# zhou-lab/biscuit

Measured on AMD Instinct MI355X. Metric: paired-end reads aligned/sec, higher is better.
Workload: dtype int32

## Files before the change

### biscuit_amd/csrc/hip/dev_common.hpp

```cpp
#pragma once
#include <stdint.h>
#include "bsx.h"

#if defined(__HIPCC__)
#include <hip/hip_runtime.h>
#define BSX_HD __host__ __device__ __forceinline__
#define BSX_D  __device__ __forceinline__
#else
#define BSX_HD inline
#define BSX_D  inline
struct uint4 { uint32_t x, y, z, w; };
#endif

struct DevFmi {
	uint64_t primary;
	uint64_t L2[5];
	uint64_t seq_len;
	const uint32_t *bwt;
	const uint64_t *sa;
	uint32_t sa_mask;
	uint32_t sa_shift;
};

struct DevSeedTab { const uint4 *t[2]; int32_t K; int32_t pad_; };

struct DevIndex {
	DevFmi fmi[2];
	const uint8_t *pac;
	int64_t l_pac;
	const int64_t *ctg_off;
	const uint8_t *ctg_alt;
	int32_t n_seqs;
	DevSeedTab tab;
	const int64_t *hole_off, *hole_end;
	int32_t n_holes, pad2_;
};

struct RegParams {
	int32_t a, w, o_del, e_del, o_ins, e_ins, pen_clip5, pen_clip3;
	int32_t min_seed_len, min_chain_weight, max_chain_gap, max_occ, bsstrand;
	uint32_t max_chain_extend;
	float mask_level, drop_ratio;
	int32_t prof;
	int32_t walk_on;
	int32_t ext_win;
	int32_t gap_cap;
	int32_t flt_len;
	const int32_t *flt_tab;
};

struct DevScoring {
	int8_t ctmat[25];
	int8_t gamat[25];
	int32_t o_del, e_del, o_ins, e_ins, zdrop, a;
	int32_t mx_ct, mx_ga;
};

BSX_HD int dev_ref_base(const uint8_t *pac, int64_t l_pac, int64_t p)
{
	if (p >= l_pac) { p = (l_pac << 1) - 1 - p; return 3 - ((pac[p >> 2] >> ((~p & 3) << 1)) & 3); }
	return (pac[p >> 2] >> ((~p & 3) << 1)) & 3;
}

BSX_HD void dev_fetch_window(uint8_t *win, const uint8_t *pac, int64_t l_pac, int64_t beg, int span, int lane)
{
	if (beg < l_pac && beg + span > l_pac) {
		for (int i = lane; i < span; i += 64) win[i] = (uint8_t)dev_ref_base(pac, l_pac, beg + i);
		return;
	}
	const bool rev = beg >= l_pac;
	const int64_t f_lo = rev ? (l_pac << 1) - (beg + span) : beg;
	const int64_t b0 = (f_lo >> 2) & ~(int64_t)3;
	const int nw = (int)((((f_lo + span - 1) >> 2) - b0) >> 2) + 1;
	for (int w = lane; w < nw; w += 64) {
		const uint8_t *pw = pac + b0 + (int64_t)4 * w;
		const uint32_t v = *reinterpret_cast<const uint32_t*>(pw);
		const int64_t f0 = (b0 + (int64_t)4 * w) << 2;
#pragma unroll
		for (int k = 0; k < 16; ++k) {
			const int b = (int)(v >> (8 * (k >> 2) + ((~k & 3) << 1))) & 3;
			const int64_t i = rev ? (f_lo + span - 1) - (f0 + k) : (f0 + k) - f_lo;
			if (i >= 0 && i < span) win[i] = (uint8_t)(rev ? 3 - b : b);
		}
	}
}

BSX_HD int dev_popc(uint32_t x)
{
#if defined(__HIP_DEVICE_COMPILE__)
	return __popc(x);
#else
	return __builtin_popcount(x);
#endif
}

BSX_HD void dev_block_count(const uint32_t w[8], int upto, uint32_t cnt[4])
{
	uint32_t a = 0, c = 0, g = 0, t = 0;
#pragma unroll
	for (int i = 0; i < 8; ++i) {
		int nv = upto + 1 - 16 * i;
		nv = nv < 0 ? 0 : (nv > 16 ? 16 : nv);
		uint32_t valid = nv == 0 ? 0u : (0x55555555u & ~(uint32_t)((1ull << ((16 - nv) << 1)) - 1));
		uint32_t lo = w[i] & valid, hi = (w[i] >> 1) & valid;
		uint32_t nt = (uint32_t)dev_popc(hi & lo), ng = (uint32_t)dev_popc(hi & ~lo), nc = (uint32_t)dev_popc(lo & ~hi);
		t += nt; g += ng; c += nc; a += (uint32_t)nv - nt - ng - nc;
	}
	cnt[0] = a; cnt[1] = c; cnt[2] = g; cnt[3] = t;
// ... 142 lines not shown
```

### biscuit_amd/csrc/hip/ext_dp.hpp

```cpp
#pragma once
#include <hip/hip_runtime.h>
#include "dev_common.hpp"
#include "wave.hpp"

template <int NC>
__device__ __forceinline__ bsx_ext_res_t ext_dp(const DevIndex &ix, const DevScoring &sc, const uint8_t *reads, const bsx_ext_job_t &J,
                                                int32_t *H, int32_t *E, uint8_t *qb, int lane)
{
	const int qlen = J.qlen, tlen = J.tlen, h0 = J.h0;
	const int8_t *mat = J.parent ? sc.ctmat : sc.gamat;
	const int o_del = sc.o_del, e_del = sc.e_del, o_ins = sc.o_ins, e_ins = sc.e_ins;
	const int oe_del = o_del + e_del, oe_ins = o_ins + e_ins, zdrop = sc.zdrop;
	for (int j = lane; j < qlen; j += 64) qb[j] = reads[(long long)J.qoff + (long long)j * J.qdir];
	for (int j = lane; j <= qlen; j += 64) {
		int v = j == 0 ? h0 : h0 - oe_ins - (j - 1) * e_ins;
		H[j] = v > 0 ? v : 0; E[j] = 0;
	}
	int mx = 0;
	for (int k = 0; k < 25; ++k) mx = mx > mat[k] ? mx : mat[k];
	int w = J.w;
	{
		int max_ins = (int)((double)(qlen * mx + J.end_bonus - o_ins) / e_ins + 1.);
		max_ins = max_ins > 1 ? max_ins : 1;
		w = w < max_ins ? w : max_ins;
		int max_del = (int)((double)(qlen * mx + J.end_bonus - o_del) / e_del + 1.);
		max_del = max_del > 1 ? max_del : 1;
		w = w < max_del ? w : max_del;
	}
	int max = h0, max_i = -1, max_j = -1, max_ie = -1, gscore = -1, max_off = 0;
	int beg = 0, end = qlen;
	int tb_reg = 4;
	WAVE_SYNC();
	for (int i = 0; i < tlen; ++i) {
		if ((i & 63) == 0) tb_reg = (i + lane < tlen) ? dev_ref_base(ix.pac, ix.l_pac, J.tpos + (long long)(i + lane) * J.tdir) : 4;
		const int t = wave_bcast(tb_reg, i & 63);
		const int8_t s0 = mat[t * 5], s1 = mat[t * 5 + 1], s2 = mat[t * 5 + 2], s3 = mat[t * 5 + 3], s4 = mat[t * 5 + 4];
		if (beg < i - w) beg = i - w;
		if (end > i + w + 1) end = i + w + 1;
		if (end > qlen) end = qlen;
		int h1_init = 0;
		if (beg == 0) { h1_init = h0 - (o_del + e_del * (i + 1)); if (h1_init < 0) h1_init = 0; }
		int m = 0, mj = -1, h1_last = h1_init;
		if (beg < end) {
			const int nch = (end - beg + 63) >> 6;
			int M[NC], Ev[NC];
#pragma unroll
			for (int c = 0; c < NC; ++c) {
				M[c] = 0; Ev[c] = 0;
				if (c < nch) {
					const int j = beg + (c << 6) + lane;
					if (j < end) {
						const int hp = H[j], q = qb[j];
						const int s = q == 0 ? s0 : q == 1 ? s1 : q == 2 ? s2 : q == 3 ? s3 : s4;
						M[c] = hp ? hp + s : 0;
						Ev[c] = E[j];
					}
// ... 23 lines not shown
						H[j + 1] = h;
						if (j == beg) H[beg] = h1_init;
						if (j == end - 1) E[end] = 0;
						if (h >= lm) { lm = h; lj = j; }
					}
				}
			}
			WAVE_SYNC();
			m = wave_max_i32(lm);
			mj = wave_max_i32(lm == m ? lj : -1);
			h1_last = H[end];
		} else {
			if (lane == 0) { H[end] = h1_init; E[end] = 0; }
			WAVE_SYNC();
		}
		const int jfin = beg < end ? end : beg;
		if (jfin == qlen) { max_ie = gscore > h1_last ? max_ie : i; gscore = gscore > h1_last ? gscore : h1_last; }
		if (m == 0) break;
		if (m > max) {
			max = m; max_i = i; max_j = mj;
			int off = mj - i; off = off < 0 ? -off : off;
			max_off = max_off > off ? max_off : off;
		} else if (zdrop > 0) {
			if (i - max_i > mj - max_j) { if (max - m - ((i - max_i) - (mj - max_j)) * e_del > zdrop) break; }
			else { if (max - m - ((mj - max_j) - (i - max_i)) * e_ins > zdrop) break; }
		}
		{
			const int nchk = (end - beg + 1 + 63) >> 6;
			int nb = end, last;
			for (int c = 0; c < nchk; ++c) {
				const int j = beg + (c << 6) + lane;
				const bool nz = j < end && (H[j] != 0 || E[j] != 0);
				const unsigned long long b = __ballot(nz);
				if (b) { nb = beg + (c << 6) + __builtin_ctzll(b); break; }
			}
			last = nb - 1;
			for (int c = nchk - 1; c >= 0; --c) {
				const int j = beg + (c << 6) + lane;
				const bool nz = j <= end && j >= nb && (H[j] != 0 || E[j] != 0);
				const unsigned long long b = __ballot(nz);
				if (b) { last = beg + (c << 6) + 63 - __builtin_clzll(b); break; }
			}
			beg = nb;
			end = last + 2 < qlen ? last + 2 : qlen;
		}
		WAVE_SYNC();
	}
	bsx_ext_res_t r;
	r.score = max; r.qle = max_j + 1; r.tle = max_i + 1; r.gtle = max_ie + 1; r.gscore = gscore; r.max_off = max_off;
	WAVE_SYNC();
	return r;
}

template <int NC>
__device__ __forceinline__ bsx_ext_res_t ext_dp_reg(const DevIndex &ix, const DevScoring &sc, const uint8_t *reads, const bsx_ext_job_t &J, int lane,
                                                    const uint8_t *win = nullptr, long long win_beg = 0, const uint8_t *qlds = nullptr, uint32_t qlds_off = 0)
{
	const int qlen = J.qlen, tlen = J.tlen, h0 = J.h0;
	const int8_t *mat = J.parent ? sc.ctmat : sc.gamat;
	const int o_del = sc.o_del, e_del = sc.e_del, o_ins = sc.o_ins, e_ins = sc.e_ins;
	const int oe_del = o_del + e_del, oe_ins = o_ins + e_ins, zdrop = sc.zdrop;
	int Hr[NC], Er[NC], sq4[NC];
	uint32_t sqp[NC];
#pragma unroll
	for (int c = 0; c < NC; ++c) {
		const int a = (c << 6) + lane;
		const int q = a < qlen ? (qlds ? (int)qlds[(int)(J.qoff - qlds_off) + a * J.qdir] : (int)reads[(long long)J.qoff + (long long)a * J.qdir]) : 4;
		sqp[c] = (uint32_t)(uint8_t)mat[q] | (uint32_t)(uint8_t)mat[5 + q] << 8 | (uint32_t)(uint8_t)mat[10 + q] << 16 | (uint32_t)(uint8_t)mat[15 + q] << 24;
		sq4[c] = mat[20 + q];
		const int v = a == 0 ? h0 : h0 - oe_ins - (a - 1) * e_ins;
		Hr[c] = (a <= qlen && v > 0) ? v : 0;
		Er[c] = 0;
	}
	const int mx = J.parent ? sc.mx_ct : sc.mx_ga;
	int w = J.w;
	{
		int max_ins = (int)((double)(qlen * mx + J.end_bonus - o_ins) / e_ins + 1.);
		max_ins = max_ins > 1 ? max_ins : 1;
		w = w < max_ins ? w : max_ins;
		int max_del = (int)((double)(qlen * mx + J.end_bonus - o_del) / e_del + 1.);
		max_del = max_del > 1 ? max_del : 1;
		w = w < max_del ? w : max_del;
	}
	int max = h0, max_i = -1, max_j = -1, max_ie = -1, gscore = -1, max_off = 0;
	int beg = 0, end = qlen;
	int tb_reg = 4;
	const bool packed_max = qlen <= 512 && (long long)h0 + (long long)qlen * mx < (1 << 21);
	for (int i = 0; i < tlen; ++i) {
		if ((i & 63) == 0) {
			const long long tp = J.tpos + (long long)(i + lane) * J.tdir;
			tb_reg = (i + lane < tlen) ? (win ? (int)win[tp - win_beg] : dev_ref_base(ix.pac, ix.l_pac, tp)) : 4;
		}
		const int t = wave_bcast(tb_reg, i & 63);
		if (beg < i - w) beg = i - w;
		if (end > i + w + 1) end = i + w + 1;
		if (end > qlen) end = qlen;
		int h1_init = 0;
		if (beg == 0) { h1_init = h0 - (o_del + e_del * (i + 1)); if (h1_init < 0) h1_init = 0; }
		int m = 0, mj = -1, h1_last = h1_init;
		if (beg < end) {
			const int c0 = NC == 1 ? 0 : beg >> 6, c1 = NC == 1 ? 0 : (end - 1) >> 6;
			int hn[NC];
			int carry = NEG_BIG, lm = -1, lj = -1;
#pragma unroll
			for (int c = 0; c < NC; ++c) {
				hn[c] = 0;
				if (c >= c0 && c <= c1) {
					const int a = (c << 6) + lane;
					const bool act = a >= beg && a < end;
					const int s = t < 4 ? (int)(int8_t)(sqp[c] >> ((t & 3) << 3)) : sq4[c];
					const int M = (act && Hr[c]) ? Hr[c] + s : 0;
					int tins = M - oe_ins; tins = tins > 0 ? tins : 0;
					const int g = act ? tins + a * e_ins : NEG_BIG;
					const int incl = wave_scan_max_incl(g);
					int excl = wave_prev(incl, NEG_BIG);
					excl = excl > carry ? excl : carry;
					{ const int tot = __builtin_amdgcn_readlane(incl, 63); carry = carry > tot ? carry : tot; }
					int f = a == beg ? 0 : excl - (a - 1) * e_ins;
					if (f < 0) f = 0;
					if (act) {
						int h = M > Er[c] ? M : Er[c];
						h = h > f ? h : f;
						int tdel = M - oe_del; tdel = tdel > 0 ? tdel : 0;
						int e = Er[c] - e_del; e = e > tdel ? e : tdel;
						Er[c] = e;
						hn[c] = h;
						if (h >= lm) { lm = h; lj = a; }
					} else if (a == end) Er[c] = 0;
				}
			}
			if (NC > 1 && (end & 63) == 0 && (end >> 6) < NC && (end >> 6) > c1) {
#pragma unroll
				for (int c = 0; c < NC; ++c) if (c == (end >> 6) && lane == 0) Er[c] = 0;
			}
#pragma unroll
			for (int c = NC - 1; c >= 0; --c) {
				if (c >= c0 && c <= c1 + 1) {
					const int a = (c << 6) + lane;
					int up = wave_prev(hn[c], 0);
					const int edge = c > 0 ? __builtin_amdgcn_readlane(hn[c > 0 ? c - 1 : 0], 63) : 0;
					if (lane == 0) up = edge;
// ... 1 lines not shown
					else if (a - 1 >= beg && a - 1 < end) Hr[c] = up;
				}
			}
			if (packed_max) {
				const int key = wave_max_i32(lm < 0 ? -1 : (lm << 9 | lj));
				m = key >> 9; mj = key < 0 ? -1 : (key & 511);
			} else {
				m = wave_max_i32(lm);
				mj = wave_max_i32(lm == m ? lj : -1);
			}
			if (end == qlen) {
				int v = 0;
#pragma unroll
				for (int c = 0; c < NC; ++c) if (c == c1) v = hn[c];
				h1_last = wave_bcast(v, (end - 1) & 63);
			}
		} else {
#pragma unroll
			for (int c = 0; c < NC; ++c) if ((c << 6) + lane == end) { Hr[c] = h1_init; Er[c] = 0; }
		}
		const int jfin = beg < end ? end : beg;
		if (jfin == qlen) { max_ie = gscore > h1_last ? max_ie : i; gscore = gscore > h1_last ? gscore : h1_last; }
		if (m == 0) break;
		if (m > max) {
			max = m; max_i = i; max_j = mj;
			int off = mj - i; off = off < 0 ? -off : off;
			max_off = max_off > off ? max_off : off;
		} else if (zdrop > 0) {
			if (i - max_i > mj - max_j) { if (max - m - ((i - max_i) - (mj - max_j)) * e_del > zdrop) break; }
			else { if (max - m - ((mj - max_j) - (i - max_i)) * e_ins > zdrop) break; }
		}
		{
			int nb = end, last;
#pragma unroll
			for (int c = 0; c < NC; ++c) {
				if (NC == 1 || (nb == end && c >= (beg >> 6) && c <= ((end - 1) >> 6))) {
					const int a = (c << 6) + lane;
					const unsigned long long b = __ballot(a >= beg && a < end && (Hr[c] != 0 || Er[c] != 0));
					if (b) nb = (c << 6) + __builtin_ctzll(b);
				}
			}
			last = nb - 1;
#pragma unroll
			for (int c = NC - 1; c >= 0; --c) {
				if (NC == 1 || (last == nb - 1 && c <= (end >> 6) && c >= (nb >> 6))) {
					const int a = (c << 6) + lane;
					const unsigned long long b = __ballot(a <= end && a >= nb && (Hr[c] != 0 || Er[c] != 0));
					if (b) last = (c << 6) + 63 - __builtin_clzll(b);
				}
			}
			beg = nb;
			end = last + 2 < qlen ? last + 2 : qlen;
		}
	}
	bsx_ext_res_t r;
	r.score = max; r.qle = max_j + 1; r.tle = max_i + 1; r.gtle = max_ie + 1; r.gscore = gscore; r.max_off = max_off;
	return r;
}

template <int NW>
__device__ __forceinline__ bsx_ext_res_t ext_dp_win(const DevIndex &ix, const DevScoring &sc, const uint8_t *reads, const bsx_ext_job_t &J, int lane,
                                                    const uint8_t *win = nullptr, long long win_beg = 0, const uint8_t *qlds = nullptr, uint32_t qlds_off = 0)
{
	const int qlen = J.qlen, tlen = J.tlen, h0 = J.h0;
	const int8_t *mat = J.parent ? sc.ctmat : sc.gamat;
	const int o_del = sc.o_del, e_del = sc.e_del, o_ins = sc.o_ins, e_ins = sc.e_ins;
	const int oe_del = o_del + e_del, oe_ins = o_ins + e_ins, zdrop = sc.zdrop;
	int Hr[NW], Er[NW], sq4[NW];
	uint32_t sqp[NW];
	int cb = 0;
#define EXT_WIN_LOAD(c_, slot_) do { const int a_ = ((slot_) << 6) + lane; \
		const int q_ = a_ < qlen ? (qlds ? (int)qlds[(int)(J.qoff - qlds_off) + a_ * J.qdir] : (int)reads[(long long)J.qoff + (long long)a_ * J.qdir]) : 4; \
		sqp[c_] = (uint32_t)(uint8_t)mat[q_] | (uint32_t)(uint8_t)mat[5 + q_] << 8 | (uint32_t)(uint8_t)mat[10 + q_] << 16 | (uint32_t)(uint8_t)mat[15 + q_] << 24; \
		sq4[c_] = mat[20 + q_]; \
		const int v_ = a_ == 0 ? h0 : h0 - oe_ins - (a_ - 1) * e_ins; \
		Hr[c_] = (a_ <= qlen && v_ > 0) ? v_ : 0; Er[c_] = 0; } while (0)
#pragma unroll
	for (int c = 0; c < NW; ++c) EXT_WIN_LOAD(c, c);
	const int mx = J.parent ? sc.mx_ct : sc.mx_ga;
	int w = J.w;
	{
		int max_ins = (int)((double)(qlen * mx + J.end_bonus - o_ins) / e_ins + 1.);
		max_ins = max_ins > 1 ? max_ins : 1;
		w = w < max_ins ? w : max_ins;
		int max_del = (int)((double)(qlen * mx + J.end_bonus - o_del) / e_del + 1.);
		max_del = max_del > 1 ? max_del : 1;
		w = w < max_del ? w : max_del;
	}
	int max = h0, max_i = -1, max_j = -1, max_ie = -1, gscore = -1, max_off = 0;
	int beg = 0, end = qlen;
	int tb_reg = 4;
	for (int i = 0; i < tlen; ++i) {
		if ((i & 63) == 0) {
			const long long tp = J.tpos + (long long)(i + lane) * J.tdir;
			tb_reg = (i + lane < tlen) ? (win ? (int)win[tp - win_beg] : dev_ref_base(ix.pac, ix.l_pac, tp)) : 4;
		}
		const int t = wave_bcast(tb_reg, i & 63);
		if (beg < i - w) beg = i - w;
		if (end > i + w + 1) end = i + w + 1;
		if (end > qlen) end = qlen;
		while ((beg >> 6) > cb) {
#pragma unroll
			for (int c = 0; c + 1 < NW; ++c) { Hr[c] = Hr[c + 1]; Er[c] = Er[c + 1]; sqp[c] = sqp[c + 1]; sq4[c] = sq4[c + 1]; }
			++cb;
			EXT_WIN_LOAD(NW - 1, cb + NW - 1);
		}
// ... 103 lines not shown
```

### biscuit_amd/csrc/hip/ext_pk.hpp

```cpp
#pragma once
#include <hip/hip_runtime.h>
#include "dev_common.hpp"
#include "wave.hpp"
#include "ext_pk_bound.h"

typedef short pk2 __attribute__((ext_vector_type(2)));
__device__ __forceinline__ pk2 pk_of(uint32_t w) { return __builtin_bit_cast(pk2, w); }
__device__ __forceinline__ uint32_t pk_word(pk2 v) { return __builtin_bit_cast(uint32_t, v); }
__device__ __forceinline__ pk2 pk_splat(int v) { return pk_of((uint32_t)(v & 0xffff) * 0x10001u); }
__device__ __forceinline__ pk2 pk_pair(int lo, int hi) { return pk_of((uint32_t)(lo & 0xffff) | (uint32_t)hi << 16); }
__device__ __forceinline__ pk2 pk_max(pk2 a, pk2 b) { return __builtin_elementwise_max(a, b); }
__device__ __forceinline__ pk2 pk_neg_mask(pk2 v) { uint32_t w; asm("v_pk_ashrrev_i16 %0, 15, %1 op_sel_hi:[0,1]" : "=v"(w) : "v"(pk_word(v))); return pk_of(w); }
__device__ __forceinline__ pk2 pk_nonzero_01(pk2 v) { uint32_t w; asm("v_pk_min_u16 %0, %1, 1 op_sel_hi:[1,0]" : "=v"(w) : "v"(pk_word(v))); return pk_of(w); }
__device__ __forceinline__ pk2 pk_zero_mask(pk2 v) { return pk_nonzero_01(v) - (pk2){1, 1}; }
__device__ __forceinline__ pk2 pk_nonzero_mask(pk2 v) { return (pk2){0, 0} - pk_nonzero_01(v); }
__device__ __forceinline__ pk2 pk_sel(pk2 mask, pk2 a, pk2 b) { return (a & mask) | (b & ~mask); }

__device__ __forceinline__ pk2 wave_scan_max_incl_pk(pk2 v)
{
	int t = 0;
#define PK_SCAN_STEP(ctrl, rows) do { t = __builtin_amdgcn_update_dpp(t, (int)pk_word(v), ctrl, rows, 0xf, true); v = pk_max(v, pk_of((uint32_t)t)); } while (0)
	PK_SCAN_STEP(DPP_ROW_SHR(1), 0xf); PK_SCAN_STEP(DPP_ROW_SHR(2), 0xf); PK_SCAN_STEP(DPP_ROW_SHR(4), 0xf); PK_SCAN_STEP(DPP_ROW_SHR(8), 0xf);
	PK_SCAN_STEP(DPP_ROW_BCAST15, 0xa); PK_SCAN_STEP(DPP_ROW_BCAST31, 0xc);
#undef PK_SCAN_STEP
	return v;
}

template <int NP>
__device__ __forceinline__ bsx_ext_res_t ext_dp_pk(const DevIndex &ix, const DevScoring &sc, const uint8_t *reads, const bsx_ext_job_t &J, int lane,
                                                   const uint8_t *win = nullptr, long long win_beg = 0, const uint8_t *qlds = nullptr, uint32_t qlds_off = 0)
{
	const int qlen = J.qlen, tlen = J.tlen, h0 = J.h0;
	const int8_t *mat = J.parent ? sc.ctmat : sc.gamat;
	const int o_del = sc.o_del, e_del = sc.e_del, o_ins = sc.o_ins, e_ins = sc.e_ins;
	const int oe_del = o_del + e_del, oe_ins = o_ins + e_ins, zdrop = sc.zdrop;
	const pk2 k_oe_ins = pk_splat(oe_ins), k_oe_del = pk_splat(oe_del), k_e_del = pk_splat(e_del), k_e_ins = pk_splat(e_ins), k_zero = pk_splat(0);
	pk2 Hp[NP], Ep[NP], sq4[NP];
	uint32_t sql[NP], sqh[NP];
#pragma unroll
	for (int p = 0; p < NP; ++p) {
		int hv[2], s4[2]; uint32_t sq[2];
#pragma unroll
		for (int u = 0; u < 2; ++u) {
			const int a = (p << 7) + (u << 6) + lane;
			const int q = a < qlen ? (qlds ? (int)qlds[(int)(J.qoff - qlds_off) + a * J.qdir] : (int)reads[(long long)J.qoff + (long long)a * J.qdir]) : 4;
			sq[u] = (uint32_t)(uint8_t)mat[q] | (uint32_t)(uint8_t)mat[5 + q] << 8 | (uint32_t)(uint8_t)mat[10 + q] << 16 | (uint32_t)(uint8_t)mat[15 + q] << 24;
			s4[u] = mat[20 + q];
			const int v = a == 0 ? h0 : h0 - oe_ins - (a - 1) * e_ins;
			hv[u] = (a <= qlen && v > 0) ? v : 0;
		}
		sql[p] = sq[0]; sqh[p] = sq[1]; sq4[p] = pk_pair(s4[0], s4[1]);
		Hp[p] = pk_pair(hv[0], hv[1]);
		Ep[p] = k_zero;
	}
	const int mx = J.parent ? sc.mx_ct : sc.mx_ga;
	int w = J.w;
	{
		int max_ins = (int)((double)(qlen * mx + J.end_bonus - o_ins) / e_ins + 1.);
		max_ins = max_ins > 1 ? max_ins : 1;
		w = w < max_ins ? w : max_ins;
		int max_del = (int)((double)(qlen * mx + J.end_bonus - o_del) / e_del + 1.);
		max_del = max_del > 1 ? max_del : 1;
		w = w < max_del ? w : max_del;
	}
	int max = h0, max_i = -1, max_j = -1, max_ie = -1, gscore = -1, max_off = 0;
	int beg = 0, end = qlen;
	int tb_reg = 4;
	for (int i = 0; i < tlen; ++i) {
		if ((i & 63) == 0) {
			const long long tp = J.tpos + (long long)(i + lane) * J.tdir;
			tb_reg = (i + lane < tlen) ? (win ? (int)win[tp - win_beg] : dev_ref_base(ix.pac, ix.l_pac, tp)) : 4;
		}
		const int t = wave_bcast(tb_reg, i & 63);
		if (beg < i - w) beg = i - w;
		if (end > i + w + 1) end = i + w + 1;
		if (end > qlen) end = qlen;
		int h1_init = 0;
		if (beg == 0) { h1_init = h0 - (o_del + e_del * (i + 1)); if (h1_init < 0) h1_init = 0; }
		int m = 0, mj = -1, h1_last = h1_init;
		unsigned long long nzl[NP], nzh[NP];
#pragma unroll
		for (int p = 0; p < NP; ++p) nzl[p] = nzh[p] = 0;
		if (beg < end) {
			const int p0 = NP == 1 ? 0 : beg >> 7, p1 = NP == 1 ? 0 : end >> 7;
			const pk2 k_beg = pk_splat(beg), k_end = pk_splat(end), k_h1 = pk_splat(h1_init);
			const int tsh = (t & 3) << 3;
			int carry = 0, edge = 0, lkey = -1, vlast = 0;
#pragma unroll
			for (int p = 0; p < NP; ++p) {
				if (NP == 1 || (p >= p0 && p <= p1)) {
					const pk2 a = pk_pair((p << 7) + lane, (p << 7) + 64 + lane);
					const pk2 db = a - k_beg, de = a - k_end;
					const pk2 act = pk_neg_mask(de & ~db);
					const pk2 isbeg = pk_zero_mask(db), isend = pk_zero_mask(de);
					const pk2 hr = Hp[p], er = Ep[p];
					const pk2 s = t < 4 ? pk_pair((int)(int8_t)(sql[p] >> tsh), (int)(int8_t)(sqh[p] >> tsh)) : sq4[p];
					const pk2 M = (hr + s) & act & pk_nonzero_mask(hr);
					const pk2 tins = pk_max(M - k_oe_ins, k_zero);
					const pk2 g = (tins + a * k_e_ins) & act;
					const pk2 incl = wave_scan_max_incl_pk(g);
					pk2 excl = pk_of((uint32_t)__builtin_amdgcn_update_dpp(0, (int)pk_word(incl), DPP_WAVE_SHR1, 0xf, 0xf, true));
					{
						const uint32_t tot = (uint32_t)__builtin_amdgcn_readlane((int)pk_word(incl), 63);
						const int tl = (int)(tot & 0xffffu), th = (int)(tot >> 16);
						const int cl = carry > tl ? carry : tl;
						excl = pk_max(excl, pk_pair(carry, cl));
						carry = cl > th ? cl : th;
					}
					pk2 f = pk_max(excl - (a - (pk2){1, 1}) * k_e_ins, k_zero);
					f = f & ~isbeg;
					const pk2 h = pk_max(pk_max(M, er), f) & act;
					const pk2 e = pk_max(er - k_e_del, pk_max(M - k_oe_del, k_zero));
					const pk2 en = pk_sel(act, e, er & ~isend);
					Ep[p] = en;
					const uint32_t hw = pk_word(h);
					const uint32_t h63 = (uint32_t)__builtin_amdgcn_readlane((int)hw, 63);
					const pk2 up = pk_of((uint32_t)wave_prev((int)hw, (int)((uint32_t)edge | h63 << 16)));
					edge = (int)(h63 >> 16);
					const pk2 hn = pk_sel(isbeg, k_h1, pk_sel((act | isend) & ~isbeg, up, hr));
					Hp[p] = hn;
					{
						const int kl = (int)((hw & 0xffffu) << 9) | ((p << 7) + lane), kh = (int)((hw >> 16) << 9) | ((p << 7) + 64 + lane);
						lkey = lkey > kl ? lkey : kl; lkey = lkey > kh ? lkey : kh;
					}
					if (end == qlen && ((end - 1) >> 7) == p) vlast = (int)(((end - 1) & 64) ? hw >> 16 : hw & 0xffffu);
					const uint32_t nz = pk_word((hn | en) & (act | isend));
					nzl[p] = __ballot((nz & 0xffffu) != 0);
					nzh[p] = __ballot(nz > 0xffffu);
				}
			}
			{
				const int key = wave_max_i32(lkey);
				m = key >> 9; mj = key & 511;
			}
			if (end == qlen) h1_last = wave_bcast(vlast, (end - 1) & 63);
		}
		const int jfin = beg < end ? end : beg;
		if (jfin == qlen) { max_ie = gscore > h1_last ? max_ie : i; gscore = gscore > h1_last ? gscore : h1_last; }
		if (m == 0) break;
		if (m > max) {
			max = m; max_i = i; max_j = mj;
			int off = mj - i; off = off < 0 ? -off : off;
			max_off = max_off > off ? max_off : off;
		} else if (zdrop > 0) {
			if (i - max_i > mj - max_j) { if (max - m - ((i - max_i) - (mj - max_j)) * e_del > zdrop) break; }
			else { if (max - m - ((mj - max_j) - (i - max_i)) * e_ins > zdrop) break; }
		}
		{
			int nb = end, last = -2;
#pragma unroll
			for (int p = NP - 1; p >= 0; --p) {
				if (nzh[p]) nb = (p << 7) + 64 + __builtin_ctzll(nzh[p]);
				if (nzl[p]) nb = (p << 7) + __builtin_ctzll(nzl[p]);
			}
#pragma unroll
			for (int p = 0; p < NP; ++p) {
				if (nzl[p]) last = (p << 7) + 63 - __builtin_clzll(nzl[p]);
				if (nzh[p]) last = (p << 7) + 127 - __builtin_clzll(nzh[p]);
			}
			if (last == -2) last = nb - 1;
			beg = nb;
			end = last + 2 < qlen ? last + 2 : qlen;
		}
	}
	bsx_ext_res_t r;
	r.score = max; r.qle = max_j + 1; r.tle = max_i + 1; r.gtle = max_ie + 1; r.gscore = gscore; r.max_off = max_off;
	return r;
}
```

### biscuit_amd/csrc/hip/k_c2r.hip

```cpp
#include <hip/hip_runtime.h>
#include "dev_common.hpp"
#include "wave.hpp"
#include "kernels.h"
#include "ext_dp.hpp"
#include "ext_pk.hpp"
#include "rgx.hpp"
#include "rg_common.hpp"

#define RG_XSEEDS 128
#define RG_XREGS 64
#define RG_XCBLK 16
template <int QC, int WC, int XSD, int XRG = RG_XREGS, bool ROWS_ = true>
struct RgC2rT {
	static const int QCAP = QC, WINCAP = WC, XSEEDS = XSD, XREGS = XRG, GAPCAP = QC > RG_QCAP ? RG_QCAP : QC;
	static const bool HBM = false, ROWS = ROWS_;
	unsigned long long pf[RG_NPF];
	bsx_region_t regs[XRG];
	RgXChain xc[RG_XCBLK];
	RgXExt xe[RG_XCBLK];
	RgXSeed sd[XSD];
	unsigned long long srt[XSD];
	uint8_t q[QC];
	uint8_t win[WC];
	int n_regs;
// ... 140 lines not shown
					if (!any) {
						if constexpr (TALLY) if (has_ext == 1 && pass == 0 && uni(W.xe[ci - xc_lo].status) == 1 && uni(W.xe[ci - xc_lo].si) == si) {
							const unsigned long long at = (unsigned long long)((const unsigned char*)(XEw + (size_t)ci * (sizeof(RgXExt) / 8)) - X.base);
							const unsigned int rw = (unsigned int)uni((int)((const unsigned int*)(X.base + rgx_rows_offset(X.cap)))[RGX_ROWS_AT(at)]);
							const unsigned long long rows = rw & ~RGX_ROWS_L;
							const unsigned long long v = lane == X4W_JOBS ? 1ull : lane == X4W_ROWS ? rows : u != 0 ? 0ull : lane == X4W_JOBS_R0 ? 1ull : rows;
							if (lane < 4 && v) atomicAdd(&counters[CTR_X4W + ((rw & RGX_ROWS_L) ? 4 : 0) + lane], v);
						}
						++pf_skip; WAVE_SYNC(); if (lane == 0) W.srt[k] = 0; WAVE_SYNC(); continue;
					}
				}
				RgXExt xe = W.xe[ci - xc_lo];
				if (has_ext == 2 && pass == 0) {
					const unsigned long long *xp = XEw + (size_t)(l0 + si) * (sizeof(RgXExt) / 8);
					const unsigned long long v = lane < (int)(sizeof(RgXExt) / 8) ? xp[lane] : 0ull;
					unsigned long long w6[sizeof(RgXExt) / 8];
#pragma unroll
					for (int q = 0; q < (int)(sizeof(RgXExt) / 8); ++q) w6[q] = (unsigned long long)(unsigned)__builtin_amdgcn_readlane((int)(v >> 32), q) << 32 | (unsigned)__builtin_amdgcn_readlane((int)v, q);
					memcpy(&xe, w6, sizeof(xe));
				}
				const bool cached = has_ext && pass == 0 && uni(xe.status) == 1 && uni(xe.si) == si;
				if (cached) ++pf_cached; else ++pf_inl;
				if (!cached && win_ok == 0) {
					const int span = (int)(rmax1 - rmax0);
					if (span > 0 && span <= WT::WINCAP) {
						dev_fetch_window(W.win, ix.pac, l_pac, rmax0, span, lane);
						win_ok = 1;
						WAVE_SYNC();
					} else win_ok = -1;
				}
				bsx_region_t R; memset(&R, 0, sizeof(R));
				int aw0 = P.w, aw1 = P.w;
				const int qe = s_qbeg + s_len;
				R.score = R.truesc = -1; R.rid = rid;
				if (cached) {
					R.rb = uni64(xe.rb); R.re = uni64(xe.re); R.qb = uni(xe.qb); R.qe = uni(xe.qe); R.score = uni(xe.score); R.truesc = uni(xe.truesc);
					aw0 = uni(xe.aw0); aw1 = uni(xe.aw1);
				} else
				for (int side = 0; side < 2; ++side) {
					if (side == 0 && s_qbeg == 0) { R.score = R.truesc = s_len * P.a; R.qb = 0; R.rb = s_rbeg; continue; }
					if (side == 1 && qe == l_query) { R.qe = l_query; R.re = s_rbeg + s_len; continue; }
					const int sc0 = R.score, clip = side ? P.pen_clip3 : P.pen_clip5;
					int aw = P.w;
					bsx_ext_res_t res; res.score = -1; res.qle = res.tle = res.gtle = 0; res.gscore = -1; res.max_off = 0;
					bsx_ext_job_t J;
					J.parent = (uint8_t)parent; J.pad = 0; J.end_bonus = clip;
					if (side == 0) { J.qoff = qoff + (uint32_t)s_qbeg - 1; J.qdir = -1; J.qlen = s_qbeg; J.tpos = s_rbeg - 1; J.tdir = -1; J.tlen = (int)(s_rbeg - rmax0); J.h0 = s_len * P.a; }
					else { J.qoff = qoff + (uint32_t)qe; J.qdir = 1; J.qlen = l_query - qe; J.tpos = s_rbeg + s_len; J.tdir = 1; J.tlen = (int)(rmax1 - (s_rbeg + s_len)); J.h0 = sc0; }
					for (int i = 0; i < 2; ++i) {
						const int prev = R.score;
						aw = P.w << i;
						J.w = aw;
						if (P.prof) { const long long now_ = (long long)__builtin_readcyclecounter(); RG_PF_ADD(W, 6, now_ - pf_t); pf_t = now_; }
						if (J.qlen < 64) res = ext_dp_reg<1>(ix, sc, reads, J, lane, win_ok > 0 ? W.win : nullptr, rmax0, W.q, qoff);
						else if constexpr (PK && WT::QCAP <= 256) {
							if (J.qlen < 128) res = ext_dp_pk<1>(ix, sc, reads, J, lane, win_ok > 0 ? W.win : nullptr, rmax0, W.q, qoff);
							else res = ext_dp_pk<2>(ix, sc, reads, J, lane, win_ok > 0 ? W.win : nullptr, rmax0, W.q, qoff);
						}
						else if (J.qlen < 128) res = ext_dp_reg<2>(ix, sc, reads, J, lane, win_ok > 0 ? W.win : nullptr, rmax0, W.q, qoff);
						else if (WT::QCAP <= 256 || J.qlen < 256) res = ext_dp_reg<RG_NC>(ix, sc, reads, J, lane, win_ok > 0 ? W.win : nullptr, rmax0, W.q, qoff);
						else if (P.ext_win && 2 * J.w + 1 <= 256 && (long long)J.h0 + (long long)J.qlen * (parent ? sc.mx_ct : sc.mx_ga) < (1 << 21))
							res = ext_dp_win<5>(ix, sc, reads, J, lane, win_ok > 0 ? W.win : nullptr, rmax0, W.q, qoff);
						else if (WT::ROWS && 2 * J.w + 1 <= 512) { WAVE_SYNC(); res = ext_dp<8>(ix, sc, reads, J, W.Hrow, W.Erow, W.qrow, lane); }
						else return 2;
						res.score = uni(res.score); res.qle = uni(res.qle); res.tle = uni(res.tle); res.gtle = uni(res.gtle);
						res.gscore = uni(res.gscore); res.max_off = uni(res.max_off);
						R.score = res.score;
						if (P.prof) { const long long now_ = (long long)__builtin_readcyclecounter(); RG_PF_ADD(W, 7, now_ - pf_t); pf_t = now_; }
						++pf_ext; pf_rows += (unsigned int)(res.tle > res.gtle ? res.tle : res.gtle);
						if (P.prof && J.qlen >= 64) RG_PF_ADD(W, 15, (unsigned long long)(res.tle > res.gtle ? res.tle : res.gtle) << (J.qlen >= 128 ? 32 : 0));
						if (R.score == prev || res.max_off < (aw >> 1) + (aw >> 2)) break;
					}
					const int local = res.gscore <= 0 || res.gscore <= R.score - clip;
					if (side == 0) {
						aw0 = aw;
						if (local) { R.qb = s_qbeg - res.qle; R.rb = s_rbeg - res.tle; R.truesc = R.score; }
						else { R.qb = 0; R.rb = s_rbeg - res.gtle; R.truesc = res.gscore; }
					} else {
						aw1 = aw;
						if (local) { R.qe = qe + res.qle; R.re = s_rbeg + s_len + res.tle; R.truesc += R.score - sc0; }
						else { R.qe = l_query; R.re = s_rbeg + s_len + res.gtle; R.truesc += res.gscore - sc0; }
					}
				}
				R.bss = (uint8_t)RG_BSS(parent, l_pac, R.rb); R.parent = (uint8_t)parent;
				if (RG_BSS(parent, l_pac, R.re) != R.bss) continue;
				int cov = 0;
				for (int i = lane; i < nl; i += 64) {
					const RgXSeed td = Lsd[i];
					if (td.qbeg >= R.qb && td.qbeg + td.len <= R.qe && td.rbeg >= R.rb && td.rbeg + td.len <= R.re) cov += td.len;
				}
				R.seedcov = uni(wave_sum_i32(cov));
				R.w = aw0 > aw1 ? aw0 : aw1; R.seedlen0 = s_len; R.frac_rep = frac_rep;
				if (uni(W.n_regs) == WT::XREGS) return 6;
				WAVE_SYNC();
				if (lane == 0) { W.regs[W.n_regs] = R; ++W.n_regs; }
				WAVE_SYNC();
			}
		}
	}
	if (P.prof) { RG_PF_ADD(W, 6, (long long)__builtin_readcyclecounter() - pf_t); RG_PF_ADD(W, 8, pf_ext); RG_PF_ADD(W, 9, pf_rows);
	              RG_PF_ADD(W, 11, pf_seen); RG_PF_ADD(W, 12, pf_skip); RG_PF_ADD(W, 13, pf_cached); RG_PF_ADD(W, 14, pf_inl); }
	return 0;
#undef C2R_STAGE_CHAINS
#undef C2R_STAGE_SEEDS
}

#ifndef C2R_WPB
#define C2R_WPB 1
#endif
template <typename WT, int OCC, bool PK = false, bool TALLY = false>
__global__ void __launch_bounds__(64 * C2R_WPB, OCC)
k_c2r(DevIndex ix, DevScoring sc, RegParams P, const uint8_t *reads, const bsx_seed_task_t *tasks, RgXPool X,
      bsx_region_t *out, unsigned long long out_cap, unsigned long long *out_cursor, long long *reg_off, int *reg_n,
// ... 84 lines not shown
```

### biscuit_amd/csrc/hip/k_ext4.hip

```cpp
#include <hip/hip_runtime.h>
#include <stdlib.h>
#include <string.h>
#include <algorithm>
#include "dev_common.hpp"
#include "wave.hpp"
#include "kernels.h"
#include "tune.h"
#include "rgx.hpp"
#include "x4.hpp"

size_t x4_job_bytes(void) { return sizeof(X4Job); }

#define X4_GAPCAP 256
#define X4_XSEEDS 128
#define X4P_WPB 4
__global__ void __launch_bounds__(64 * X4P_WPB)
k_x4prep(DevIndex ix, RegParams P, const bsx_seed_task_t *tasks, RgXPool X, X4Job *jobs, unsigned int jcap, unsigned int *jcount)
{
	__shared__ int gap_tab[X4_GAPCAP + 1];
	__shared__ int s_pre[X4P_WPB][64];
	__shared__ unsigned long long s_rec[X4P_WPB][64];
	__shared__ unsigned int s_qoff[X4P_WPB][64];
	__shared__ int s_lq[X4P_WPB][64];
	P.gap_cap = X4_GAPCAP;
	for (int q = threadIdx.x; q <= X4_GAPCAP; q += blockDim.x) gap_tab[q] = rg_cal_max_gap(P, q);
	__syncthreads();
	const int lane = wave_lane(), wv = (int)(threadIdx.x >> 6);
	const unsigned int n = *X.xcount;
	const unsigned int i0 = ((unsigned int)blockIdx.x * X4P_WPB + (unsigned int)wv) * 64u;
	if (i0 >= n) return;
	const long long l_pac = ix.l_pac;
	int nk = 0;
	if (i0 + lane < n) {
		const int t = X.xlist[i0 + lane];
		const unsigned long long at = (unsigned long long)X.xoff[t];
		const RgXHdr *H = (const RgXHdr*)(X.base + at);
		nk = H->has_ext ? H->n_chains : 0;
		s_rec[wv][lane] = at;
		s_qoff[wv][lane] = tasks[t].qoff;
		s_lq[wv][lane] = tasks[t].len << 1 | (tasks[t].parent & 1);
	}
	const int incl = wave_scan_sum_incl(nk);
	s_pre[wv][lane] = incl;
	const int tot = __builtin_amdgcn_readlane(incl, 63);
	WAVE_SYNC();
	for (int b = 0; b < tot; b += 64) {
		const int j = b + lane;
		int n_it = 0, mode = 0, best = -1, ci = 0, l_query = 0, parent = 0, s = 0;
		long long rmax0 = 0, rmax1 = 0;
		const RgXSeed *XS = nullptr; RgXExt *XE = nullptr; RgXChain c; c.pos = 0; c.rid = 0; c.seed_off = 0; c.n_main = c.n_extra = 0; c.pad = 0;
		RgXExt xe0; xe0.rb = xe0.re = 0; xe0.qb = xe0.qe = 0; xe0.score = xe0.truesc = -1; xe0.aw0 = xe0.aw1 = P.w; xe0.si = -1; xe0.status = 0;
		if (j < tot) {
			int lo = 0, hi = 63;
			while (lo < hi) { const int mid = (lo + hi) >> 1; if (s_pre[wv][mid] > j) hi = mid; else lo = mid + 1; }
			s = lo;
			const unsigned long long at = s_rec[wv][s];
			const RgXHdr *H = (const RgXHdr*)(X.base + at);
			const int nch = H->n_chains, n_sd = H->n_seeds;
			mode = H->has_ext;
			ci = j - (s_pre[wv][s] - nch);
			l_query = s_lq[wv][s] >> 1; parent = s_lq[wv][s] & 1;
			const RgXChain *XC = (const RgXChain*)(H + 1);
// ... 97 lines not shown
{
#define X4_PK_STEP(n) do { const uint32_t t_ = (uint32_t)__builtin_amdgcn_update_dpp(0, (int)v, DPP_ROW_ROR(n), 0xf, 0xf, false); \
		const x4_us2 m_ = __builtin_elementwise_max(__builtin_bit_cast(x4_us2, v), __builtin_bit_cast(x4_us2, t_)); v = __builtin_bit_cast(uint32_t, m_); } while (0)
	X4_PK_STEP(1); X4_PK_STEP(2); X4_PK_STEP(4); X4_PK_STEP(8);
#undef X4_PK_STEP
	return v;
}
__device__ __forceinline__ int q_prev(int v, int first) { return __builtin_amdgcn_update_dpp(first, v, DPP_ROW_SHR(1), 0xf, 0xf, false); }
__device__ __forceinline__ int q_ror1(int v) { return __builtin_amdgcn_update_dpp(v, v, DPP_ROW_ROR(1), 0xf, 0xf, false); }
__device__ __forceinline__ int q_last(int v) { return __builtin_amdgcn_update_dpp(v, v, DPP_ROW_NEWBCAST(15), 0xf, 0xf, false); }

enum { X4_IDLE = 0, X4_NEXT, X4_ROW, X4_AFTER, X4_REFILL, X4_DONE };
#define X4_ROWS 48

template <int NCQ, bool CHAIN, bool TALLY = false>
__global__ void __launch_bounds__(256, X4_OCC)
k_ext4(DevIndex ix, DevScoring sc, RegParams P, const uint8_t *reads, const void *jobs_, void *res_, unsigned char *xbase,
       const unsigned int *n_ptr, unsigned int n_fixed, unsigned int *cursor, unsigned long long *prof, int take_second)
{
	__shared__ uint32_t s_sqp[2][8];
	if (threadIdx.x < 10) {
		const int p = threadIdx.x / 5, q = threadIdx.x % 5;
		const int8_t *mat = p ? sc.ctmat : sc.gamat;
		s_sqp[p][q] = (uint32_t)(uint8_t)mat[q] | (uint32_t)(uint8_t)mat[5 + q] << 8 | (uint32_t)(uint8_t)mat[10 + q] << 16 | (uint32_t)(uint8_t)mat[15 + q] << 24;
	}
	__syncthreads();
	const int lane = wave_lane(), l = lane & 15, gsh = lane & 48;
	unsigned int n = n_ptr ? *n_ptr : n_fixed, n_first = n;
	if (CHAIN) {
		n_first = n < n_fixed / 2 ? n : n_fixed / 2;
		const unsigned int n_second = take_second ? (n_ptr[2] < n_fixed / 2 ? n_ptr[2] : n_fixed / 2) : 0u;
		n = n_first + n_second;
	}
	const int o_del = sc.o_del, e_del = sc.e_del, o_ins = sc.o_ins, e_ins = sc.e_ins;
	const int oe_del = o_del + e_del, oe_ins = o_ins + e_ins, zdrop = sc.zdrop;
	const long long l_pac = ix.l_pac;
	int st = X4_IDLE, wait = 0;
	unsigned int e = 0;
	unsigned int wnext = 0, wend = 0; bool wdone = false;
	long long s_rbeg = 0, rmax0 = 0, rmax1 = 0; unsigned long long ext_at = 0;
	unsigned int qoff0 = 0; int l_query = 0, s_qbeg = 0, s_len = 0, par = 0, si = 0;
	int side = 0, attempt = 0, prev = 0, sc0 = 0, aw = 0, clip = 0;
	int R_qb = 0, R_qe = 0, R_score = 0, R_truesc = 0, aw0 = 0, aw1 = 0; long long R_rb = 0, R_re = 0;
	unsigned int jq = 0; int jqdir = 1, jtdir = 1, jbonus = 0; long long jtpos = 0;
	int qlen = 0, tlen = 0, h0 = 0, w = 0, i = 0, beg = 0, end = 0;
	long long tF = 0; int tfd = 1, tcomp = 0, yleft = 0;
	uint32_t y0 = 0, y1 = 0, y2 = 0;
	int max = 0, max_i = -1, max_j = -1, max_ie = -1, gscore = -1, max_off = 0;
	int Hr[NCQ], Er[NCQ]; uint32_t sqp[NCQ];
#pragma unroll
	for (int c = 0; c < NCQ; ++c) { Hr[c] = Er[c] = 0; sqp[c] = 0; }
	unsigned int pf_rows = 0, pf_trips = 0, pf_jobs = 0, pf_cold = 0, pf_slots = 0, pf_nrows = 0;
	[[maybe_unused]] unsigned int jrows = 0;
	for (;;) {
		{
			const bool cold = st != X4_ROW && st != X4_DONE;
			const unsigned long long cm = __ballot(cold), rm = __ballot(st == X4_ROW);
			if (cold) ++wait;
			if (cm && (rm == 0 || __popcll(cm) >= 32 || __ballot(wait >= 3))) {
				++pf_cold;
				if (st == X4_REFILL) {
					x4_bases(ix.pac, tF + (long long)i * tfd, tfd, tlen - i, y0, y1, y2);
					yleft = X4_ROWS; st = X4_ROW;
				}
				if (st == X4_AFTER) {
					const int r_score = max, r_qle = max_j + 1, r_tle = max_i + 1, r_gtle = max_ie + 1, r_gscore = gscore, r_off = max_off;
					if (!CHAIN) {
						if (l == 0) { bsx_ext_res_t r; r.score = r_score; r.qle = r_qle; r.tle = r_tle; r.gtle = r_gtle; r.gscore = r_gscore; r.max_off = r_off; ((bsx_ext_res_t*)res_)[e] = r; }
						st = X4_IDLE;
					} else {
						R_score = r_score;
						if (attempt == 0 && !(R_score == prev || r_off < (aw >> 1) + (aw >> 2))) { attempt = 1; st = X4_NEXT; }
						else {
							const int local = r_gscore <= 0 || r_gscore <= R_score - clip;
							if (side == 0) {
								aw0 = aw;
								if (local) { R_qb = s_qbeg - r_qle; R_rb = s_rbeg - r_tle; R_truesc = R_score; }
								else { R_qb = 0; R_rb = s_rbeg - r_gtle; R_truesc = r_gscore; }
							} else {
								aw1 = aw;
								if (local) { R_qe = s_qbeg + s_len + r_qle; R_re = s_rbeg + s_len + r_tle; R_truesc += R_score - sc0; }
								else { R_qe = l_query; R_re = s_rbeg + s_len + r_gtle; R_truesc += r_gscore - sc0; }
							}
							++side; attempt = 0; st = X4_NEXT;
						}
					}
				}
				auto x4_step = [&]() {
					if (CHAIN && st == X4_NEXT && attempt == 0) {
						if (side == 0 && s_qbeg == 0) { R_score = R_truesc = s_len * P.a; R_qb = 0; R_rb = s_rbeg; side = 1; }
						if (side == 1 && s_qbeg + s_len == l_query) { R_qe = l_query; R_re = s_rbeg + s_len; side = 2; }
						if (side >= 2) {
							if (l == 0) {
								RgXExt xe; xe.rb = R_rb; xe.re = R_re; xe.qb = R_qb; xe.qe = R_qe; xe.score = R_score; xe.truesc = R_truesc;
								xe.aw0 = aw0; xe.aw1 = aw1; xe.si = si; xe.status = 1;
								*(RgXExt*)(xbase + ext_at) = xe;
								if constexpr (TALLY) ((unsigned int*)res_)[RGX_ROWS_AT(ext_at)] = jrows;
							}
							st = X4_IDLE;
						}
					}
				};
				x4_step();
				const unsigned long long need = __ballot(st == X4_IDLE);
				if (need) {
					const unsigned long long heads = need & 0x0001000100010001ull;
					if (wnext == wend) {
						unsigned int base = 0;
						if (lane == 0) base = atomicAdd(cursor, 64u);
						base = (unsigned int)__builtin_amdgcn_readfirstlane((int)base);
						wnext = base < n ? base : n; wend = base + 64u < n ? base + 64u : n;
						if (wnext == wend) wdone = true;
					}
					const unsigned int e_new = wnext + (unsigned int)__popcll(heads & ((1ull << gsh) - 1));
					const bool served = e_new < wend;
					wnext = wnext + (unsigned int)__popcll(heads) < wend ? wnext + (unsigned int)__popcll(heads) : wend;
					if (st == X4_IDLE) {
					if (!served) { if (wdone) st = X4_DONE; }
					else if (CHAIN) {
						e = e_new;
						const X4Job J = ((const X4Job*)jobs_)[e < n_first ? e : n_fixed / 2 + (e - n_first)];
						s_rbeg = J.s_rbeg; rmax0 = J.rmax0; rmax1 = J.rmax1; ext_at = J.ext_at; qoff0 = J.qoff;
						l_query = J.l_query; s_qbeg = J.s_qbeg; s_len = J.s_len; par = J.parent; si = J.si;
						side = 0; attempt = 0; aw0 = aw1 = P.w; R_score = R_truesc = -1; R_qb = R_qe = 0; R_rb = R_re = 0;
						if constexpr (TALLY) jrows = 0;
						++pf_jobs;
						st = X4_NEXT;
					} else {
						e = e_new;
						const bsx_ext_job_t J = ((const bsx_ext_job_t*)jobs_)[e];
						par = J.parent ? 1 : 0;
						jq = J.qoff; jqdir = J.qdir; qlen = J.qlen; jtpos = J.tpos; jtdir = J.tdir; tlen = J.tlen; h0 = J.h0; aw = J.w; jbonus = J.end_bonus;
						++pf_jobs;
						st = X4_NEXT;
					}
					}
				}
				x4_step();
				if (st == X4_NEXT) {
					const bool go = true;
					if (CHAIN) {
						const int qe = s_qbeg + s_len;
						prev = R_score;
						if (attempt == 0) sc0 = R_score;
						aw = P.w << attempt;
						clip = side ? P.pen_clip3 : P.pen_clip5;
						jbonus = clip;
						if (side == 0) { jq = qoff0 + (unsigned int)s_qbeg - 1; jqdir = -1; qlen = s_qbeg; jtpos = s_rbeg - 1; jtdir = -1; tlen = (int)(s_rbeg - rmax0); h0 = s_len * P.a; }
						else { jq = qoff0 + (unsigned int)qe; jqdir = 1; qlen = l_query - qe; jtpos = s_rbeg + s_len; jtdir = 1; tlen = (int)(rmax1 - (s_rbeg + s_len)); h0 = sc0; }
					}
					if (go) {
						const int mx = par ? sc.mx_ct : sc.mx_ga;
						if (qlen + 1 > 16 * NCQ || qlen < 0 || (long long)h0 + (long long)qlen * mx >= (1 << 21)) {
							if (CHAIN) st = X4_IDLE;
							else { if (l == 0) { bsx_ext_res_t r; r.score = X4_DECLINED; r.qle = r.tle = r.gtle = r.gscore = r.max_off = 0; ((bsx_ext_res_t*)res_)[e] = r; } st = X4_IDLE; }
						} else {
							max = h0; max_i = max_j = max_ie = -1; gscore = -1; max_off = 0;
							beg = 0; end = qlen; i = 0;
							if (tlen <= 0) st = X4_AFTER;
							else {
#pragma unroll
								for (int c = 0; c < NCQ; ++c) {
									const int a = (c << 4) + l;
									int q = a < qlen ? (int)reads[(long long)jq + (long long)a * jqdir] : 4;
									q = q < 4 ? q : 4;
									sqp[c] = s_sqp[par][q];
									const int v = a == 0 ? h0 : h0 - oe_ins - (a - 1) * e_ins;
									Hr[c] = (a <= qlen && v > 0) ? v : 0;
									Er[c] = 0;
								}
								w = aw;
								{
									int max_ins = (int)((double)(qlen * mx + jbonus - o_ins) / e_ins + 1.);
									max_ins = max_ins > 1 ? max_ins : 1;
									w = w < max_ins ? w : max_ins;
									int max_del = (int)((double)(qlen * mx + jbonus - o_del) / e_del + 1.);
									max_del = max_del > 1 ? max_del : 1;
									w = w < max_del ? w : max_del;
								}
								if (jtpos >= l_pac) { tF = (l_pac << 1) - 1 - jtpos; tfd = -jtdir; tcomp = 3; } else { tF = jtpos; tfd = jtdir; tcomp = 0; }
								x4_bases(ix.pac, tF, tfd, tlen, y0, y1, y2);
								yleft = X4_ROWS;
								st = X4_ROW;
							}
						}
					}
				}
				if (st == X4_ROW || st == X4_DONE) wait = 0;
			}
			if (rm == 0 && __ballot(st == X4_ROW) == 0) { if (__ballot(st != X4_DONE) == 0) break; continue; }
		}
		++pf_trips;
		const bool run = st == X4_ROW;
		if (run) { ++pf_rows; if (CHAIN && s_len < X4_NARROW) ++pf_nrows; if constexpr (TALLY) ++jrows; }
		const int t = (int)(y0 & 3u) ^ tcomp;
		y0 = __builtin_amdgcn_alignbit(y1, y0, 2); y1 = __builtin_amdgcn_alignbit(y2, y1, 2); y2 >>= 2; --yleft;
		beg = beg > i - w ? beg : i - w;
		end = end < i + w + 1 ? end : i + w + 1; end = end < qlen ? end : qlen;
		int h1_init = h0 - (o_del + e_del * (i + 1)); h1_init = (beg == 0 && h1_init > 0) ? h1_init : 0;
		int m = 0, mj = -1, h1_last = h1_init;
		const bool nonempty = run && beg < end;
		const int c_lo = beg >> 4, c_hi = end >> 4;
		const unsigned int sm_l = nonempty ? (2u << c_hi) - (1u << c_lo) : 0u;
		const unsigned int smask = (unsigned int)__builtin_amdgcn_readlane((int)sm_l, 0) | (unsigned int)__builtin_amdgcn_readlane((int)sm_l, 16) |
		                           (unsigned int)__builtin_amdgcn_readlane((int)sm_l, 32) | (unsigned int)__builtin_amdgcn_readlane((int)sm_l, 48);
		uint32_t zpk = 0;
		pf_slots += (unsigned int)__builtin_popcount(smask);
		if (smask) {
			int carry = NEG_BIG, kmax = -1, hprev = 0, vlast = 0;
			const int tsh = t << 3;
#pragma unroll
			for (int c = 0; c < NCQ; ++c) {
				if (smask >> c & 1u) {
					const int a = (c << 4) + l;
					const bool in = nonempty && c >= c_lo && c <= c_hi;
					const bool act = in && a >= beg && a < end;
					const int hr = Hr[c], er = Er[c];
					const int s = (int)(int8_t)(sqp[c] >> tsh);
					const int M = (act && hr) ? hr + s : 0;
					int tins = M - oe_ins; tins = tins > 0 ? tins : 0;
					const int g = act ? tins + a * e_ins : NEG_BIG;
					const int incl = q_scan_max_incl(g);
					int excl = q_prev(incl, NEG_BIG);
					excl = excl > carry ? excl : carry;
					{ const int tot = q_last(incl); carry = carry > tot ? carry : tot; }
					int f = excl - (a - 1) * e_ins;
					f = (a == beg || f < 0) ? 0 : f;
					int h = M > er ? M : er; h = h > f ? h : f; h = act ? h : 0;
					int ee = M - oe_del; ee = ee > 0 ? ee : 0; ee = ee > er - e_del ? ee : er - e_del;
					const int en = act ? ee : ((in && a == end) ? 0 : er);
					Er[c] = en;
					{ const int key = act ? (h << 9 | a) : -1; kmax = kmax > key ? kmax : key; }
					vlast = (act && a == end - 1) ? h : vlast;
					int up = q_prev(h, 0);
					const int edge = q_ror1(hprev);
					up = l == 0 ? edge : up;
					const int hn = !in ? hr : a == beg ? h1_init : (a - 1 >= beg && a - 1 < end) ? up : hr;
					Hr[c] = hn;
					hprev = h;
					const bool nz = in && a >= beg && a <= end && (hn | en) != 0;
					{
						const uint32_t hi = (nz && a < end && (zpk >> 16) == 0) ? (uint32_t)(0xffff - a) << 16 : zpk & 0xffff0000u;
						const uint32_t lo = nz ? (uint32_t)(a + 1) : zpk & 0xffffu;
						zpk = hi | lo;
					}
				}
			}
			{
				const int key = q_allmax(kmax);
				m = nonempty ? key >> 9 : 0; mj = (nonempty && key >= 0) ? (key & 511) : -1;
			}
			if (__ballot(nonempty && end == qlen)) {
				const int v = q_allmax(vlast);
				h1_last = (nonempty && end == qlen) ? v : h1_last;
			}
		}
		if (__ballot(run && !nonempty)) {
#pragma unroll
			for (int c = 0; c < NCQ; ++c) { const bool hit = run && !nonempty && (c << 4) + l == end; Hr[c] = hit ? h1_init : Hr[c]; Er[c] = hit ? 0 : Er[c]; }
		}
		bool stop = false;
		if (run) {
			const int jfin = beg < end ? end : beg;
			if (jfin == qlen) { max_ie = gscore > h1_last ? max_ie : i; gscore = gscore > h1_last ? gscore : h1_last; }
			stop = m == 0;
			if (!stop) {
				if (m > max) {
					max = m; max_i = i; max_j = mj;
					int off = mj - i; off = off < 0 ? -off : off;
					max_off = max_off > off ? max_off : off;
				} else if (zdrop > 0) {
					if (i - max_i > mj - max_j) stop = max - m - ((i - max_i) - (mj - max_j)) * e_del > zdrop;
					else stop = max - m - ((mj - max_j) - (i - max_i)) * e_ins > zdrop;
				}
			}
		}
		const bool shrink = run && !stop;
		{
			const uint32_t zr = q_allmax_pk(zpk);
			int nb = (zr >> 16) ? 0xffff - (int)(zr >> 16) : 0x7fffffff;
			int last = (int)(zr & 0xffffu) - 1;
			if (shrink) {
				nb = nb < end ? nb : end;
				last = last > nb - 1 ? last : nb - 1;
				beg = nb;
				end = last + 2 < qlen ? last + 2 : qlen;
				++i;
				if (i >= tlen) stop = true;
				else if (yleft == 0) st = X4_REFILL;
			}
		}
		if (run && stop) st = X4_AFTER;
	}
	if (prof) {
		pf_rows = (unsigned int)wave_sum_i32(l == 0 ? (int)pf_rows : 0); pf_jobs = (unsigned int)wave_sum_i32(l == 0 ? (int)pf_jobs : 0);
		if (lane == 0) { atomicAdd(&prof[EXT4_JOBS], (unsigned long long)pf_jobs); atomicAdd(&prof[EXT4_ROWS], (unsigned long long)pf_rows); atomicAdd(&prof[EXT4_TRIPS], (unsigned long long)pf_trips); atomicAdd(&prof[EXT4_COLD], (unsigned long long)pf_cold); atomicAdd(&prof[EXT4_SLOTS], (unsigned long long)pf_slots); }
		pf_nrows = (unsigned int)wave_sum_i32(l == 0 ? (int)pf_nrows : 0);
		if (lane == 0) atomicAdd(&prof[EXT4_NARROW_ROWS], (unsigned long long)pf_nrows);
	}
}

int x4_max_query(int ncq) { return 16 * ncq - 1; }

void launch_ext4_batch(hipStream_t st, int n_cu, const DevIndex &ix, const DevScoring &sc, const uint8_t *reads, const bsx_ext_job_t *jobs, bsx_ext_res_t *res,
                       unsigned int n, unsigned int *cursor, int max_qlen)
{
	const long long want = ((long long)n + 15) / 16;
	const int grid = (int)std::max<long long>(1, std::min<long long>(want, (long long)n_cu * 8));
	RegParams P; memset(&P, 0, sizeof(P));
	if (max_qlen <= x4_max_query(10))
		hipLaunchKernelGGL((k_ext4<10, false>), dim3(grid), dim3(256), 0, st, ix, sc, P, reads, (const void*)jobs, (void*)res, (unsigned char*)nullptr, (const unsigned int*)nullptr, n, cursor, (unsigned long long*)nullptr, 0);
	else
		hipLaunchKernelGGL((k_ext4<16, false>), dim3(grid), dim3(256), 0, st, ix, sc, P, reads, (const void*)jobs, (void*)res, (unsigned char*)nullptr, (const unsigned int*)nullptr, n, cursor, (unsigned long long*)nullptr, 0);
}

void launch_x4(hipStream_t st, int n_cu, const RgLaunch &G, const RgXPoolArg &XA, void *jobs, unsigned long long job_cap, unsigned int *ctr32, unsigned long long *prof)
{
	const DevIndex &ix = *G.ix; const DevScoring &sc = *G.sc; const RegParams &P = *G.P;
	const uint8_t *reads = G.reads; const bsx_seed_task_t *tasks = G.tasks; const long long n_tasks = G.n_tasks;
	RgXPool X = rgx_pool(&XA);
	const unsigned int jcap = (unsigned int)std::min<unsigned long long>(job_cap, 0xfffffff0ull);
	const int pgrid = (int)((n_tasks + 64 * X4P_WPB - 1) / (64 * X4P_WPB));
	(void)hipMemsetAsync(ctr32, 0, 16, st);
	if (XA.rows) (void)hipMemsetAsync(XA.rows, 0, rgx_rows_bytes(X.cap), st);
	hipLaunchKernelGGL(k_x4prep, dim3(std::max(1, pgrid)), dim3(64 * X4P_WPB), 0, st, ix, P, tasks, X, (X4Job*)jobs, jcap, ctr32);
	const int use_l = (int)bsx_tune_long("xl", 1);
	if (use_l) launch_extl(st, n_cu, ix, sc, P, reads, jobs, jcap, ctr32, X.base, n_tasks * 4, prof, XA.rows);
	const int wpc = 3;
	const int grid = (int)std::max<long long>(1, std::min<long long>((n_tasks * 4 + 15) / 16, (long long)n_cu * wpc));
	if (XA.rows) hipLaunchKernelGGL((k_ext4<10, true, true>), dim3(grid), dim3(256), 0, st, ix, sc, P, reads, (const void*)jobs, (void*)XA.rows, X.base, (const unsigned int*)ctr32, jcap, ctr32 + 1, prof, use_l ? 0 : 1);
	else hipLaunchKernelGGL((k_ext4<10, true>), dim3(grid), dim3(256), 0, st, ix, sc, P, reads, (const void*)jobs, (void*)nullptr, X.base, (const unsigned int*)ctr32, jcap, ctr32 + 1, prof, use_l ? 0 : 1);
}
```

### biscuit_amd/csrc/hip/k_extend.hip

```cpp
#include <hip/hip_runtime.h>
#include "dev_common.hpp"
#include "wave.hpp"
#include "kernels.h"
#include "ext_dp.hpp"
#include "ext_pk.hpp"

template <int NC>
__global__ void __launch_bounds__(256)
k_extend(DevIndex ix, DevScoring sc, const uint8_t *reads, const bsx_ext_job_t *jobs, const int *order, long long n,
         bsx_ext_res_t *res, int qcap, int32_t *hbm_rows)
{
	extern __shared__ int32_t lds[];
	const int lane = wave_lane();
	const int waves_per_block = blockDim.x >> 6;
	const int wave = threadIdx.x >> 6;
	const int stride = 2 * (qcap + 2) + ((qcap + 3) >> 2) + 1;
	int32_t *H = hbm_rows ? hbm_rows + ((size_t)blockIdx.x * waves_per_block + wave) * (size_t)stride : lds + wave * stride;
	int32_t *E = H + (qcap + 2);
	uint8_t *qb = reinterpret_cast<uint8_t*>(E + (qcap + 2));

	for (long long jj = (long long)blockIdx.x * waves_per_block + wave; jj < n; jj += (long long)gridDim.x * waves_per_block) {
		const int job = order[jj];
		const bsx_ext_job_t J = jobs[job];
		const bsx_ext_res_t r = ext_dp<NC>(ix, sc, reads, J, H, E, qb, lane);
// ... 12 lines not shown
	const size_t lds = (size_t)wpb * stride * 4;
	long long blocks = (n + wpb - 1) / wpb;
	long long cap = (long long)n_cu * 32;
	if (blocks > cap) blocks = cap;
	if (lds > 48 * 1024) (void)hipFuncSetAttribute((const void*)k_extend<NC>, hipFuncAttributeMaxDynamicSharedMemorySize, (int)lds);
	hipLaunchKernelGGL(k_extend<NC>, dim3((unsigned)blocks), dim3(wpb * 64), lds, st, ix, sc, reads, jobs, order, n, res, qcap, (int32_t*)nullptr);
}
size_t extend_hbm_row_bytes(int qcap) { return (size_t)(2 * (qcap + 2) + ((qcap + 3) >> 2) + 1) * 4; }
void launch_extend_hbm(hipStream_t st, const DevIndex &ix, const DevScoring &sc, const uint8_t *reads, const bsx_ext_job_t *jobs, const int *order,
                       long long n, bsx_ext_res_t *res, int qcap, int blocks, void *rows)
{
	hipLaunchKernelGGL(k_extend<32>, dim3((unsigned)blocks), dim3(256), 0, st, ix, sc, reads, jobs, order, n, res, qcap, (int32_t*)rows);
}

void launch_extend(hipStream_t st, const DevIndex &ix, const DevScoring &sc, const uint8_t *reads, const bsx_ext_job_t *jobs, const int *order,
                   long long n, bsx_ext_res_t *res, int qcap, int nc, int n_cu)
{
	if (nc <= 4) launch_ext_nc<4>(st, ix, sc, reads, jobs, order, n, res, qcap, n_cu);
	else if (nc <= 8) launch_ext_nc<8>(st, ix, sc, reads, jobs, order, n, res, qcap, n_cu);
	else launch_ext_nc<32>(st, ix, sc, reads, jobs, order, n, res, qcap, n_cu);
}

__global__ void __launch_bounds__(256)
k_extend_win(DevIndex ix, DevScoring sc, const uint8_t *reads, const bsx_ext_job_t *jobs, long long n, bsx_ext_res_t *res)
{
	const int lane = wave_lane();
	const int waves_per_block = blockDim.x >> 6, wave = threadIdx.x >> 6;
	for (long long jj = (long long)blockIdx.x * waves_per_block + wave; jj < n; jj += (long long)gridDim.x * waves_per_block) {
		const bsx_ext_job_t J = jobs[jj];
		const int mx = J.parent ? sc.mx_ct : sc.mx_ga;
		bsx_ext_res_t r;
		if (2 * J.w + 1 <= 256 && (long long)J.h0 + (long long)J.qlen * mx < (1 << 21)) r = ext_dp_win<5>(ix, sc, reads, J, lane);
		else { r.score = X4_DECLINED; r.qle = r.tle = r.gtle = r.gscore = r.max_off = 0; }
		if (lane == 0) res[jj] = r;
	}
}
void launch_extwin_batch(hipStream_t st, int n_cu, const DevIndex &ix, const DevScoring &sc, const uint8_t *reads, const bsx_ext_job_t *jobs, bsx_ext_res_t *res, long long n)
{
	long long blocks = (n + 3) / 4;
	if (blocks > (long long)n_cu * 8) blocks = (long long)n_cu * 8;
	hipLaunchKernelGGL(k_extend_win, dim3((unsigned)(blocks > 0 ? blocks : 1)), dim3(256), 0, st, ix, sc, reads, jobs, n, res);
}

template <bool PK>
__global__ void __launch_bounds__(256)
k_extend_pk(DevIndex ix, DevScoring sc, const uint8_t *reads, const bsx_ext_job_t *jobs, long long n, bsx_ext_res_t *res)
{
	const int lane = wave_lane();
	const int waves_per_block = blockDim.x >> 6, wave = threadIdx.x >> 6;
	for (long long jj = (long long)blockIdx.x * waves_per_block + wave; jj < n; jj += (long long)gridDim.x * waves_per_block) {
		const bsx_ext_job_t J = jobs[jj];
		bsx_ext_res_t r;
		if (J.qlen > EXT_PK_QMAX) { r.score = X4_DECLINED; r.qle = r.tle = r.gtle = r.gscore = r.max_off = 0; }
		else if (!PK) r = ext_dp_reg<4>(ix, sc, reads, J, lane);
		else if (J.qlen < 128) r = ext_dp_pk<1>(ix, sc, reads, J, lane);
		else r = ext_dp_pk<2>(ix, sc, reads, J, lane);
		if (lane == 0) res[jj] = r;
	}
}
void launch_extpk_batch(hipStream_t st, int n_cu, const DevIndex &ix, const DevScoring &sc, const uint8_t *reads, const bsx_ext_job_t *jobs, bsx_ext_res_t *res, long long n, bool packed)
{
	long long blocks = (n + 3) / 4;
	if (blocks > (long long)n_cu * 8) blocks = (long long)n_cu * 8;
	if (packed) hipLaunchKernelGGL(k_extend_pk<true>, dim3((unsigned)(blocks > 0 ? blocks : 1)), dim3(256), 0, st, ix, sc, reads, jobs, n, res);
	else hipLaunchKernelGGL(k_extend_pk<false>, dim3((unsigned)(blocks > 0 ? blocks : 1)), dim3(256), 0, st, ix, sc, reads, jobs, n, res);
}
```

### biscuit_amd/csrc/hip/k_extl.hip

```cpp
#include <hip/hip_runtime.h>
#include <stdlib.h>
#include <string.h>
#include <algorithm>
#include "dev_common.hpp"
#include "wave.hpp"
#include "kernels.h"
#include "rgx.hpp"
#include "x4.hpp"

#define XL_W 64
#define XL_QCOLS 128
#ifndef XL_OCC
#define XL_OCC 2
#endif
enum { XL_IDLE = 0, XL_NEXT, XL_ROW, XL_AFTER, XL_REFILL, XL_BAIL, XL_DONE };

__device__ __forceinline__ int xl_max3(int a, int b, int c) { const int m = a > b ? a : b; return m > c ? m : c; }

template <bool CHAIN, bool TALLY = false>
__global__ void __launch_bounds__(64, XL_OCC)
k_extl(DevIndex ix, DevScoring sc, RegParams P, const uint8_t *reads, void *jobs_, void *res_, unsigned int jcap, unsigned int *ctr32, unsigned char *xbase, unsigned long long *prof)
{
	X4Job *jobs = (X4Job*)jobs_;
	__shared__ uint32_t s_srow[2][4];
	if (threadIdx.x < 8) {
		const int p = threadIdx.x >> 2, t = threadIdx.x & 3;
		const int8_t *mat = p ? sc.ctmat : sc.gamat;
		s_srow[p][t] = (uint32_t)(uint8_t)mat[t * 5] | (uint32_t)(uint8_t)mat[t * 5 + 1] << 8 | (uint32_t)(uint8_t)mat[t * 5 + 2] << 16 | (uint32_t)(uint8_t)mat[t * 5 + 3] << 24;
	}
	__syncthreads();
	const int lane = (int)threadIdx.x;
	const unsigned int half = jcap / 2;
	const unsigned int n = !CHAIN ? jcap : ctr32[2] < half ? ctr32[2] : half;
	unsigned int e = 0;
	unsigned int bq = 0; int bqdir = 1, btdir = 1; long long btpos = 0;
	const int o_del = sc.o_del, e_del = sc.e_del, o_ins = sc.o_ins, e_ins = sc.e_ins;
	const int oe_del = o_del + e_del, oe_ins = o_ins + e_ins, zdrop = sc.zdrop;
	const long long l_pac = ix.l_pac;
	int st = XL_IDLE, wait = 0;
	unsigned int wnext = 0, wend = 0; bool wdone = false;
	long long s_rbeg = 0, rmax0 = 0, rmax1 = 0; unsigned long long ext_at = 0;
	unsigned int qoff0 = 0; int l_query = 0, s_qbeg = 0, s_len = 0, par = 0, si = 0;
	int side = 0, attempt = 0, prev = 0, sc0 = 0, aw = 0, clip = 0;
	int R_qb = 0, R_qe = 0, R_score = 0, R_truesc = 0, aw0 = 0, aw1 = 0; long long R_rb = 0, R_re = 0;
	int qlen = 0, tlen = 0, h0 = 0, w = 0, i = 0, beg = 0, end = 0, base = 0;
	long long tF = 0; int tfd = 1, tcomp = 0, yleft = 0;
	uint32_t y0 = 0, y1 = 0, y2 = 0;
	int max = 0, max_i = -1, max_j = -1, max_ie = -1, gscore = -1, max_off = 0;
	uint32_t R[XL_W];
	uint32_t QF[XL_QCOLS / 16];
	uint32_t QW[XL_W / 16];
	uint32_t M0 = 0, M1 = 0, M2 = 0, M3 = 0;
#pragma unroll
	for (int p = 0; p < XL_W; ++p) R[p] = 0;
#pragma unroll
	for (int g = 0; g < XL_QCOLS / 16; ++g) QF[g] = 0;
#pragma unroll
	for (int g = 0; g < XL_W / 16; ++g) QW[g] = 0;
	unsigned int pf_rows = 0, pf_trips = 0, pf_jobs = 0, pf_cold = 0, pf_bail = 0;
	[[maybe_unused]] unsigned int jrows = 0;
#define XL_QWIN() do { const int b16_ = base >> 4; _Pragma("unroll") for (int g_ = 0; g_ < XL_W / 16; ++g_) { uint32_t v_ = 0; \
		_Pragma("unroll") for (int k_ = 0; k_ < XL_QCOLS / 16; ++k_) v_ = b16_ + g_ == k_ ? QF[k_] : v_; QW[g_] = v_; } } while (0)
	for (;;) {
		{
			const bool cold = st != XL_ROW && st != XL_DONE;
			const unsigned long long cm = __ballot(cold), rm = __ballot(st == XL_ROW);
			if (cold) ++wait;
			if (cm && (rm == 0 || __popcll(cm) >= 16 || __ballot(wait >= 4))) {
				++pf_cold;
				if (st == XL_REFILL) { x4_bases(ix.pac, tF + (long long)i * tfd, tfd, tlen - i, y0, y1, y2); yleft = 48; st = XL_ROW; }
				if (st == XL_AFTER) {
					const int r_score = max, r_qle = max_j + 1, r_tle = max_i + 1, r_gtle = max_ie + 1, r_gscore = gscore, r_off = max_off;
					R_score = r_score;
					if (!CHAIN) {
						bsx_ext_res_t r; r.score = r_score; r.qle = r_qle; r.tle = r_tle; r.gtle = r_gtle; r.gscore = r_gscore; r.max_off = r_off;
						((bsx_ext_res_t*)res_)[e] = r;
						st = XL_IDLE;
					} else
					if (attempt == 0 && !(R_score == prev || r_off < (aw >> 1) + (aw >> 2))) { attempt = 1; st = XL_NEXT; }
					else {
						const int local = r_gscore <= 0 || r_gscore <= R_score - clip;
						if (side == 0) {
							aw0 = aw;
							if (local) { R_qb = s_qbeg - r_qle; R_rb = s_rbeg - r_tle; R_truesc = R_score; }
							else { R_qb = 0; R_rb = s_rbeg - r_gtle; R_truesc = r_gscore; }
						} else {
							aw1 = aw;
							if (local) { R_qe = s_qbeg + s_len + r_qle; R_re = s_rbeg + s_len + r_tle; R_truesc += R_score - sc0; }
							else { R_qe = l_query; R_re = s_rbeg + s_len + r_gtle; R_truesc += r_gscore - sc0; }
						}
						++side; attempt = 0; st = XL_NEXT;
					}
				}
				auto xl_step = [&]() {
					if (CHAIN && st == XL_NEXT && attempt == 0) {
						if (side == 0 && s_qbeg == 0) { R_score = R_truesc = s_len * P.a; R_qb = 0; R_rb = s_rbeg; side = 1; }
						if (side == 1 && s_qbeg + s_len == l_query) { R_qe = l_query; R_re = s_rbeg + s_len; side = 2; }
						if (side >= 2) {
							RgXExt xe; xe.rb = R_rb; xe.re = R_re; xe.qb = R_qb; xe.qe = R_qe; xe.score = R_score; xe.truesc = R_truesc;
							xe.aw0 = aw0; xe.aw1 = aw1; xe.si = si; xe.status = 1;
							*(RgXExt*)(xbase + ext_at) = xe;
							if constexpr (TALLY) ((unsigned int*)res_)[RGX_ROWS_AT(ext_at)] = jrows | RGX_ROWS_L;
							st = XL_IDLE;
						}
					}
				};
				xl_step();
				{
					const unsigned long long bm = __ballot(st == XL_BAIL);
					if (bm) {
						unsigned int b0 = 0;
						if (lane == 0) b0 = atomicAdd(&ctr32[0], (unsigned int)__popcll(bm));
						b0 = (unsigned int)__builtin_amdgcn_readfirstlane((int)b0);
// ... 10 lines not shown
					}
				}
				const unsigned long long need = __ballot(st == XL_IDLE);
				if (need) {
					if (wnext == wend) {
						unsigned int b0 = 0;
						if (lane == 0) b0 = atomicAdd(&ctr32[3], 64u);
						b0 = (unsigned int)__builtin_amdgcn_readfirstlane((int)b0);
						wnext = b0 < n ? b0 : n; wend = b0 + 64u < n ? b0 + 64u : n;
						if (wnext == wend) wdone = true;
					}
					const unsigned int e_new = wnext + (unsigned int)__popcll(need & ((1ull << lane) - 1));
					const bool served = e_new < wend;
					wnext = wnext + (unsigned int)__popcll(need) < wend ? wnext + (unsigned int)__popcll(need) : wend;
					if (st == XL_IDLE) {
						if (!served) { if (wdone) st = XL_DONE; }
						else if (!CHAIN) {
							e = e_new;
							const bsx_ext_job_t J = ((const bsx_ext_job_t*)jobs_)[e];
							par = J.parent ? 1 : 0;
							bq = J.qoff; bqdir = J.qdir; qlen = J.qlen; btpos = J.tpos; btdir = J.tdir; tlen = J.tlen; h0 = J.h0; aw = J.w; clip = J.end_bonus;
							++pf_jobs;
							st = XL_NEXT;
						} else {
							const X4Job J = jobs[half + e_new];
							s_rbeg = J.s_rbeg; rmax0 = J.rmax0; rmax1 = J.rmax1; ext_at = J.ext_at; qoff0 = J.qoff;
							l_query = J.l_query; s_qbeg = J.s_qbeg; s_len = J.s_len; par = J.parent; si = J.si;
							side = 0; attempt = 0; aw0 = aw1 = P.w; R_score = R_truesc = -1; R_qb = R_qe = 0; R_rb = R_re = 0;
							if constexpr (TALLY) jrows = 0;
							++pf_jobs;
							st = XL_NEXT;
						}
					}
				}
				xl_step();
				if (st == XL_NEXT) {
					const int qe = s_qbeg + s_len;
					unsigned int jq; int jqdir, jtdir; long long jtpos;
					if (!CHAIN) { jq = bq; jqdir = bqdir; jtdir = btdir; jtpos = btpos; }
					else {
					prev = R_score;
					if (attempt == 0) sc0 = R_score;
					aw = P.w << attempt;
					clip = side ? P.pen_clip3 : P.pen_clip5;
					if (side == 0) { jq = qoff0 + (unsigned int)s_qbeg - 1; jqdir = -1; qlen = s_qbeg; jtpos = s_rbeg - 1; jtdir = -1; tlen = (int)(s_rbeg - rmax0); h0 = s_len * P.a; }
					else { jq = qoff0 + (unsigned int)qe; jqdir = 1; qlen = l_query - qe; jtpos = s_rbeg + s_len; jtdir = 1; tlen = (int)(rmax1 - (s_rbeg + s_len)); h0 = sc0; }
					}
					const int mx = par ? sc.mx_ct : sc.mx_ga;
					int jmax0 = h0 > oe_ins ? (h0 - oe_ins - 1) / e_ins + 1 : 0;
					jmax0 = jmax0 < qlen ? jmax0 : qlen;
					if (qlen < 0 || h0 < 0 || jmax0 + 2 >= XL_W || (long long)h0 + (long long)qlen * mx >= 32768) st = XL_BAIL;
					else {
						max = h0; max_i = max_j = max_ie = -1; gscore = -1; max_off = 0;
						beg = 0; end = qlen; i = 0; base = 0;
						if (tlen <= 0) st = XL_AFTER;
						else {
							const uint8_t *qp = reads + jq;
							const int nq = qlen < XL_QCOLS ? qlen : XL_QCOLS;
							uint32_t amb = 0;
#pragma unroll
							for (int k = 0; k < XL_QCOLS / 16; ++k) QF[k] = 0;
#pragma unroll
							for (int g = 0; g < XL_QCOLS / 4; ++g) {
								uint32_t x = 0;
								if (g * 4 + 4 <= nq) {
									if (jqdir > 0) { uint32_t v; __builtin_memcpy(&v, qp + g * 4, 4); x = v; }
									else { uint32_t v; __builtin_memcpy(&v, qp - g * 4 - 3, 4); x = __builtin_bswap32(v); }
								} else if (g * 4 < nq) {
									for (int k = 0; k < 3; ++k) if (g * 4 + k < nq) x |= (uint32_t)qp[(long long)(g * 4 + k) * jqdir] << (k << 3);
								}
								amb |= x & 0xfcfcfcfcu;
								const uint32_t p4 = (x & 3u) | ((x >> 6) & 0xcu) | ((x >> 12) & 0x30u) | ((x >> 18) & 0xc0u);
								QF[g >> 2] |= p4 << ((g & 3) << 3);
							}
							if (amb) st = XL_BAIL;
							else {
								XL_QWIN();
								M0 = s_srow[par][0]; M1 = s_srow[par][1]; M2 = s_srow[par][2]; M3 = s_srow[par][3];
#pragma unroll
								for (int p = 0; p < XL_W; ++p) {
									const int v = p == 0 ? h0 : h0 - oe_ins - (p - 1) * e_ins;
									R[p] = (p <= qlen && v > 0) ? (uint32_t)v : 0u;
								}
								w = aw;
								{
									int max_ins = (int)((double)(qlen * mx + clip - o_ins) / e_ins + 1.);
									max_ins = max_ins > 1 ? max_ins : 1;
									w = w < max_ins ? w : max_ins;
									int max_del = (int)((double)(qlen * mx + clip - o_del) / e_del + 1.);
									max_del = max_del > 1 ? max_del : 1;
									w = w < max_del ? w : max_del;
								}
								if (jtpos >= l_pac) { tF = (l_pac << 1) - 1 - jtpos; tfd = -jtdir; tcomp = 3; } else { tF = jtpos; tfd = jtdir; tcomp = 0; }
								x4_bases(ix.pac, tF, tfd, tlen, y0, y1, y2);
								yleft = 48;
								st = XL_ROW;
							}
						}
					}
				}
				if (st == XL_ROW || st == XL_DONE) wait = 0;
			}
			if (rm == 0 && __ballot(st == XL_ROW) == 0) { if (__ballot(st != XL_DONE) == 0) break; continue; }
		}
		++pf_trips;
		const bool run = st == XL_ROW;
		if (run) { ++pf_rows; if constexpr (TALLY) ++jrows; }
		const int t = (int)(y0 & 3u) ^ tcomp;
		y0 = __builtin_amdgcn_alignbit(y1, y0, 2); y1 = __builtin_amdgcn_alignbit(y2, y1, 2); y2 >>= 2; --yleft;
		beg = beg > i - w ? beg : i - w;
		end = end < i + w + 1 ? end : i + w + 1; end = end < qlen ? end : qlen;
		int h1 = h0 - (o_del + e_del * (i + 1)); h1 = (beg == 0 && h1 > 0) ? h1 : 0;
		int f = 0, key = -1, first = XL_W, last = -1;
		const uint32_t srow = t == 0 ? M0 : t == 1 ? M1 : t == 2 ? M2 : M3;
		const int rb = run ? beg - base : XL_W + 1, re_e = run ? end - base : -1, re = re_e < XL_W ? re_e : XL_W;
#pragma unroll
		for (int p = 0; p < XL_W; ++p) {
			const uint32_t x = R[p];
			const bool c_act = p >= rb && p < re;
			const bool c_end = p == re_e;
			const int Hd = (int)(x & 0xffffu), e = (int)(x >> 16);
			const int q2 = (int)((QW[p >> 4] >> ((p & 15) << 1)) & 3u);
			const int s = (int)(int8_t)(srow >> (q2 << 3));
			const int M = Hd ? Hd + s : 0;
			const int h = xl_max3(M, e, f);
			const int e2 = xl_max3(e - e_del, M - oe_del, 0);
			const int f2 = xl_max3(f - e_ins, M - oe_ins, 0);
			const uint32_t nr = (uint32_t)h1 | (c_act ? (uint32_t)e2 << 16 : 0u);
			const uint32_t xn = (c_act || c_end) ? nr : x;
			R[p] = xn;
			{ const int k = h << 8 | p; key = (c_act && k > key) ? k : key; }
			h1 = c_act ? h : h1;
			f = c_act ? f2 : f;
			const bool nz = (c_act || c_end) && xn != 0u;
			first = (nz && first == XL_W) ? p : first;
			last = nz ? p : last;
		}
		const bool wide = run && re_e >= XL_W && (h1 | f) != 0;
		const int m = key < 0 ? 0 : key >> 8, mj = key < 0 ? -1 : base + (key & 255);
		bool stop = false;
		if (run) {
			const int jfin = beg < end ? end : beg;
			if (jfin == qlen) { max_ie = gscore > h1 ? max_ie : i; gscore = gscore > h1 ? gscore : h1; }
			stop = m == 0;
			if (!stop) {
				if (m > max) {
					max = m; max_i = i; max_j = mj;
					int off = mj - i; off = off < 0 ? -off : off;
					max_off = max_off > off ? max_off : off;
				} else if (zdrop > 0) {
					if (i - max_i > mj - max_j) stop = max - m - ((i - max_i) - (mj - max_j)) * e_del > zdrop;
					else stop = max - m - ((mj - max_j) - (i - max_i)) * e_ins > zdrop;
				}
			}
			if (!stop) {
				int nb = first < XL_W ? base + first : end;
				int lastc = last >= 0 ? base + last : nb - 1;
				lastc = lastc > nb - 1 ? lastc : nb - 1;
				beg = nb;
				end = lastc + 2 < qlen ? lastc + 2 : qlen;
				++i;
				if (i >= tlen) stop = true;
				else if (yleft == 0) st = XL_REFILL;
			}
			if (stop) st = XL_AFTER;
			if (wide) st = XL_BAIL;
		}
		while (__ballot((st == XL_ROW || st == XL_REFILL) && beg - base >= 16)) {
			const bool sh = (st == XL_ROW || st == XL_REFILL) && beg - base >= 16;
			if (sh && base + 16 + XL_W > XL_QCOLS) st = XL_BAIL;
			const bool go = sh && st != XL_BAIL;
#pragma unroll
			for (int p = 0; p < XL_W; ++p) { const uint32_t nx = p + 16 < XL_W ? R[p + 16 < XL_W ? p + 16 : p] : 0u; R[p] = go ? nx : R[p]; }
			base += go ? 16 : 0;
			if (go) XL_QWIN();
			if (sh && !go) base = beg;
		}
	}
	if (prof) {
		const unsigned int r = (unsigned int)wave_sum_i32((int)pf_rows), jb = (unsigned int)wave_sum_i32((int)pf_jobs), bl = (unsigned int)wave_sum_i32((int)pf_bail);
		if (lane == 0) { atomicAdd(&prof[EXTL_JOBS], (unsigned long long)jb); atomicAdd(&prof[EXTL_ROWS], (unsigned long long)r); atomicAdd(&prof[EXTL_TRIPS], (unsigned long long)pf_trips); atomicAdd(&prof[EXTL_COLD], (unsigned long long)pf_cold); atomicAdd(&prof[EXTL_SENT_ON], (unsigned long long)bl); }
	}
}

void launch_extl(hipStream_t st, int n_cu, const DevIndex &ix, const DevScoring &sc, const RegParams &P, const uint8_t *reads, void *jobs, unsigned int jcap,
                 unsigned int *ctr32, unsigned char *xbase, long long n_upper, unsigned long long *prof, unsigned int *rows)
{
	const int wpc = 4 * XL_OCC;
	const int grid = (int)std::max<long long>(1, std::min<long long>((n_upper + 63) / 64, (long long)n_cu * wpc));
	if (rows) hipLaunchKernelGGL((k_extl<true, true>), dim3(grid), dim3(64), 0, st, ix, sc, P, reads, jobs, (void*)rows, jcap, ctr32, xbase, prof);
	else hipLaunchKernelGGL(k_extl<true>, dim3(grid), dim3(64), 0, st, ix, sc, P, reads, jobs, (void*)nullptr, jcap, ctr32, xbase, prof);
}

void launch_extl_batch(hipStream_t st, int n_cu, const DevIndex &ix, const DevScoring &sc, const uint8_t *reads, const bsx_ext_job_t *jobs, bsx_ext_res_t *res,
                       unsigned int n, unsigned int *ctr32)
{
	RegParams P; memset(&P, 0, sizeof(P));
	const int grid = (int)std::max<long long>(1, std::min<long long>(((long long)n + 63) / 64, (long long)n_cu * 4 * XL_OCC));
	hipLaunchKernelGGL(k_extl<false>, dim3(grid), dim3(64), 0, st, ix, sc, P, reads, (void*)jobs, (void*)res, n, ctr32, (unsigned char*)nullptr, (unsigned long long*)nullptr);
}
```

### biscuit_amd/csrc/hip/rg_task.hpp

```cpp
#pragma once
#include "parsort.hpp"
#include "ext_dp.hpp"
#include "ext_pk.hpp"
#include "rgx.hpp"
#include "rg_common.hpp"

__device__ __forceinline__ int rg_seed_conv_test(const DevIndex &ix, long long rb, int ln, const uint8_t *q)
{
	const long long l_pac = ix.l_pac;
	int bad = 0;
	const bool rev = rb >= l_pac;
	const long long f0 = rev ? (l_pac << 1) - rb - ln : rb;
	for (int done = 0; done < ln; ) {
		const long long f = f0 + done;
		unsigned long long w;
		__builtin_memcpy(&w, ix.pac + (f >> 2), 8);
		const int k0 = (int)(f & 3);
		int m = 32 - k0; if (m > ln - done) m = ln - done;
		for (int k = k0; k < k0 + m; ++k) {
			const int b = (int)(w >> (((k >> 2) << 3) + ((~k & 3) << 1))) & 3;
			const int at = done + (k - k0);
			const int i = rev ? ln - 1 - at : at, r = rev ? 3 - b : b, qq = q[i];
			bad |= (r == 3 && qq == 1) || (r == 0 && qq == 2);
		}
// ... 883 lines not shown
							qd = rg.qe - (s_qbeg + s_len); rd = rg.re - (s_rbeg + s_len);
							max_gap = rg_gap(gap, P, (int)(qd < rd ? qd : rd));
							w = max_gap < rg.w ? max_gap : rg.w;
							hit = hit || (qd - rd < w && rd - qd < w);
						}
					}
					const unsigned long long hm = __ballot(hit);
					if (hm) u = base + (int)__builtin_ctzll(hm);
				}
				if (u < nr) {
					bool any = false;
					for (int base = k + 1; base < nl && !any; base += 64) {
						const int i = base + lane;
						bool alt = false;
						if (i < nl && S.srt[i] != 0) {
							const int oo = S.lst[(int)(uint32_t)S.srt[i]];
							const long long t_rbeg = S.s_rbeg[oo]; const int t_qbeg = S.s_qbeg[oo], t_len = S.s_len[oo];
							if (!(t_len < s_len * .95))
								alt = (s_qbeg <= t_qbeg && s_qbeg + s_len - t_qbeg >= s_len >> 2 && t_qbeg - s_qbeg != t_rbeg - s_rbeg) ||
								      (t_qbeg <= s_qbeg && t_qbeg + t_len - s_qbeg >= s_len >> 2 && s_qbeg - t_qbeg != s_rbeg - t_rbeg);
						}
						any = __ballot(alt) != 0;
					}
					if (!any) { ++pf_skip; WAVE_SYNC(); if (lane == 0) S.srt[k] = 0; WAVE_SYNC(); continue; }
				}
				++pf_inl;
				if (win_ok == 0) {
					const int span = (int)(rmax1 - rmax0);
					if (span > 0 && span <= RG_WIN) {
						dev_fetch_window(D.win, ix.pac, l_pac, rmax0, span, lane);
						win_ok = 1;
						WAVE_SYNC();
					} else win_ok = -1;
				}
				bsx_region_t R; memset(&R, 0, sizeof(R));
				int aw0 = P.w, aw1 = P.w;
				const int qe = s_qbeg + s_len;
				R.score = R.truesc = -1; R.rid = rid;
				for (int side = 0; side < 2; ++side) {
					if (side == 0 && s_qbeg == 0) { R.score = R.truesc = s_len * P.a; R.qb = 0; R.rb = s_rbeg; continue; }
					if (side == 1 && qe == l_query) { R.qe = l_query; R.re = s_rbeg + s_len; continue; }
					const int sc0 = R.score, clip = side ? P.pen_clip3 : P.pen_clip5;
					int aw = P.w;
					bsx_ext_res_t res; res.score = -1; res.qle = res.tle = res.gtle = 0; res.gscore = -1; res.max_off = 0;
					bsx_ext_job_t J;
					J.parent = (uint8_t)parent; J.pad = 0; J.end_bonus = clip;
					if (side == 0) { J.qoff = qoff + (uint32_t)s_qbeg - 1; J.qdir = -1; J.qlen = s_qbeg; J.tpos = s_rbeg - 1; J.tdir = -1; J.tlen = (int)(s_rbeg - rmax0); J.h0 = s_len * P.a; }
					else { J.qoff = qoff + (uint32_t)qe; J.qdir = 1; J.qlen = l_query - qe; J.tpos = s_rbeg + s_len; J.tdir = 1; J.tlen = (int)(rmax1 - (s_rbeg + s_len)); J.h0 = sc0; }
					for (int i = 0; i < 2; ++i) {
						const int prev = R.score;
						aw = P.w << i;
						J.w = aw;
						RG_STAGE(6);
						if (J.qlen < 64) res = ext_dp_reg<1>(ix, sc, reads, J, lane, win_ok > 0 ? D.win : nullptr, rmax0, D.q, qoff);
						else if constexpr (PK) {
							if (J.qlen < 128) res = ext_dp_pk<1>(ix, sc, reads, J, lane, win_ok > 0 ? D.win : nullptr, rmax0, D.q, qoff);
							else res = ext_dp_pk<2>(ix, sc, reads, J, lane, win_ok > 0 ? D.win : nullptr, rmax0, D.q, qoff);
						}
						else if (J.qlen < 128) res = ext_dp_reg<2>(ix, sc, reads, J, lane, win_ok > 0 ? D.win : nullptr, rmax0, D.q, qoff);
						else res = ext_dp_reg<RG_NC>(ix, sc, reads, J, lane, win_ok > 0 ? D.win : nullptr, rmax0, D.q, qoff);
						res.score = uni(res.score); res.qle = uni(res.qle); res.tle = uni(res.tle); res.gtle = uni(res.gtle);
						res.gscore = uni(res.gscore); res.max_off = uni(res.max_off);
						R.score = res.score;
						RG_STAGE(7);
						++pf_ext; pf_rows += (unsigned int)(res.tle > res.gtle ? res.tle : res.gtle);
						if (P.prof && J.qlen >= 64) RG_PF_ADD(D, 15, (unsigned long long)(res.tle > res.gtle ? res.tle : res.gtle) << (J.qlen >= 128 ? 32 : 0));
						if (R.score == prev || res.max_off < (aw >> 1) + (aw >> 2)) break;
					}
					const int local = res.gscore <= 0 || res.gscore <= R.score - clip;
					if (side == 0) {
						aw0 = aw;
						if (local) { R.qb = s_qbeg - res.qle; R.rb = s_rbeg - res.tle; R.truesc = R.score; }
						else { R.qb = 0; R.rb = s_rbeg - res.gtle; R.truesc = res.gscore; }
					} else {
						aw1 = aw;
						if (local) { R.qe = qe + res.qle; R.re = s_rbeg + s_len + res.tle; R.truesc += R.score - sc0; }
						else { R.qe = l_query; R.re = s_rbeg + s_len + res.gtle; R.truesc += res.gscore - sc0; }
					}
				}
				R.bss = (uint8_t)RG_BSS(parent, l_pac, R.rb); R.parent = (uint8_t)parent;
				if (RG_BSS(parent, l_pac, R.re) != R.bss) continue;
				int cov = 0;
				for (int i = lane; i < nl; i += 64) {
					const int oo = S.lst[i];
					const long long t_rbeg = S.s_rbeg[oo]; const int t_qbeg = S.s_qbeg[oo], t_len = S.s_len[oo];
					if (t_qbeg >= R.qb && t_qbeg + t_len <= R.qe && t_rbeg >= R.rb && t_rbeg + t_len <= R.re) cov += t_len;
				}
				R.seedcov = uni(wave_sum_i32(cov));
				R.w = aw0 > aw1 ? aw0 : aw1; R.seedlen0 = s_len; R.frac_rep = frac_rep;
				if (uni(S.n_regs) == Store::RCAP) return 6;
				WAVE_SYNC();
				if (lane == 0) { S.regs[S.n_regs] = R; ++S.n_regs; }
				WAVE_SYNC();
			}
		}
	}
	RG_STAGE(6);
	if (P.prof) { RG_PF_ADD(D, 8, pf_ext); RG_PF_ADD(D, 9, pf_rows); RG_PF_ADD(D, 11, pf_seen); RG_PF_ADD(D, 12, pf_skip); RG_PF_ADD(D, 14, pf_inl); }
	return 0;
#undef RG_STAGE
}
```

### biscuit_amd/csrc/hip/shim.hip

```cpp
#include <time.h>
#include <atomic>
#include "shim_dev.hpp"
#include "index_build.h"
#include "ext_pk_bound.h"
#include "rgx.hpp"

#include <sys/time.h>
static double bsx_now_s(void) { struct timeval tv; gettimeofday(&tv, 0); return tv.tv_sec + tv.tv_usec * 1e-6; }
#define BSX_DEVICE_SA_INTV_DEFAULT 2
static inline unsigned long long *dev_counters(Lane &L) { return (unsigned long long*)L.small.p; }
static inline CtrShared *ctr_shared(Lane &L) { return (CtrShared*)(dev_counters(L) + CTR_SHARED); }
static inline TierCtr *ctr_tiers(Lane &L, bool main_seq) { return (TierCtr*)(dev_counters(L) + (main_seq ? CTR_MAIN : CTR_SIDE)); }
static inline size_t seed_lane_bytes(long long mem_cap, int list_cap) { return (size_t)mem_cap * 32 + (size_t)list_cap * 16; }

extern "C" BSX_API int bsx_device_open(int ordinal, bsx_device_t **out)
{
	int n = 0;
	*out = nullptr;
	if (hipGetDeviceCount(&n) != hipSuccess || n <= 0) { fprintf(stderr, "[bsx-hip] no HIP device available\n"); return BSX_E_NODEVICE; }
	if (ordinal < 0 || ordinal >= n) return BSX_E_ARG;
	HIPCHK(hipSetDevice(ordinal));
	if (hipSetDeviceFlags(hipDeviceScheduleBlockingSync) != hipSuccess) (void)hipGetLastError();
	bsx_device *d = new bsx_device();
	d->ordinal = ordinal;
	hipDeviceProp_t prop;
	HIPCHK(hipGetDeviceProperties(&prop, ordinal));
	snprintf(d->name, sizeof(d->name), "%s (%s, %d CUs)", prop.name, prop.gcnArchName, prop.multiProcessorCount);
	d->n_cu = prop.multiProcessorCount;
	for (int l = 0; l < BSX_LANES; ++l) {
		Lane &L = d->lane[l];
		int lo = 0, hi = 0;
		HIPCHK(hipDeviceGetStreamPriorityRange(&lo, &hi));
		const int reserve = (int)bsx_tune_long("reserve_cu_every", 0);
		bool masked = false;
		if (reserve >= 2 && d->n_cu >= 16) {
			std::vector<uint32_t> mask((size_t)(d->n_cu + 31) / 32, 0u);
			int n_free = d->n_cu / reserve;
			if (d->n_cu >= 64) n_free = (n_free + 31) / 32 * 32;
			if (n_free >= d->n_cu) n_free = d->n_cu / 2;
			for (int cu = 0; cu < d->n_cu - n_free; ++cu) mask[cu >> 5] |= 1u << (cu & 31);
			masked = hipExtStreamCreateWithCUMask(&L.st, (uint32_t)mask.size(), mask.data()) == hipSuccess &&
			         hipExtStreamCreateWithCUMask(&L.st2, (uint32_t)mask.size(), mask.data()) == hipSuccess &&
			         hipExtStreamCreateWithCUMask(&L.st3, (uint32_t)mask.size(), mask.data()) == hipSuccess;
			if (!masked) { (void)hipGetLastError(); if (L.st) { (void)hipStreamDestroy(L.st); L.st = nullptr; } if (L.st2) { (void)hipStreamDestroy(L.st2); L.st2 = nullptr; } if (L.st3) { (void)hipStreamDestroy(L.st3); L.st3 = nullptr; } }
		}
		if (!masked) {
			HIPCHK(hipStreamCreateWithPriority(&L.st, hipStreamNonBlocking, lo));
			HIPCHK(hipStreamCreateWithPriority(&L.st2, hipStreamNonBlocking, lo));
			HIPCHK(hipStreamCreateWithPriority(&L.st3, hipStreamNonBlocking, lo));
		}
		for (hipEvent_t *e : {&L.ev_timed_begin, &L.ev_timed_end, &L.ev_seed2_begin, &L.ev_seed2_end, &L.ev_occ_end, &L.ev_tier1_end, &L.ev_tiers_end}) HIPCHK(hipEventCreate(e));
		HIPCHK(hipEventCreate(&L.ev_t3a));
		HIPCHK(hipEventCreate(&L.ev_t3b));
		HIPCHK(hipStreamCreateWithPriority(&L.st_hi, hipStreamNonBlocking, hi));
		if (masked && bsx_tune_long("small_copies_unmasked", 1)) { HIPCHK(hipStreamCreateWithPriority(&L.st_cp, hipStreamNonBlocking, hi)); HIPCHK(hipEventCreateWithFlags(&L.ev_cp, hipEventDisableTiming)); }
		HIPCHK(hipEventCreateWithFlags(&L.ev_seed_done, hipEventDisableTiming));
		HIPCHK(hipEventCreateWithFlags(&L.ev_regions_done, hipEventDisableTiming));
// ... 167 lines not shown
	}
	if ((rc = build_seed_tables(d)) != BSX_OK) return rc;
	d->has_index = true;
	return BSX_OK;
}

extern "C" BSX_API int bsx_device_build_index(bsx_device_t *d, bsx_index_t *idx, int fill_host)
{
	if (!d || !idx || !idx->pac || idx->ref.l_pac <= 0) return BSX_E_ARG;
	HIPCHK(hipSetDevice(d->ordinal));
	int rc;
	if ((rc = upload_ref(d, idx)) != BSX_OK) return rc;
	const char *e = bsx_tune_str("device_sa_intv");
	int dense = e ? atoi(e) : BSX_DEVICE_SA_INTV_DEFAULT;
	if (dense < 1 || dense > 32 || (dense & (dense - 1))) dense = BSX_DEVICE_SA_INTV_DEFAULT;
	Lane &L = d->lane[0];
	for (int i = 1; i >= 0; --i) {
		bsx_fmi_t *f = &idx->fmi[i], meta;
		memset(&meta, 0, sizeof(meta));
		free(f->bwt); free(f->sa); f->bwt = nullptr; f->sa = nullptr;
		d->bwt[i].release(); d->sa[i].release();
		const uint64_t n = (uint64_t)idx->ref.l_pac * 2;
		uint32_t *h_bwt = nullptr; uint64_t *h_sa = nullptr;
		if (fill_host) {
			const uint64_t n_occ = (n + 127) / 128 + 1, words = ((n + 15) >> 4) + n_occ * 8, n_sa = (n + 32) / 32;
			h_bwt = (uint32_t*)calloc(words + 16, 4); h_sa = (uint64_t*)calloc(n_sa, 8);
			if (!h_bwt || !h_sa) { free(h_bwt); free(h_sa); return BSX_E_NOMEM; }
		}
		rc = bsx_ix_build_fmi(L.st, d->n_cu, (const uint8_t*)d->pac.p, idx->ref.l_pac, i, dense, 32, &d->bwt[i], &d->sa[i], &meta, h_bwt, h_sa);
		if (rc != BSX_OK) { free(h_bwt); free(h_sa); return rc; }
		launch_bwt_planes(L.st, (uint32_t*)d->bwt[i].p, (unsigned long long)meta.bwt_size);
		HIPCHK(hipStreamSynchronize(L.st));
		*f = meta; f->bwt = h_bwt; f->sa = h_sa;
		DevFmi &g = d->ix.fmi[i];
		g.primary = meta.primary; for (int k = 0; k < 5; ++k) g.L2[k] = meta.L2[k];
		g.seq_len = meta.seq_len; g.bwt = (const uint32_t*)d->bwt[i].p; g.sa = (const uint64_t*)d->sa[i].p;
		g.sa_mask = (uint32_t)dense - 1; g.sa_shift = 0;
		while ((1 << g.sa_shift) < dense) ++g.sa_shift;
	}
	devbuf_drain(d->ordinal);
	if ((rc = build_seed_tables(d)) != BSX_OK) return rc;
	d->has_index = true;
	return BSX_OK;
}

static int lane_set_opt(bsx_device_t *d, int lane, const bsx_opt_t *o)
{
	if (!d || !o) return BSX_E_ARG;
	DevScoring &sc = d->lane[lane].sc;
	memcpy(sc.ctmat, o->ctmat, 25); memcpy(sc.gamat, o->gamat, 25);
	sc.o_del = o->o_del; sc.e_del = o->e_del; sc.o_ins = o->o_ins; sc.e_ins = o->e_ins; sc.zdrop = o->zdrop; sc.a = o->a;
	sc.mx_ct = sc.mx_ga = 0;
	for (int k = 0; k < 25; ++k) { sc.mx_ct = std::max<int>(sc.mx_ct, sc.ctmat[k]); sc.mx_ga = std::max<int>(sc.mx_ga, sc.gamat[k]); }
	return BSX_OK;
}
extern "C" BSX_API int bsx_device_set_opt(bsx_device_t *d, const bsx_opt_t *o) { return lane_set_opt(d, 0, o); }

#define XFER_CHUNK ((size_t)8 << 20)
__global__ void __launch_bounds__(256)
k_patch_lists(const int *which, int n, const long long *off2, const int *cnt2, long long *off, int *cnt)
{
	const int j = blockIdx.x * blockDim.x + threadIdx.x;
	if (j < n) { off[which[j]] = off2[j]; cnt[which[j]] = cnt2[j]; }
}
__global__ void __launch_bounds__(256)
k_copy_bytes(const unsigned char *src, unsigned char *dst, size_t n)
{
	const size_t tid = (size_t)blockIdx.x * blockDim.x + threadIdx.x, nth = (size_t)gridDim.x * blockDim.x;
	if ((((size_t)src | (size_t)dst) & 15) == 0) {
		const size_t n16 = n >> 4;
		for (size_t i = tid; i < n16; i += nth) reinterpret_cast<uint4*>(dst)[i] = reinterpret_cast<const uint4*>(src)[i];
		for (size_t i = (n16 << 4) + tid; i < n; i += nth) dst[i] = src[i];
	} else if ((((size_t)src | (size_t)dst) & 3) == 0) {
		const size_t n4 = n >> 2;
		for (size_t i = tid; i < n4; i += nth) reinterpret_cast<uint32_t*>(dst)[i] = reinterpret_cast<const uint32_t*>(src)[i];
		for (size_t i = (n4 << 2) + tid; i < n; i += nth) dst[i] = src[i];
	} else for (size_t i = tid; i < n; i += nth) dst[i] = src[i];
}
static void copy_by_kernel(hipStream_t st, void *dst, const void *src, size_t n)
{
	const unsigned int blocks = (unsigned int)std::min<size_t>(std::max<size_t>(1, (n / 16 + 255) / 256), 2048);
	hipLaunchKernelGGL(k_copy_bytes, dim3(blocks), dim3(256), 0, st, (const unsigned char*)src, (unsigned char*)dst, n);
}
int xfer(Lane &L, hipStream_t st, void *dst, const void *src, size_t n, bool h2d)
{
	if (n == 0) return BSX_OK;
	const bool zc = st == L.st_hi;
	if (!zc && n < ((size_t)256 << 10)) {
		hipStream_t cs = L.st_cp && (st == L.st || st == L.st2 || st == L.st3) ? L.st_cp : st;
		if (cs != st) { HIPCHK(hipEventRecord(L.ev_cp, st)); HIPCHK(hipStreamWaitEvent(cs, L.ev_cp, 0)); }
		HIPCHK(hipMemcpyAsync(dst, src, n, h2d ? hipMemcpyHostToDevice : hipMemcpyDeviceToHost, cs));
		HIPCHK(hipStreamSynchronize(cs));
		return BSX_OK;
	}
	int rc;
	if ((rc = L.pin.reserve(2 * XFER_CHUNK)) != BSX_OK) return rc;
	char *pin = (char*)L.pin.p;
	size_t off = 0, prev_off = 0, prev_m = 0;
	int i = 0;
	for (; off < n; off += XFER_CHUNK, ++i) {
		const size_t m = std::min(XFER_CHUNK, n - off);
		char *p = pin + (size_t)(i & 1) * XFER_CHUNK;
		if (h2d) {
			if (i >= 2) HIPCHK(hipEventSynchronize(L.pev[i & 1]));
			memcpy(p, (const char*)src + off, m);
			if (zc) copy_by_kernel(st, (char*)dst + off, p, m); else HIPCHK(hipMemcpyAsync((char*)dst + off, p, m, hipMemcpyHostToDevice, st));
// ... 65 lines not shown
	HIPCHK(hipSetDevice(d->ordinal));
	uint64_t tot = 0;
	for (int l = 0; l < BSX_LANES; ++l) {
		static const int at[3] = {CTR_TAB_LOOKUPS, CTR_SEED2 + CTR_TAB_LOOKUPS, CTR_SEED3 + CTR_TAB_LOOKUPS};
		for (int b = 0; b < 3; ++b) {
			uint64_t t = 0;
			HIPCHK(hipMemcpy(&t, dev_counters(d->lane[l]) + at[b], 8, hipMemcpyDeviceToHost));
			tot += t;
			if (reset) HIPCHK(hipMemset(dev_counters(d->lane[l]) + at[b], 0, 8));
		}
	}
	if (lookups) *lookups = tot;
	if (depth) *depth = d->has_index ? d->ix.tab.K : 0;
	return BSX_OK;
}

extern "C" BSX_API int bsx_device_seed_passes(bsx_device_t *d, uint64_t w[6], double ms[2], int reset)
{
	if (!d || !w || !ms) return BSX_E_ARG;
	HIPCHK(hipSetDevice(d->ordinal));
	for (int k = 0; k < 6; ++k) w[k] = 0;
	ms[0] = ms[1] = 0;
	for (int l = 0; l < BSX_LANES; ++l) {
		Lane &L = d->lane[l];
		uint64_t t[2], u = 0;
		unsigned long long *ctr = dev_counters(L);
		HIPCHK(hipMemcpy(t, ctr + CTR_FM_SLOW, 16, hipMemcpyDeviceToHost));
		HIPCHK(hipMemcpy(&u, ctr + CTR_TAB_LOOKUPS, 8, hipMemcpyDeviceToHost));
		w[0] += t[0] + t[1]; w[1] += u;
		HIPCHK(hipMemcpy(t, ctr + CTR_SEED2 + CTR_FM_SLOW, 16, hipMemcpyDeviceToHost));
		HIPCHK(hipMemcpy(&u, ctr + CTR_SEED2 + CTR_TAB_LOOKUPS, 8, hipMemcpyDeviceToHost));
		w[2] += t[0] + t[1]; w[3] += u;
		w[4] += (uint64_t)L.seed2_launches; w[5] += L.seed2_tasks;
		ms[0] += L.k_ms[KT_SEED]; ms[1] += L.seed2_ms;
		if (reset) { L.seed2_ms = 0; L.seed2_launches = 0; L.seed2_tasks = 0; }
	}
	return BSX_OK;
}

static std::atomic<uint64_t> g_ext_forms[2];
static bool ext_pk_wanted(void) { return bsx_tune_long("ext_pk", 1) != 0; }
static bool ext_pk_scoring(const DevScoring &sc, long long hmax, int qmax, bool per_read)
{
	int mn = 0;
	for (int k = 0; k < 25; ++k) mn = std::min<int>(mn, std::min<int>(sc.ctmat[k], sc.gamat[k]));
	const int mx = std::max(sc.mx_ct, sc.mx_ga);
	if (per_read) return ext_pk_exact_reads(sc.a, mx, mn, sc.o_del, sc.e_del, sc.o_ins, sc.e_ins, qmax);
	return ext_pk_exact(mx, mn, sc.o_del, sc.e_del, sc.o_ins, sc.e_ins, hmax, qmax);
}
extern "C" BSX_API int bsx_ext_forms(uint64_t c[2], int reset)
{
	if (!c) return BSX_E_ARG;
	for (int k = 0; k < 2; ++k) { c[k] = g_ext_forms[k].load(); if (reset) g_ext_forms[k].store(0); }
	return BSX_OK;
}

extern "C" BSX_API int bsx_device_region_work(bsx_device_t *d, uint64_t w[5], int reset)
{
	if (!d || !w) return BSX_E_ARG;
	for (int k = 0; k < 5; ++k) w[k] = 0;
	for (int l = 0; l < BSX_LANES; ++l) for (int k = 0; k < 5; ++k) { w[k] += d->lane[l].work[k]; if (reset) d->lane[l].work[k] = 0; }
	return BSX_OK;
}

extern "C" BSX_API int bsx_device_kernel_time(bsx_device_t *d, int k, double *total_ms, int64_t *launches, int reset)
{
	if (!d || k < 0 || k >= KT_N) return BSX_E_ARG;
	double ms = 0; int64_t n = 0;
	for (int l = 0; l < BSX_LANES; ++l) {
		ms += d->lane[l].k_ms[k]; n += d->lane[l].k_launch[k];
		if (reset) { d->lane[l].k_ms[k] = 0; d->lane[l].k_launch[k] = 0; }
	}
	if (total_ms) *total_ms = ms;
	if (launches) *launches = n;
	return BSX_OK;
}

static bool intv_info_lt(const bsx_intv_t &a, const bsx_intv_t &b) { return a.info < b.info; }

struct SeedAsm {
	const long long *off; const int *cnt; const bsx_intv_t *dense;
	const int64_t *redo_of; const std::vector<std::vector<bsx_intv_t>> *redo;
	bsx_intv_t *out; const int64_t *out_off;
};
static void seed_asm_worker(void *data, long i, int tid)
{
	const SeedAsm *A = (const SeedAsm*)data;
	(void)tid;
	bsx_intv_t *dst = A->out + A->out_off[i];
	const int64_t n = A->out_off[i + 1] - A->out_off[i];
	if (n <= 0) return;
	if (A->redo_of && A->redo_of[i] >= 0) std::copy((*A->redo)[A->redo_of[i]].begin(), (*A->redo)[A->redo_of[i]].end(), dst);
	else memcpy(dst, A->dense + A->off[i], sizeof(bsx_intv_t) * (size_t)n);
	if (n > 1) std::sort(dst, dst + n, intv_info_lt);
}

struct SeedPlan {
	int mem_cap, list_cap; bool direct;
	unsigned long long direct_n, dense_cap;
	int quota, trip_budget, budget2_mul, n_slabs, grid;
	size_t scratch_bytes;
};
static SeedPlan seed_plan(const bsx_device_t *d, int64_t n, int max_len)
{
	SeedPlan S;
	S.mem_cap = bsx_tune_is_set("seed_mem_cap") ? std::max(4, (int)bsx_tune_long("seed_mem_cap", 64)) : std::max(64, max_len); S.list_cap = max_len + 2;
// ... 265 lines not shown
	B.seed_direct = SP.direct; B.direct_n = SP.direct_n;
	B.dense_cap = SP.dense_cap; B.regs_cap = (unsigned long long)n * 24 + 65536;
	B.seed_quota = SP.quota; B.trip_budget = SP.trip_budget; B.budget2_mul = SP.budget2_mul;
	B.merge_min = bsx_tune_long("redo_merge_min", 4096);
	B.reg_quota = std::max(1, (int)bsx_tune_long("regions_quota", 16));
	B.n_slabs = SP.n_slabs; B.grid = SP.grid;
	const size_t scratch_bytes = SP.scratch_bytes;
	B.big_grid = d->n_cu * 3; B.huge_grid = d->n_cu * std::max(1, std::min(3, (int)bsx_tune_long("tier3_wgs", 2)));
	B.order3 = bsx_tune_long("tier3_order", 1) != 0;
	B.c2rh_grid = d->n_cu * 5;
	B.chain = (int)bsx_tune_long("chain_stages", 3);
	B.use_mid = (int)bsx_tune_long("regions_mid", 1);
	B.mid_quota = std::max(1, (int)bsx_tune_long("mid_quota", 8));
	B.c2r_quota = std::max(1, (int)bsx_tune_long("c2r_quota", 16));
	B.use_1c = bsx_tune_long("tier1c", 1) != 0;
	B.tier2_export = (int)bsx_tune_long("tier2_export", 0);
	B.trace = bsx_phases() != 0; B.trace_tiers = B.trace || bsx_tune_long("tiers", 0) != 0; B.per_tier = bsx_phases() == 2;
	B.early3 = bsx_tune_long("tier3_early", 1) != 0 && !B.export_all && !B.long_reads && bsx_phases() != 2 && L.st3;
	TRY(L.scratch.reserve(scratch_bytes));
	TRY(L.jobs.reserve((size_t)n * sizeof(bsx_seed_task_t)));
	TRY(L.out.reserve((size_t)B.dense_cap * sizeof(DevIntv)));
	TRY(L.aux.reserve((size_t)n * 12 + 64));
	TRY(L.qpack.reserve(seedt_pack_bytes(n)));
	TRY(L.regs.reserve((size_t)B.regs_cap * sizeof(bsx_region_t)));
	TRY(L.regmeta.reserve((size_t)n * 49 + 64));
	TRY(L.c2rslab.reserve(std::max((size_t)B.c2rh_grid * c2r_hbm_slab_bytes(false), B.export_all ? (size_t)d->n_cu * 2 * c2r_hbm_slab_bytes(true) : (size_t)0)));
	TRY(L.slabs.reserve((size_t)B.big_grid * 6 * regions_slab_bytes(2)));
	TRY(L.slabs3.reserve((size_t)B.huge_grid * 4 * regions_slab_bytes(3)));
	B.pos_cap = bsx_tune_is_set("pos_cap") ? strtoull(bsx_tune_str("pos_cap"), 0, 10) : (unsigned long long)n * 384 * lf + (1u << 20);
	TRY(L.pos.reserve((size_t)B.pos_cap * 8));
	TRY(L.posoff.reserve((size_t)n * 8 + 64));
	B.xcap = (unsigned long long)n * 2560 * lf + (64u << 20);
	TRY(L.xpool.reserve(B.trace ? (size_t)rgx_rows_offset(B.xcap) + rgx_rows_bytes(B.xcap) : (size_t)B.xcap));
	TRY(L.xmeta.reserve((size_t)n * 12 + 64));
	B.use_x4 = (int)bsx_tune_long("x4", 1);
	B.x4_cap = (unsigned long long)n * 12 * lf + (1u << 20);
	if (B.use_x4 && !B.export_all) TRY(L.x4jobs.reserve((size_t)B.x4_cap * x4_job_bytes()));
	B.ssw_cap = !B.any_flt ? 0 : bsx_tune_is_set("ssw_cap") ? std::max(8ull, strtoull(bsx_tune_str("ssw_cap"), 0, 10))
	                                   : std::min<unsigned long long>((unsigned long long)n * 24 * lf + (1u << 20), 0x3ffffff0ull);
	if (B.any_flt) TRY(L.sswjobs.reserve((size_t)B.ssw_cap * seedsw_job_bytes()));

	TierSeq &M = B.main;
	M.st = L.st; M.main_seq = true; M.c = ctr_tiers(L, true);
	Bump lists(L.aux), meta(L.regmeta), xmeta(L.xmeta), posoff(L.posoff);
	seq_carve(M, (size_t)n, lists, meta, xmeta, posoff);
	B.retry_e = meta.take<int>((size_t)n);
	if (!lists.ok() || !meta.ok() || !xmeta.ok() || !posoff.ok()) return BSX_E_INTERNAL;
	CtrShared *SH = ctr_shared(L);
	RgLaunch &G = M.G;
	G.ix = &d->ix; G.sc = &L.sc; G.P = &B.R; G.reads = (const uint8_t*)L.reads.p; G.tasks = (const bsx_seed_task_t*)L.jobs.p;
	G.seeds_dense = (const DevIntv*)L.out.p;
	G.out = (bsx_region_t*)L.regs.p; G.out_cap = B.regs_cap; G.out_cursor = &SH->region_cursor;
	G.counters = dev_counters(L); G.pos = (unsigned long long*)L.pos.p;
	G.ext_pk = !B.long_reads && ext_pk_wanted() && ext_pk_scoring(L.sc, 0, B.max_len, true);
	++g_ext_forms[G.ext_pk ? 0 : 1];
	M.X.base = (unsigned char*)L.xpool.p; M.X.cap = B.xcap; M.X.cursor = &SH->xpool_cursor; M.X.xcount = &M.c->front.x_count;
	M.X.ext = B.use_x4 && !B.export_all ? 1 : 0;
	M.X.rows = B.trace && M.X.ext ? (unsigned int*)((unsigned char*)L.xpool.p + rgx_rows_offset(B.xcap)) : nullptr;
	return BSX_OK;
}

static int rg_seed_first(RgBatch &B)
{
	Lane &L = B.L; bsx_device_t *d = B.d; const int64_t n = B.n; TierSeq &M = B.main;
	CtrShared *SH = ctr_shared(L); unsigned long long *ctr = dev_counters(L);
	L.rb_tasks = n;
	L.ddl.valid = false;
	H2D(L.st, L.jobs.p, B.tasks, (size_t)n * sizeof(bsx_seed_task_t));
	HIPCHK(hipMemsetAsync(SH, 0, offsetof(CtrShared, early3), L.st));
	HIPCHK(hipMemsetAsync(&M.c->front, 0, sizeof(M.c->front), L.st));
	HIPCHK(hipMemsetAsync(&SH->early3, 0, sizeof(SH->early3), L.st));
	HIPCHK(hipMemsetAsync(ctr + CTR_OVERFLOW, 0, 8, L.st));
	HIPCHK(hipMemsetAsync(&M.c->late, 0, sizeof(M.c->late), L.st));
	HIPCHK(hipMemsetD32Async((hipDeviceptr_t)&SH->seed.intv_cursor, (int)(uint32_t)B.direct_n, 1, L.st));
	HIPCHK(hipMemsetD32Async((hipDeviceptr_t)((uint32_t*)&SH->seed.intv_cursor + 1), (int)(uint32_t)(B.direct_n >> 32), 1, L.st));
	if (B.chain >= 1) {
		std::lock_guard<std::mutex> g(d->chain_mu);
		if (d->chain_seed && d->chain_seed != L.ev_seed_done) HIPCHK(hipStreamWaitEvent(L.st, d->chain_seed, 0));
		if (B.chain >= 4 && d->chain_regions && d->chain_regions != L.ev_regions_done) HIPCHK(hipStreamWaitEvent(L.st, d->chain_regions, 0));
	}
	HIPCHK(hipEventRecord(L.ev_timed_begin, L.st));
	launch_seed(L.st, B.grid, d->ix, M.G.reads, M.G.tasks, (int)n, B.P,
	            (DevIntv*)L.scratch.p, B.list_cap, B.mem_cap, (DevIntv*)L.out.p, B.dense_cap, &SH->seed.intv_cursor, M.offs, M.cnts,
	            &SH->seed.task_cursor, ctr, B.seed_quota, (unsigned int*)L.slabflags.p, B.n_slabs, B.trip_budget, B.R.prof, (uint32_t*)L.qpack.p, B.seed_direct ? 0ull : ~0ull);
	HIPCHK(hipEventRecord(L.ev_timed_end, L.st));
	if (B.chain >= 1) {
		std::lock_guard<std::mutex> g(d->chain_mu);
		HIPCHK(hipEventRecord(L.ev_seed_done, L.st));
		d->chain_seed = L.ev_seed_done;
	}
	return BSX_OK;
}

static int rg_seed_merged(RgBatch &B)
{
	Lane &L = B.L; bsx_device_t *d = B.d; const int64_t n = B.n; TierSeq &M = B.main;
	CtrShared *SH = ctr_shared(L); unsigned long long *ctr = dev_counters(L);
	unsigned long long n_over = 0;
	const bool may_merge = B.merge_min >= 0 && B.merge_min <= (long)n;
	if (may_merge && (L.last_overflow < 0 || L.last_overflow >= B.merge_min / 4)) {
		HIPCHK(hipEventSynchronize(L.ev_timed_end));
		D2H(L.st, &n_over, ctr + CTR_OVERFLOW, 8);
		L.last_overflow = (long)n_over;
	}
	if (may_merge && (long)n_over >= B.merge_min) {
		B.first_n.resize((size_t)n);
// ... 296 lines not shown
	L.k_ms[KT_SEED] += ms0; L.k_launch[KT_SEED] += 1; L.k_ms[KT_TIER1] += ms1; L.k_launch[KT_TIER1] += 1; L.k_ms[KT_TIERS_LATER] += ms2; L.k_launch[KT_TIERS_LATER] += 1;
	HIPCHK(hipGetLastError());
	return BSX_OK;
}

static int rg_download(RgBatch &B, bsx_region_t **out, int64_t *out_cap, int64_t *out_off, int32_t *out_n)
{
	Lane &L = B.L; const int64_t n = B.n; TierSeq &M = B.main; CtrShared *SH = ctr_shared(L);
	unsigned long long used = 0;
	std::vector<long long> h_off((size_t)n);
	D2H(L.st, h_off.data(), M.G.reg_off, (size_t)n * 8);
	D2H(L.st, out_n, M.G.reg_n, (size_t)n * 4);
	D2H(L.st, &used, &SH->region_cursor, 8);
	if (used > B.regs_cap) used = B.regs_cap;
	{
		unsigned long long n_occ = 0;
		D2H(L.st, &n_occ, &SH->k3_cursor, 8);
		L.work[0] += (uint64_t)n; L.work[2] += n_occ < B.pos_cap ? n_occ : B.pos_cap; L.work[3] += used;
		for (int64_t i = 0; i < n; ++i) L.work[4] += (uint64_t)(B.tasks[i].len > 0 ? B.tasks[i].len : 0);
	}
	for (int64_t i = 0; i < n; ++i) out_off[i] = h_off[i];
	L.rs.used_main = used; L.rs.regs_cap = B.regs_cap;
	for (size_t j = 0; j < B.redo.size(); ++j) out_n[B.redo[j]] = BSX_REGIONS_PENDING;
	if (*out_cap < (int64_t)used + 65536) { *out_cap = (int64_t)used + 65536; *out = (bsx_region_t*)realloc(*out, sizeof(bsx_region_t) * (size_t)*out_cap); }
	D2H(L.st, *out, L.regs.p, (size_t)used * sizeof(bsx_region_t));
	B.used = used;
	return BSX_OK;
}

static int rg_report(RgBatch &B)
{
	Lane &L = B.L; unsigned long long *ctr = dev_counters(L);
	CtrShared sh; TierCtr tc;
	D2H(L.st, &tc, B.main.c, sizeof(tc));
	D2H(L.st, &sh, ctr_shared(L), sizeof(sh));
	const TierCtr::Front &f = tc.front;
	fprintf(stderr, "[M::regions_batch] %lld strand searches: %llu intervals, %llu occurrences looked up ahead | left tier 1: %u, left tier 1b: %u, reached tier 2: %u, left tier 2: %u | second chains -> regions launch: %u | every tier exports: %d\n",
	        (long long)B.n, sh.seed.intv_cursor, sh.k3_cursor, f.ra_count, f.rm_count, B.long_reads || B.export_all ? f.rl_count : f.rl_count ? f.rl_count : f.rm_count, f.rb_count, f.rc_count, B.export_all ? 1 : 0);
	unsigned long long sp[CTR_SEED_N];
	D2H(L.st, sp, ctr + CTR_SEED_CYC, sizeof(sp));
	HIPCHK(hipMemsetAsync(ctr + CTR_SEED_CYC, 0, sizeof(sp), L.st));
	if (sp[0]) fprintf(stderr, "[M::regions_batch] k_seed: %.0f M wave cycles, %.1f%% in the full machine (%llu passes, %.0f cycles each), publishing %.1f%% | %llu wave trips, %.0f cycles per trip\n",
	                   sp[0] * 1e-6, 100.0 * sp[1] / sp[0], sp[4], sp[4] ? (double)sp[1] / sp[4] : 0.0, 100.0 * sp[2] / sp[0], sp[3], sp[3] ? (double)sp[0] / sp[3] : 0.0);
	unsigned long long tq[CTR_SEEDT_N];
	D2H(L.st, tq, ctr + CTR_SEEDT_HOT, sizeof(tq));
	HIPCHK(hipMemsetAsync(ctr + CTR_SEEDT_HOT, 0, sizeof(tq), L.st));
	if (sp[0] && tq[3]) fprintf(stderr, "[M::regions_batch] k_seedt: short machine %.1f%%, fetch %.1f%%, post %.1f%% of the wave cycles | %.1f requests per wave trip\n",
	                            100.0 * tq[0] / sp[0], 100.0 * tq[1] / sp[0], 100.0 * tq[2] / sp[0], sp[3] ? (double)tq[3] / sp[3] : 0.0);
	unsigned long long xp[CTR_EXT_N];
	D2H(L.st, xp, ctr + CTR_EXT, sizeof(xp));
	HIPCHK(hipMemsetAsync(ctr + CTR_EXT, 0, sizeof(xp), L.st));
	if (xp[EXT4_JOBS] || xp[EXTL_JOBS]) fprintf(stderr, "[M::regions_batch] k_ext4: %llu jobs, %llu rows in %llu wave trips (%.2f rows per trip), %llu passes between extensions, %.2f slots per trip, %llu rows of narrow jobs\n", xp[0], xp[1], xp[2], xp[2] ? (double)xp[1] / xp[2] : 0.0, xp[3], xp[2] ? (double)xp[4] / xp[2] : 0.0, xp[5]);
	if (xp[EXTL_JOBS]) fprintf(stderr, "[M::regions_batch] k_extl: %llu jobs (%llu sent on to k_ext4), %llu rows in %llu wave trips (%.1f rows per trip), %llu passes between extensions\n", xp[6], xp[10], xp[7], xp[8], xp[8] ? (double)xp[7] / xp[8] : 0.0, xp[9]);
	unsigned long long xw[CTR_X4W_N];
	D2H(L.st, xw, ctr + CTR_X4W, sizeof(xw));
	HIPCHK(hipMemsetAsync(ctr + CTR_X4W, 0, sizeof(xw), L.st));
	if (xp[EXT4_JOBS] || xp[EXTL_JOBS]) for (int k = 0; k < 2; ++k)
		fprintf(stderr, "[M::regions_batch] %s: unread jobs %llu with %llu rows (%.3f%% of the kernel's rows) | of which inside the strand search's first region: %llu jobs, %llu rows (%.4f%%)\n",
		        k ? "k_extl" : "k_ext4", xw[4 * k + X4W_JOBS], xw[4 * k + X4W_ROWS], xp[k ? EXTL_ROWS : EXT4_ROWS] ? 100.0 * xw[4 * k + X4W_ROWS] / xp[k ? EXTL_ROWS : EXT4_ROWS] : 0.0,
		        xw[4 * k + X4W_JOBS_R0], xw[4 * k + X4W_ROWS_R0], xp[k ? EXTL_ROWS : EXT4_ROWS] ? 100.0 * xw[4 * k + X4W_ROWS_R0] / xp[k ? EXTL_ROWS : EXT4_ROWS] : 0.0);
	unsigned long long pf[CTR_STAGE_N];
	D2H(L.st, pf, ctr + CTR_STAGE, sizeof(pf));
	HIPCHK(hipMemsetAsync(ctr + CTR_STAGE, 0, sizeof(pf), L.st));
	double tot = 0; for (int k = 0; k < 8; ++k) tot += (double)pf[k];
	if (tot > 0) fprintf(stderr, "[M::regions_batch] wave cycles by stage (all tiers): intervals %.1f%% occurrences %.1f%% chaining %.1f%% weights+order %.1f%% sort %.1f%% filter %.1f%% chain prologues+seed tests %.1f%% extension %.1f%% | %.0f M cycles, %llu extensions, %llu rows\n",
	        100 * pf[0] / tot, 100 * pf[1] / tot, 100 * pf[2] / tot, 100 * pf[3] / tot, 100 * pf[4] / tot, 100 * pf[5] / tot, 100 * pf[6] / tot, 100 * pf[7] / tot, tot * 1e-6, pf[8], pf[9]);
	if (pf[10]) fprintf(stderr, "[M::regions_batch] seed filter: %llu alignments\n", pf[10]);
	if (pf[11]) fprintf(stderr, "[M::regions_batch] seed loops (mem_chain2region1): %llu seeds reached, %llu skipped as contained, %llu took the extension made ahead, %llu extended in place\n", pf[11], pf[12], pf[13], pf[14]);
	unsigned long long tk[2 * CTR_TIER_TIME_N];
	D2H(L.st, tk, ctr + CTR_TIER2_TIME, sizeof(tk));
	HIPCHK(hipMemsetAsync(ctr + CTR_TIER2_TIME, 0, sizeof(tk), L.st));
	for (int k = 0; k < 2; ++k) if (tk[4 * k + 2])
		fprintf(stderr, "[M::regions_batch] tier %d: %llu strand searches, %.2f M cycles each on average, the longest %.1f M, the busiest wave %.1f M, all of them %.0f M\n",
		        2 + k, tk[4 * k + 2], 1e-6 * tk[4 * k + 1] / tk[4 * k + 2], 1e-6 * tk[4 * k], 1e-6 * tk[4 * k + 3], 1e-6 * tk[4 * k + 1]);
	unsigned long long th[CTR_T3_N];
	D2H(L.st, th, ctr + CTR_T3_LONGEST, sizeof(th));
	HIPCHK(hipMemsetAsync(ctr + CTR_T3_LONGEST, 0, sizeof(th), L.st));
	if (th[0]) {
		fprintf(stderr, "[M::regions_batch] tier 3: the longest strand search: %.1f M cycles, %llu intervals, %llu chains kept, %llu regions | strand searches by duration, < 2^k x 65536 cycles:",
		        (double)(th[0] >> 36) * 4096e-6, (th[0] >> 24) & 4095, (th[0] >> 14) & 16383, th[0] & 16383);
		for (int k = 0; k < CTR_T3_HIST_N; ++k) if (th[2 + k]) fprintf(stderr, " k=%d: %llu |", k, th[2 + k]);
		fprintf(stderr, "\n");
	}
	return BSX_OK;
}

static int rg_declined(RgBatch &B, const int32_t *out_n, bsx_intv_t **decl_intv, int64_t *decl_cap, int64_t *decl_off)
{
	Lane &L = B.L; const int64_t n = B.n; TierSeq &M = B.main;
	std::vector<int64_t> decl;
	for (int64_t i = 0; i < n; ++i) if (out_n[i] < -1 && out_n[i] != BSX_REGIONS_PENDING) decl.push_back(i);
	decl_off[0] = 0;
	if (decl.empty()) return BSX_OK;
	std::vector<long long> s_off((size_t)n); std::vector<int> s_n((size_t)n);
	D2H(L.st, s_off.data(), M.offs, (size_t)n * 8);
	D2H(L.st, s_n.data(), M.cnts, (size_t)n * 4);
	int64_t tot = 0;
	for (size_t j = 0; j < decl.size(); ++j) { decl_off[j] = tot; tot += s_n[decl[j]]; }
	decl_off[decl.size()] = tot;
	if (*decl_cap < tot) { *decl_cap = tot + (tot >> 2) + 16; *decl_intv = (bsx_intv_t*)realloc(*decl_intv, sizeof(bsx_intv_t) * (size_t)*decl_cap); }
	const bsx_intv_t *dense = nullptr;
	if (decl.size() > 256 && tot > 0) {
		std::vector<long long> which(decl.begin(), decl.end()), doff(decl_off, decl_off + decl.size());
		for (size_t j = 0; j < decl.size(); ++j) if (s_n[decl[j]] < 0) { which.clear(); break; }
		if (!which.empty()) {
			const size_t nb = decl.size() * 8;
// ... 82 lines not shown
		bool any = false;
		for (size_t j = 0; j < n2 && !any; ++j) any = rn[j] > 0;
		if (any) { stretch.resize((size_t)(hi - lo)); D2H(L.st2, stretch.data(), (const bsx_region_t*)L.regs.p + lo, sizeof(bsx_region_t) * (size_t)(hi - lo)); }
	}
	long hist[16] = {0};
	for (size_t j = 0; j < n2; ++j) {
		const int64_t i = L.rs.tasks[j];
		if (rn[j] < 0) { out_n[i] = -1; out_off[i] = 0; ++hist[(-rn[j]) & 15]; continue; }
		if (*out_cap < used + rn[j]) { *out_cap = used + rn[j] + 1024 + (*out_cap >> 2); *out = (bsx_region_t*)realloc(*out, sizeof(bsx_region_t) * (size_t)*out_cap); }
		if (rn[j] > 0) {
			if (!stretch.empty() && (unsigned long long)roff[j] >= lo && (unsigned long long)roff[j] + (unsigned long long)rn[j] <= hi)
				memcpy(*out + used, stretch.data() + ((unsigned long long)roff[j] - lo), sizeof(bsx_region_t) * (size_t)rn[j]);
			else D2H(L.st2, *out + used, (const bsx_region_t*)L.regs.p + roff[j], sizeof(bsx_region_t) * (size_t)rn[j]);
		}
		out_off[i] = used; out_n[i] = rn[j];
		used += rn[j];
	}
	if (bsx_phases()) {
		fprintf(stderr, "[M::regions_finish] left to the caller after the second pass, by reason:");
		for (int k = 1; k < 16; ++k) if (hist[k]) fprintf(stderr, " %d: %ld", k, hist[k]);
		fprintf(stderr, "\n");
	}
	L.rs.active = false;
	return BSX_OK;
}

static int lane_sa_batch(bsx_device_t *d, int lane, int64_t n, const bsx_sa_job_t *jobs, uint64_t *pos)
{
	if (!d || !d->has_index) return BSX_E_NODEVICE;
	Lane &L = d->lane[lane];
	if (n == 0) return BSX_OK;
	HIPCHK(hipSetDevice(d->ordinal));
	int rc;
	if ((rc = L.jobs.reserve((size_t)n * sizeof(bsx_sa_job_t))) != BSX_OK) return rc;
	if ((rc = L.res.reserve((size_t)n * 8)) != BSX_OK) return rc;
	HIPCHK(hipMemcpyAsync(L.jobs.p, jobs, (size_t)n * sizeof(bsx_sa_job_t), hipMemcpyHostToDevice, L.st));
	int grid = (int)std::min<int64_t>((n + 255) / 256, (int64_t)d->n_cu * 8);
	HIPCHK(hipEventRecord(L.ev_timed_begin, L.st));
	launch_sa(L.st, grid, d->ix, (const bsx_sa_job_t*)L.jobs.p, (long long)n, (uint64_t*)L.res.p, dev_counters(L));
	HIPCHK(hipEventRecord(L.ev_timed_end, L.st));
	if ((rc = finish_timed(L, KT_K3)) != BSX_OK) return rc;
	D2H(L.st, pos, L.res.p, (size_t)n * 8);
	return BSX_OK;
}

static int lane_extend_batch(bsx_device_t *d, int lane, int64_t n, const bsx_ext_job_t *jobs, bsx_ext_res_t *res)
{
	if (!d || !d->has_index) return BSX_E_NODEVICE;
	Lane &L = d->lane[lane];
	if (n == 0) return BSX_OK;
	HIPCHK(hipSetDevice(d->ordinal));
	if (bsx_tune_is_set("ext4")) {
		int rc, max_q = 0;
		for (int64_t i = 0; i < n; ++i) max_q = std::max(max_q, jobs[i].qlen);
		if ((max_q > x4_max_query(16) && bsx_tune_long("ext4", 0) != 3) || n > 0x7fffffff) return BSX_E_ARG;
		if (bsx_tune_long("ext4", 0) == 4) {
			long long hmax = 0;
			for (int64_t i = 0; i < n; ++i) hmax = std::max(hmax, (long long)jobs[i].h0 + (long long)jobs[i].qlen * (jobs[i].parent ? L.sc.mx_ct : L.sc.mx_ga));
			const bool packed = ext_pk_wanted() && ext_pk_scoring(L.sc, hmax, max_q, false);
			if ((rc = L.jobs.reserve((size_t)n * sizeof(bsx_ext_job_t))) != BSX_OK) return rc;
			if ((rc = L.res.reserve((size_t)n * sizeof(bsx_ext_res_t))) != BSX_OK) return rc;
			HIPCHK(hipMemcpyAsync(L.jobs.p, jobs, (size_t)n * sizeof(bsx_ext_job_t), hipMemcpyHostToDevice, L.st));
			launch_extpk_batch(L.st, d->n_cu, d->ix, L.sc, (const uint8_t*)L.reads.p, (const bsx_ext_job_t*)L.jobs.p, (bsx_ext_res_t*)L.res.p, (long long)n, packed);
			++g_ext_forms[packed ? 0 : 1];
			HIPCHK(hipGetLastError());
			D2H(L.st, res, L.res.p, (size_t)n * sizeof(bsx_ext_res_t));
			for (int64_t i = 0; i < n; ++i) if (res[i].score == X4_DECLINED) return BSX_E_ARG;
			return BSX_OK;
		}
		if ((rc = L.jobs.reserve((size_t)n * sizeof(bsx_ext_job_t))) != BSX_OK) return rc;
		if ((rc = L.res.reserve((size_t)n * sizeof(bsx_ext_res_t))) != BSX_OK) return rc;
		if ((rc = L.aux.reserve(64)) != BSX_OK) return rc;
		HIPCHK(hipMemcpyAsync(L.jobs.p, jobs, (size_t)n * sizeof(bsx_ext_job_t), hipMemcpyHostToDevice, L.st));
		HIPCHK(hipMemsetAsync(L.aux.p, 0, 64, L.st));
		if (bsx_tune_long("ext4", 0) != 3) launch_ext4_batch(L.st, d->n_cu, d->ix, L.sc, (const uint8_t*)L.reads.p, (const bsx_ext_job_t*)L.jobs.p, (bsx_ext_res_t*)L.res.p, (unsigned int)n, (unsigned int*)L.aux.p, max_q);
		if (bsx_tune_long("ext4", 0) == 3) {
			launch_extwin_batch(L.st, d->n_cu, d->ix, L.sc, (const uint8_t*)L.reads.p, (const bsx_ext_job_t*)L.jobs.p, (bsx_ext_res_t*)L.res.p, (long long)n);
		} else
		if (bsx_tune_long("ext4", 0) == 2) {
			HIPCHK(hipMemsetAsync(L.aux.p, 0, 64, L.st));
			launch_extl_batch(L.st, d->n_cu, d->ix, L.sc, (const uint8_t*)L.reads.p, (const bsx_ext_job_t*)L.jobs.p, (bsx_ext_res_t*)L.res.p, (unsigned int)n, (unsigned int*)L.aux.p);
			unsigned int c[4]; D2H(L.st, c, L.aux.p, 16);
			fprintf(stderr, "[M::extl] %lld jobs, %u left to k_ext4\n", (long long)n, c[0]);
		}
		HIPCHK(hipGetLastError());
		D2H(L.st, res, L.res.p, (size_t)n * sizeof(bsx_ext_res_t));
		for (int64_t i = 0; i < n; ++i) if (res[i].score == X4_DECLINED) return BSX_E_ARG;
		return BSX_OK;
	}
	const int hp_hi = 0;
	hipStream_t S = hp_hi ? L.st_hi : L.st;
	static const int QCAP[4] = {256, 1024, 16384, 0x7fffffff}, BAND[4] = {256, 512, 2048, 2048}, NCS[4] = {4, 8, 32, 32};
	std::vector<int> order[4];
	int hbm_qmax = 0, rc0;
	for (int64_t i = 0; i < n; ++i) {
		const bsx_ext_job_t &j = jobs[i];
		if (j.qlen <= 0 || j.tlen < 0 || j.h0 <= 0) { fprintf(stderr, "[bsx-hip] extend job %lld: invalid (qlen=%d tlen=%d h0=%d)\n", (long long)i, j.qlen, j.tlen, j.h0); return BSX_E_ARG; }
		long long band = std::min<long long>(j.qlen, 2LL * j.w + 1);
		int c = 0;
		while (c < 4 && (j.qlen > QCAP[c] || band > BAND[c])) ++c;
		if (c == 4) { fprintf(stderr, "[bsx-hip] extend job %lld: a band of %lld columns is beyond the kernel's 2048 (-w above 511)\n", (long long)i, band); return BSX_E_ARG; }
		if (c == 3) hbm_qmax = std::max(hbm_qmax, j.qlen);
		order[c].push_back((int)i);
	}
	const int hbm_blocks = order[3].empty() ? 0 : (int)std::max<size_t>(1, std::min<size_t>(std::min<size_t>((order[3].size() + 3) / 4, (size_t)d->n_cu), ((size_t)2 << 30) / (4 * extend_hbm_row_bytes(hbm_qmax))));
	if (hbm_blocks && (rc0 = L.scratch.reserve((size_t)hbm_blocks * 4 * extend_hbm_row_bytes(hbm_qmax))) != BSX_OK) return rc0;
	int rc;
	if ((rc = L.jobs.reserve((size_t)n * sizeof(bsx_ext_job_t))) != BSX_OK) return rc;
	if ((rc = L.res.reserve((size_t)n * sizeof(bsx_ext_res_t))) != BSX_OK) return rc;
	if ((rc = L.aux.reserve((size_t)n * 4 + 64)) != BSX_OK) return rc;
	HIPCHK(hipMemcpyAsync(L.jobs.p, jobs, (size_t)n * sizeof(bsx_ext_job_t), hipMemcpyHostToDevice, S));
	size_t off = 0;
	for (int c = 0; c < 4; ++c) if (!order[c].empty()) {
		HIPCHK(hipMemcpyAsync((int*)L.aux.p + off, order[c].data(), order[c].size() * 4, hipMemcpyHostToDevice, S));
		off += order[c].size();
	}
	HIPCHK(hipEventRecord(L.ev_timed_begin, S));
	off = 0;
	for (int c = 0; c < 4; ++c) if (!order[c].empty()) {
		if (c == 3)
			launch_extend_hbm(S, d->ix, L.sc, (const uint8_t*)L.reads.p, (const bsx_ext_job_t*)L.jobs.p, (const int*)L.aux.p + off,
			                  (long long)order[c].size(), (bsx_ext_res_t*)L.res.p, hbm_qmax, hbm_blocks, L.scratch.p);
		else
		launch_extend(S, d->ix, L.sc, (const uint8_t*)L.reads.p, (const bsx_ext_job_t*)L.jobs.p, (const int*)L.aux.p + off,
		              (long long)order[c].size(), (bsx_ext_res_t*)L.res.p, QCAP[c], NCS[c], d->n_cu);
		off += order[c].size();
	}
	HIPCHK(hipEventRecord(L.ev_timed_end, S));
	if ((rc = finish_timed(L, KT_EXTEND)) != BSX_OK) return rc;
	D2H(S, res, L.res.p, (size_t)n * sizeof(bsx_ext_res_t));
	return BSX_OK;
}

static int lane_sw_batch(bsx_device_t *d, int lane, int64_t n, const bsx_sw_job_t *jobs, bsx_sw_res_t *res)
{
	if (!d || !d->has_index) return BSX_E_NODEVICE;
	Lane &L = d->lane[lane];
	if (n == 0) return BSX_OK;
	std::lock_guard<std::mutex> hi_lock(L.hi_mu);
// ... 395 lines not shown
```

### biscuit_amd/csrc/hip/shim_dev.hpp

```cpp
#pragma once
#include <hip/hip_runtime.h>
#include <stdio.h>
#include <stdlib.h>
#include <string.h>
#include <algorithm>
#include <vector>
#include <mutex>
#include "devbuf.hpp"
#include "kernels.h"
#include "tune.h"

#define HIPCHK(x) do { hipError_t e_ = (x); if (e_ != hipSuccess) { fprintf(stderr, "[bsx-hip] %s failed: %s (%s:%d)\n", #x, hipGetErrorString(e_), __FILE__, __LINE__); return BSX_E_NODEVICE; } } while (0)
#define TRY(x) do { int rc_ = (x); if (rc_ != BSX_OK) return rc_; } while (0)

#define BSX_LANES 6
enum KTime { KT_SEED = 0, KT_K3 = 1, KT_EXTEND = 2, KT_SW = 3, KT_GLOBAL = 4, KT_TIER1 = 5, KT_TIERS_LATER = 6, KT_SEED_OTHER = 7, KT_N = 8 };
struct Lane {
	hipStream_t st = nullptr;
	hipEvent_t ev_seed_done = nullptr, ev_regions_done = nullptr;
	hipStream_t st_hi = nullptr;
	hipEvent_t ev_timed_begin = nullptr, ev_timed_end = nullptr;
	hipEvent_t ev_seed2_begin = nullptr, ev_seed2_end = nullptr;
	hipEvent_t ev_occ_end = nullptr, ev_tier1_end = nullptr, ev_tiers_end = nullptr;
	hipEvent_t tier_ev[12] = {};
	hipStream_t st_cp = nullptr;
	hipEvent_t ev_cp = nullptr;
	hipStream_t st3 = nullptr;
	hipEvent_t ev_t3a = nullptr, ev_t3b = nullptr;
	hipStream_t st2 = nullptr;
	DevScoring sc;
	DevBuf reads; size_t n_reads = 0;
	DevBuf gath;
	DevBuf qpack;
	int64_t rb_tasks = 0;
	int flt_key[3] = {-1, -1, -1};
	DevBuf fltab, jobs, res, scratch, scratch2, out, aux, pool, regs, regmeta, slabs, slabs3, slabflags, redo, pos, posoff, xpool, xmeta, x4jobs, tags, mdpool, gctx, qcjobs, qcpool, mdkeys, mdres, mdslot, dd, sswjobs, c2rslab;
	DevBuf small;
	HostBuf hstage;
	HostBuf pin;
	hipEvent_t pev[2] = {nullptr, nullptr};
	struct {
		bool active = false;
		std::vector<int64_t> tasks;
		std::vector<bsx_seed_task_t> sub;
		unsigned int n2u = 0;
		HostBuf hres;
		hipEvent_t ev = nullptr, ev_tiers = nullptr;
		unsigned long long used_main = 0;
		unsigned long long regs_cap = 0;
	} rs;
	double k_ms[KT_N] = {0, 0, 0, 0, 0, 0, 0, 0};
	int64_t k_launch[KT_N] = {0, 0, 0, 0, 0, 0, 0, 0};
	uint64_t work[5] = {0, 0, 0, 0, 0};
	struct { bool valid = false; int64_t n_reads = 0; int per_read = 0; size_t o_idx = 0, o_off = 0, o_pool = 0; bool with_long = false; } ddl;
	DevBuf msw_jobs, msw_res, msw_meta, msw_roff; int64_t msw_token = -1;
	std::mutex hi_mu;
	long last_overflow = -1;
	double seed2_ms = 0; int64_t seed2_launches = 0; uint64_t seed2_tasks = 0;
	void release_buffers()
	{
		DevBuf *b[] = {&reads, &gath, &qpack, &fltab, &jobs, &res, &scratch, &scratch2, &out, &aux, &pool, &regs, &regmeta, &slabs, &slabs3, &slabflags, &redo, &pos, &posoff, &xpool, &xmeta,
		               &x4jobs, &tags, &mdpool, &gctx, &qcjobs, &qcpool, &mdkeys, &mdres, &mdslot, &dd, &sswjobs, &c2rslab, &small, &msw_jobs, &msw_res, &msw_meta, &msw_roff};
		for (DevBuf *x : b) x->release();
		hstage.release(); pin.release(); flt_key[0] = -1;
	}
};

static inline void dev_free(void *p) { if (p) (void)hipFree(p); }
static inline void stream_release(hipStream_t &st) { if (st) (void)hipStreamDestroy(st); st = nullptr; }
struct QcState {
	DevBuf counts; std::mutex mu;
	void release() { counts.release(); }
};
struct CovState {
	void *diff = nullptr; uint32_t *mask[2] = {nullptr, nullptr}; std::mutex mu;
	void release() { dev_free(diff); dev_free(mask[0]); dev_free(mask[1]); diff = nullptr; mask[0] = mask[1] = nullptr; }
};
struct MethState {
	void *st = nullptr; std::mutex mu;
	void release() { dev_free(st); st = nullptr; }
};
struct MarkdupState {
	MdSlot *tab = nullptr; uint64_t slots = 0, used = 0; std::mutex mu;
	void release() { dev_free(tab); tab = nullptr; slots = used = 0; }
};
struct SortState {
	std::vector<std::pair<uint64_t*, int64_t>> runs;
	hipStream_t st = nullptr;
	DevBuf k[2], p[2], counts, btot;
	std::mutex mu;
	void release() { for (auto &r : runs) dev_free(r.first); runs.clear(); for (DevBuf *x : {&k[0], &k[1], &p[0], &p[1], &counts, &btot}) x->release(); stream_release(st); }
};
struct BamState {
	hipStream_t st = nullptr;
	uint64_t tab_serial = 0;
	DevBuf names, noff, nid, text, cnt, start, size, bad, pay, err;
	DevBuf bz_in, bz_tok, bz_cand, bz_slots, bz_sizes, bz_out, bz_ops; bool bz_ops_ok = false;
	std::mutex mu;
	void release()
	{
		for (DevBuf *x : {&names, &noff, &nid, &text, &cnt, &start, &size, &bad, &pay, &err, &bz_in, &bz_tok, &bz_cand, &bz_slots, &bz_sizes, &bz_out, &bz_ops}) x->release();
		tab_serial = 0; bz_ops_ok = false; stream_release(st);
	}
};

struct bsx_device {
	int ordinal = 0;
	char name[256];
	int n_cu = 0;
	DevIndex ix; bool has_index = false;
	DevBuf bwt[2], sa[2], pac, ctg, holes, seedtab[2];
	QcState qc; CovState cov; MethState meth; MarkdupState md; SortState sort; BamState bam;
	Lane lane[BSX_LANES];
	std::mutex chain_mu;
	hipEvent_t chain_seed = nullptr, chain_regions = nullptr;
// ... 10 lines not shown
```

### biscuit_amd/csrc/host/tune.c

```c
#include <pthread.h>
#include "bsx_core.h"
#include "tune.h"

typedef struct { const char *name, *doc; char *val; } knob_t;
static knob_t g_knobs[] = {
	{"phases", "[0] 1: per-phase lines on stderr and the kernels' cycle counters; 2: the stage counters read after every region launch (also $BSX_PHASES)", 0},
	{"tiers", "[0] 1: HIP events between the region launches of a chunk, printed (no cycle counters): bench.py's stand-alone chunk", 0},
	{"seed_form", "[table] classic: seeding without the table of k-mer intervals (k_seed.hip: the reference's own sequence of bwt_extend calls, what counts its FM-block touches)", 0},
	{"seed_tab_k", "[from the text's size: 18 at 3.1 Gbp] levels of the table of k-mer intervals; 0: none", 0},
	{"seed_mem_cap", "[max(64, longest read)] entries of a strand search's first-pass interval list (tests: short lists, so that ordinary reads are seeded again)", 0},
	{"seed_direct", "[1] 0: interval lists copied behind each other instead of written where they stay", 0},
	{"seed_batch_form", "[batch] chunk: bsx_seed_batch launches as the chunk-wide seeding pass of bsx_regions_batch does (its list length, lists written where they stay, budget, quota, grid and slabs; what is left seeded again with lists eight times as long) -- tests: the production launch, list for list", 0},
	{"seed_quota", "[0 = persistent lanes; 1 for seed_form=classic] strand searches a lane of the seeding kernel takes", 0},
	{"tier3_early", "[1] the last HBM tier's launch for what is known to need it when the occurrences are counted: on a stream of its own beside the other tiers; 0: behind them", 0},
	{"tier3_order", "[1] the last HBM tier takes its strand searches longest first (by occurrences to visit); 0: in the order the tier before handed them on", 0},
	{"tier3_wgs", "[2] workgroups of four waves per CU in the last HBM tier's launch (1..3)", 0},
	{"seed_budget2", "[8] the second seeding pass's budget in first-pass budgets; what exceeds it is seeded a third time on the side stream, without one", 0},
	{"seed_trip_budget", "[4096] FM extensions (per 256 bases of read) after which the first seeding pass hands a strand search to the second; 0: never", 0},
	{"redo_merge_min", "[4096] from how many overflowed strand searches the second seeding pass runs inside the chunk's launch sequence (1: always; negative or huge: never)", 0},
	{"async_redo", "[0] 1: bsx_process_seqs collects the strand searches seeded again on the side stream only in the back half", 0},
	{"device_sa_intv", "[2] the device's suffix-array sample: every n-th rank (a power of two up to the files' 32)", 0},
	{"pos_cap", "[384 per strand search] seed occurrences the chunk-wide position table holds (tests: strand searches that find no room)", 0},
	{"ssw_cap", "[24 per strand search] jobs the seed filter's chunk-wide list holds (tests: seeds that find no room)", 0},
	{"regions_quota", "[16] strand searches per wave of the first region tier", 0},
	{"mid_quota", "[8] strand searches per wave of the larger LDS tiers", 0},
	{"c2r_quota", "[16] strand searches per wave of the chains -> regions launch", 0},
	{"regions_occ", "[5] waves per SIMD the first region tier's register allocation targets (3..5)", 0},
	{"regions_mid", "[1] 0: no second LDS tier", 0},
	{"tier1c", "[1] 0: no third LDS tier / second chains -> regions launch for ordinary reads (the tier sequence of rounds 2-4)", 0},
	{"x4", "[1] 0: every extension inline in the chains -> regions loop (no k_x4prep / k_extl / k_ext4 ahead of it)", 0},
	{"xl", "[1] 0: the narrow extension jobs through k_ext4 as well (no lane-per-job kernel)", 0},
	{"ext_win", "[1] chunks with long reads: an extension's rows in five register slots that follow the band (ext_dp_win); 0: in LDS (the form of rounds 3-5)", 0},
	{"ext4", "[off] tests: bsx_extend_batch through the quarter-wave kernel (1) / then the lane-per-job kernel (2) of the regions path / through the wavefront-per-job form with a register window (3) / with the rows of the region kernels' inline extensions, packed 16-bit when the batch allows (4)", 0},
	{"sw_form", "[off] tests: bsx_sw_batch through the seed filter's alignments, score only, jobs of up to 199 x 199 in the order given -- ssw16: the packed 16-bit kernel (k_swl16), sixteen consecutive jobs to a wavefront, qlen = 0 an empty job; scoring options it cannot hold fail the call / ssw32: a wavefront per job through the 32-bit alignment of a seed without room in the job list", 0},
	{"ext_pk", "[1] extension rows of 64 columns and more in packed 16-bit, two columns per lane (ext_pk.hpp), where the scoring options keep every intermediate inside 16 bits; 0: always the 32-bit rows", 0},
	{"chain_stages", "[3] how consecutive chunks' front halves are chained on the device: 0 none, 1 seeding, 2 seeding and regions, 3 the same but the HBM tiers hold nobody back, 4 strictly one after the other", 0},
	{"small_copies_unmasked", "[1] the front half's copies of less than 256 KB go through the lane's unmasked stream (the CUs the front-half streams leave alone); 0: through the stream they are ordered on", 0},
	{"reserve_cu_every", "[0] n >= 2: the front-half streams leave one compute unit in n (of every shader engine of every XCD) to the back half's short batches; < 2: none", 0},
	{"host_chain", "[0] 1: every strand search chained on the host over the batch kernels (A/B against the region kernels)", 0},
	{"host_dedup", "[0] 1: mem_sort_deduplicate of every read on the host (A/B against k_dedup)", 0},
	{"stream_whole_chunk", "[0] N: a chunk's own thread runs its back half too, at most N at a time", 0},
	{"no_chunk_scan", "[0] 1 (several ranks): no boundary scan of plain input files, every rank parses everything", 0},
	{"no_chunk_skip", "[0] 1 (several ranks): the other ranks' chunks are parsed into records and dropped instead of walked", 0},
	{"index_batch", "[256 M] suffixes per batch of the device index builder's first round", 0},
	{"back_slices", "[4] slices the pairs of a chunk are cut into for the stages after the insert-size statistics (mate rescue .. SAM text); 1: the stages over the whole chunk", 0},
	{"back_threads", "[2] threads that take those slices alternately (one waits for its slice's K5 / K6 batch while the other runs host stages); up to 4", 0},
	{"shard_pairs", "[0] several ranks (RANK / WORLD_SIZE): 1 = every rank aligns its slice of EVERY chunk (inputs with fewer chunks than GPUs) instead of every world-th chunk", 0},
	{"gather_via_rank0", "[0] several ranks with $BSX_OUT: 1 = the records go through rank 0 even where every rank could write its own chunks into the file", 0},
	{"gather_transport", "[rccl] several ranks: socket = Unix-domain sockets through rank 0 instead of RCCL", 0},
	{"tier2_export", "[0] the first HBM tier of the region kernels in steps -- chains exported, seeds extended ahead (k_extl / k_ext4; 1: every chain's best seed, 2: every seed of every main list), the seed loop by a chains -> regions launch with its regions in HBM -- instead of its monolithic form (same SAM; measured no faster, DESIGN.md section 4)", 0},
	{"msw_plan", "[0] 1: mate rescue's plan pass (which candidates need an alignment, over which window) by k_msw_plan over the lists on the device, its K5 batch run from device memory, instead of by the host's first replay pass (same SAM; measured slower, DESIGN.md section 4)", 0},
	{"long_dedup", "[1] 0: reads with more than 32 regions are de-duplicated on the host (A/B against k_dedup_long)", 0},
	{"markdup_slots", "[32 per key of the first batch, at least 65536] slots of the first table of template keys (--markdup), a power of two; it doubles before a batch would load it beyond one half", 0},
	{"cov_lds_bins", "[512] depths below this are counted in a workgroup's LDS histograms by the coverage tables' last pass (--qc-cov), deeper ones in HBM directly; a power of two up to 512", 0},
	{"meth_flush_tiles", "[1024] tests: tiles after which a wave of the base-averaged conversion table's pass (--qc-meth) adds its sums to the 64-bit cells (32-bit registers: at most 1024)", 0},
	{"cov_flush_tiles", "[524287] tests: tiles after which a workgroup of that pass adds its LDS histograms to the bins (32-bit cells: at most 2^32 / 4096 - 1)", 0},
	{"sort_buf_bytes", "[1 GB / runs, at most 8 MB] bytes of the buffer every sorted run of --sort is read back through in the final merge (tests: 1, a record is then many fills)", 0},
	{"bam_piece_bytes", "[32 MB] bytes of SAM text (whole lines; a longer line alone) the writer of --bam encodes and deflates at a time: the file does not depend on it (tests: small pieces, so that records and block_size fields straddle pieces and blocks)", 0},
	{"markdup_hash_bits", "[64] tests: low bits kept of a template key's claim word (different keys then meet in one slot and take the next salt)", 0},
};
#define N_KNOBS ((int)(sizeof(g_knobs) / sizeof(g_knobs[0])))
static pthread_mutex_t g_mu = PTHREAD_MUTEX_INITIALIZER;
static int g_env_done = 0, g_phases_env = -1;

static int find(const char *name)
{
	int i;
	for (i = 0; i < N_KNOBS; ++i) if (strcmp(g_knobs[i].name, name) == 0) return i;
	return -1;
}

static void set_locked(int i, const char *value, size_t len)
{
	free(g_knobs[i].val);
	g_knobs[i].val = 0;
	if (value) { g_knobs[i].val = (char*)malloc(len + 1); memcpy(g_knobs[i].val, value, len); g_knobs[i].val[len] = 0; }
}

static void env_locked(void)
{
	const char *e, *p;
	if (g_env_done) return;
	g_env_done = 1;
	e = getenv("BSX_TUNE");
	for (p = e; p && *p; ) {
		const char *q = strchr(p, ','), *eq;
		size_t n = q ? (size_t)(q - p) : strlen(p);
		char name[64];
// ... 50 lines not shown
```

### include/bsx.h

```cpp
#ifndef BSX_H
#define BSX_H

#include <stdint.h>
#include <stddef.h>
#include <stdio.h>

#ifdef __cplusplus
extern "C" {
#endif

#define BSX_EXPORT __attribute__((visibility("default")))

#define BSX_OK            0
#define BSX_E_NODEVICE  (-1)
#define BSX_E_ARG       (-2)
#define BSX_E_IO        (-3)
#define BSX_E_NOMEM     (-4)
#define BSX_E_FORMAT    (-5)
#define BSX_E_INTERNAL  (-6)

#define BSX_F_PE             0x2
#define BSX_F_NOPAIRING      0x4
#define BSX_F_ALL            0x8
#define BSX_F_NO_MULTI       0x10
// ... 292 lines not shown
int bsx_sort_schedule(bsx_device_t *dev, int64_t *n_total, uint32_t **run_of);
int bsx_sort_info(bsx_device_t *dev, uint64_t *n_runs, uint64_t *n_keys);
int bsx_sort_reset(bsx_device_t *dev);

typedef struct bsx_sorter bsx_sorter_t;
int  bsx_sorter_dir_ok(const char *tmp_dir);
int  bsx_sorter_open(bsx_device_t *dev, const char *header, const char *tmp_dir, bsx_sorter_t **out);
int  bsx_sorter_add(bsx_sorter_t *s, const char *text, size_t len);
int  bsx_sorter_finish(bsx_sorter_t *s, int (*sink)(void *ud, const char *text, size_t len), void *ud);
void bsx_sorter_counts(const bsx_sorter_t *s, uint64_t *n_runs, uint64_t *n_records);
void bsx_sorter_close(bsx_sorter_t *s);
char *bsx_sort_header(const char *header);

#define BSX_BGZF_BLOCK   0xff00
#define BSX_BAM_E_LINE   1
#define BSX_BAM_E_TAG    2
#define BSX_BAM_E_INT    3
#define BSX_BAM_E_NAME   4
#define BSX_BAM_E_CIGAR  5
#define BSX_BAM_E_REF    6
#define BSX_BAM_E_QUAL   7
typedef struct bsx_bam_refs bsx_bam_refs_t;
typedef struct bsx_bam_writer bsx_bam_writer_t;
typedef int (*bsx_bam_sink_fn)(void *ud, const void *data, size_t len, int is_header);
int  bsx_bam_refs_open(const char *header_text, bsx_bam_refs_t **out);
void bsx_bam_refs_close(bsx_bam_refs_t *refs);
int  bsx_bam_header(const char *header_text, uint8_t **out, size_t *out_len);
const char *bsx_bam_strerror(int why);
int  bsx_bam_encode(bsx_device_t *dev, const bsx_bam_refs_t *refs, const char *text, size_t len, uint8_t **out, size_t *out_cap, size_t *out_len,
                    int64_t *n_records, int64_t *bad_record, int *bad_why);
int  bsx_bgzf_deflate(bsx_device_t *dev, const uint8_t *payload, size_t len, uint8_t **out, size_t *out_cap, size_t *out_len);
int  bsx_bam_writer_open(bsx_device_t *dev, const char *header_text, bsx_bam_sink_fn sink, void *ud, bsx_bam_writer_t **out);
int  bsx_bam_writer_add(bsx_bam_writer_t *w, const char *text, size_t len);
int  bsx_bam_writer_close(bsx_bam_writer_t *w, int finish);
void bsx_bam_writer_refused(const bsx_bam_writer_t *w, int64_t *record, int *why);
void bsx_bam_writer_counts(const bsx_bam_writer_t *w, uint64_t *n_records, uint64_t *payload_bytes, uint64_t *bytes_written);

int bsx_tune_set(const char *name, const char *value);
const char *bsx_tune_str(const char *name);
long bsx_tune_long(const char *name, long dflt);
int bsx_tune_is_set(const char *name);
int bsx_phases(void);
const char *bsx_tune_name(int i);
const char *bsx_tune_doc(int i);

int bsx_device_counters(bsx_device_t *dev, uint64_t c[4], int reset);
int bsx_device_seed_passes(bsx_device_t *dev, uint64_t w[6], double ms[2], int reset);
extern void (*bsx_pes_hist_hook)(void *ud, int64_t *hist, int n_bins);
extern void *bsx_pes_hist_ud;
void bsx_pestat_sync_empty(const bsx_opt_t *opt);
void bsx_chunk_slice_offset(int64_t first);
int bsx_device_region_work(bsx_device_t *dev, uint64_t w[5], int reset);
int bsx_ext_forms(uint64_t c[2], int reset);
int bsx_device_seed_table(bsx_device_t *dev, uint64_t *lookups, int *depth, int reset);
int bsx_device_kernel_time(bsx_device_t *dev, int k, double *total_ms, int64_t *launches, int reset);

typedef struct bsx_transport {
	void *ctx;
	int rank, world;
	int (*all_gather)(void *ctx, const int64_t *mine, int n, int64_t *all);
	int (*send)(void *ctx, int dst, const void *buf, size_t n_bytes);
	int (*recv_many)(void *ctx, int n_src, const int *src, void *const *buf, const size_t *n_bytes);
	int (*all_reduce_sum)(void *ctx, int64_t *buf, int n);
	void (*close)(void *ctx);
} bsx_transport_t;
int bsx_transport_local(int world, bsx_transport_t *out);
int bsx_transport_rccl(int rank, int world, int device, const char *id_path, bsx_transport_t *gather, bsx_transport_t *reduce);
int bsx_transport_socket(int rank, int world, const char *path, bsx_transport_t *gather, bsx_transport_t *reduce);
typedef struct bsx_gather bsx_gather_t;
int bsx_gather_open(const bsx_transport_t *tr, const char *direct_path, void (*sink)(void *ud, int64_t chunk, const void *buf, size_t n), void *ud,
                    int max_pending, bsx_gather_t **out);
int bsx_gather_set_header(bsx_gather_t *g, const void *hdr, size_t n);
int bsx_gather_submit(bsx_gather_t *g, int64_t chunk, void *buf, size_t n);
int bsx_gather_close_input(bsx_gather_t *g);
int bsx_gather_run(bsx_gather_t *g, int64_t *n_chunks);
void bsx_gather_stats(const bsx_gather_t *g, int64_t out[3]);
void bsx_gather_free(bsx_gather_t *g);
int bsx_gather_direct_ok(const char *path, int world, int local_world);

int bsx_process_seqs(bsx_device_t *dev, const bsx_opt_t *opt, const bsx_index_t *idx,
                     int64_t n_processed, int n, bsx_read_t *reads, const bsx_pestat_t *pes0);

typedef struct bsx_stream bsx_stream_t;
int  bsx_stream_open(bsx_device_t *dev, const bsx_opt_t *opt, const bsx_index_t *idx, const bsx_pestat_t *pes0, bsx_stream_t **out);
int  bsx_stream_depth(const bsx_stream_t *s);
int  bsx_stream_push(bsx_stream_t *s, int64_t n_processed, int n, bsx_read_t *reads);
int  bsx_stream_flush(bsx_stream_t *s);
void bsx_stream_close(bsx_stream_t *s);

typedef struct bsx_bsconv_conf {
	int annotate;
	int filter_u;
	int show_filtered;
	int max_cph, max_cpa, max_cpc, max_cpt, max_cpy;
	float max_cph_frac, max_cpy_frac;
} bsx_bsconv_conf_t;
void bsx_bsconv_conf_init(bsx_bsconv_conf_t *conf);
int  bsx_stream_set_bsconv(bsx_stream_t *s, const bsx_bsconv_conf_t *conf);
int  bsx_stream_bsconv_totals(const bsx_stream_t *s, uint64_t out[8], uint64_t *n, uint64_t *n_filtered);
int  bsx_process_set_bsconv(const bsx_bsconv_conf_t *conf);
int  bsx_process_bsconv_totals(uint64_t out[8], uint64_t *n, uint64_t *n_filtered, int reset);

#define BSX_QC_N_MAPQ 61
#define BSX_QC_ISIZE  1000
typedef struct bsx_qc_totals {
	bsx_qc_counts_t dev;
// ... 57 lines not shown
```

Before: 706,900.

## Stop extension DP early once remaining rows cannot change any result

Adds an early-termination rule to the banded extension kernels (reg, packed, ext4, extl, c2r). After each row where the row max is below the global score, it computes a wave-wide upper bound on what any remaining cell could still reach and ends the extension if that bound cannot beat gscore. This is meant to skip DP rows that cannot alter the result fields, in exchange for an extra per-row reduction and, when tracing, atomic counters. The rule defaults to on through a tune knob.

```diff
diff --git a/biscuit_amd/csrc/hip/dev_common.hpp b/biscuit_amd/csrc/hip/dev_common.hpp
--- a/biscuit_amd/csrc/hip/dev_common.hpp
+++ b/biscuit_amd/csrc/hip/dev_common.hpp
@@ -54,6 +54,8 @@
 	int8_t gamat[25];
 	int32_t o_del, e_del, o_ins, e_ins, zdrop, a;
 	int32_t mx_ct, mx_ga;
+	int32_t ext_stop;
+	unsigned long long *xs_ctr;
 };
 
 BSX_HD int dev_ref_base(const uint8_t *pac, int64_t l_pac, int64_t p)
diff --git a/biscuit_amd/csrc/hip/ext_dp.hpp b/biscuit_amd/csrc/hip/ext_dp.hpp
--- a/biscuit_amd/csrc/hip/ext_dp.hpp
+++ b/biscuit_amd/csrc/hip/ext_dp.hpp
@@ -2,6 +2,7 @@
 #include <hip/hip_runtime.h>
 #include "dev_common.hpp"
 #include "wave.hpp"
+#include "ext_stop.hpp"
 
 template <int NC>
 __device__ __forceinline__ bsx_ext_res_t ext_dp(const DevIndex &ix, const DevScoring &sc, const uint8_t *reads, const bsx_ext_job_t &J,
@@ -131,7 +132,7 @@
 	return r;
 }
 
-template <int NC>
+template <int NC, int XS_FAM = -1>
 __device__ __forceinline__ bsx_ext_res_t ext_dp_reg(const DevIndex &ix, const DevScoring &sc, const uint8_t *reads, const bsx_ext_job_t &J, int lane,
                                                     const uint8_t *win = nullptr, long long win_beg = 0, const uint8_t *qlds = nullptr, uint32_t qlds_off = 0)
 {
@@ -165,7 +166,9 @@
 	int beg = 0, end = qlen;
 	int tb_reg = 4;
 	const bool packed_max = qlen <= 512 && (long long)h0 + (long long)qlen * mx < (1 << 21);
+	[[maybe_unused]] bool xs_fired = false;
 	for (int i = 0; i < tlen; ++i) {
+		if constexpr (XS_FAM >= 0) if (xs_fired) ext_stop_dead_row(sc, XS_FAM, lane);
 		if ((i & 63) == 0) {
 			const long long tp = J.tpos + (long long)(i + lane) * J.tdir;
 			tb_reg = (i + lane < tlen) ? (win ? (int)win[tp - win_beg] : dev_ref_base(ix.pac, ix.l_pac, tp)) : 4;
@@ -273,6 +276,11 @@
 			beg = nb;
 			end = last + 2 < qlen ? last + 2 : qlen;
 		}
+		if (ext_stop_gate(m, gscore) && i + 1 < tlen && (XS_FAM >= 0 ? !xs_fired && ext_stop_armed(sc) : sc.ext_stop != 0)) {
+			const int phi = ext_stop_phi_reg<NC>(Hr, Er, beg, qlen, J.parent ? sc.mx_ct : sc.mx_ga, lane);
+			if constexpr (XS_FAM >= 0) { if (ext_stop_decide(sc, XS_FAM, phi, gscore, tlen - 1 - i, lane, xs_fired)) break; }
+			else if (ext_stop_fires(phi, gscore)) break;
+		}
 	}
 	bsx_ext_res_t r;
 	r.score = max; r.qle = max_j + 1; r.tle = max_i + 1; r.gtle = max_ie + 1; r.gscore = gscore; r.max_off = max_off;
diff --git a/biscuit_amd/csrc/hip/ext_pk.hpp b/biscuit_amd/csrc/hip/ext_pk.hpp
--- a/biscuit_amd/csrc/hip/ext_pk.hpp
+++ b/biscuit_amd/csrc/hip/ext_pk.hpp
@@ -3,6 +3,7 @@
 #include "dev_common.hpp"
 #include "wave.hpp"
 #include "ext_pk_bound.h"
+#include "ext_stop.hpp"
 
 typedef short pk2 __attribute__((ext_vector_type(2)));
 __device__ __forceinline__ pk2 pk_of(uint32_t w) { return __builtin_bit_cast(pk2, w); }
@@ -26,7 +27,7 @@
 	return v;
 }
 
-template <int NP>
+template <int NP, int XS_FAM = -1>
 __device__ __forceinline__ bsx_ext_res_t ext_dp_pk(const DevIndex &ix, const DevScoring &sc, const uint8_t *reads, const bsx_ext_job_t &J, int lane,
                                                    const uint8_t *win = nullptr, long long win_beg = 0, const uint8_t *qlds = nullptr, uint32_t qlds_off = 0)
 {
@@ -66,7 +67,9 @@
 	int max = h0, max_i = -1, max_j = -1, max_ie = -1, gscore = -1, max_off = 0;
 	int beg = 0, end = qlen;
 	int tb_reg = 4;
+	[[maybe_unused]] bool xs_fired = false;
 	for (int i = 0; i < tlen; ++i) {
+		if constexpr (XS_FAM >= 0) if (xs_fired) ext_stop_dead_row(sc, XS_FAM, lane);
 		if ((i & 63) == 0) {
 			const long long tp = J.tpos + (long long)(i + lane) * J.tdir;
 			tb_reg = (i + lane < tlen) ? (win ? (int)win[tp - win_beg] : dev_ref_base(ix.pac, ix.l_pac, tp)) : 4;
@@ -162,6 +165,11 @@
 			beg = nb;
 			end = last + 2 < qlen ? last + 2 : qlen;
 		}
+		if (ext_stop_gate(m, gscore) && i + 1 < tlen && (XS_FAM >= 0 ? !xs_fired && ext_stop_armed(sc) : sc.ext_stop != 0)) {
+			const int phi = ext_stop_phi_pk<NP>(Hp, Ep, beg, qlen, J.parent ? sc.mx_ct : sc.mx_ga, lane);
+			if constexpr (XS_FAM >= 0) { if (ext_stop_decide(sc, XS_FAM, phi, gscore, tlen - 1 - i, lane, xs_fired)) break; }
+			else if (ext_stop_fires(phi, gscore)) break;
+		}
 	}
 	bsx_ext_res_t r;
 	r.score = max; r.qle = max_j + 1; r.tle = max_i + 1; r.gtle = max_ie + 1; r.gscore = gscore; r.max_off = max_off;
diff --git a/biscuit_amd/csrc/hip/ext_stop.hpp b/biscuit_amd/csrc/hip/ext_stop.hpp
--- /dev/null
+++ b/biscuit_amd/csrc/hip/ext_stop.hpp
@@ -0,0 +1,60 @@
+#pragma once
+#include <hip/hip_runtime.h>
+#include "dev_common.hpp"
+#include "wave.hpp"
+#include "ext_stop_rule.h"
+
+enum { XS_STOPS = 0,
+       XS_EVALS = 1,
+       XS_LEFT = 2,
+       XS_DEAD = 3,
+       XS_WOULD = 4,
+       XS_N = 5 };
+enum { XS_FAM_EXT4 = 0, XS_FAM_EXTL = 1, XS_FAM_TIER = 2, XS_FAM_C2R = 3, XS_FAM_WAVE = 4, XS_FAM_N = 5 };
+
+template <int NC>
+__device__ __forceinline__ int ext_stop_phi_reg(const int (&Hr)[NC], const int (&Er)[NC], int beg, int qlen, int mx, int lane)
+{
+	int phi = 0;
+#pragma unroll
+	for (int c = 0; c < NC; ++c) {
+		const int a = (c << 6) + lane;
+		const int t = ext_stop_term(Hr[c], Er[c], (qlen - 1 - a) * mx, mx);
+		phi = (a >= beg && a <= qlen && t > phi) ? t : phi;
+	}
+	return wave_max_i32(phi);
+}
+
+template <int NP, typename PK>
+__device__ __forceinline__ int ext_stop_phi_pk(const PK (&Hp)[NP], const PK (&Ep)[NP], int beg, int qlen, int mx, int lane)
+{
+	int phi = 0;
+#pragma unroll
+	for (int p = 0; p < NP; ++p) {
+		const uint32_t hw = __builtin_bit_cast(uint32_t, Hp[p]), ew = __builtin_bit_cast(uint32_t, Ep[p]);
+#pragma unroll
+		for (int u = 0; u < 2; ++u) {
+			const int a = (p << 7) + (u << 6) + lane;
+			const int t = ext_stop_term((int)(u ? hw >> 16 : hw & 0xffffu), (int)(u ? ew >> 16 : ew & 0xffffu), (qlen - 1 - a) * mx, mx);
+			phi = (a >= beg && a <= qlen && t > phi) ? t : phi;
+		}
+	}
+	return wave_max_i32(phi);
+}
+
+__device__ __forceinline__ bool ext_stop_armed(const DevScoring &sc) { return sc.ext_stop != 0 || sc.xs_ctr != nullptr; }
+__device__ __forceinline__ bool ext_stop_decide(const DevScoring &sc, int fam, int phi, int gscore, int rows_left, int lane, bool &fired)
+{
+	const bool fire = ext_stop_fires(phi, gscore);
+	if (sc.xs_ctr && lane == 0) {
+		unsigned long long *c = sc.xs_ctr + XS_N * fam;
+		atomicAdd(&c[XS_EVALS], 1ull);
+		if (fire) { atomicAdd(&c[sc.ext_stop ? XS_STOPS : XS_WOULD], 1ull); atomicAdd(&c[XS_LEFT], (unsigned long long)rows_left); }
+	}
+	fired = fire;
+	return fire && sc.ext_stop != 0;
+}
+__device__ __forceinline__ void ext_stop_dead_row(const DevScoring &sc, int fam, int lane)
+{
+	if (sc.xs_ctr && lane == 0) atomicAdd(&sc.xs_ctr[XS_N * fam + XS_DEAD], 1ull);
+}
diff --git a/biscuit_amd/csrc/hip/ext_stop_rule.h b/biscuit_amd/csrc/hip/ext_stop_rule.h
--- /dev/null
+++ b/biscuit_amd/csrc/hip/ext_stop_rule.h
@@ -0,0 +1,21 @@
+#pragma once
+#if defined(__HIPCC__) || defined(__CUDACC__)
+#define EXT_STOP_HD __host__ __device__
+#else
+#define EXT_STOP_HD
+#endif
+
+EXT_STOP_HD inline int ext_stop_term(int h, int e, int q1mx, int mx)
+{
+	const int ph = h > 0 ? h + q1mx + mx : 0, pe = e > 0 ? e + q1mx : 0;
+	return ph > pe ? ph : pe;
+}
+EXT_STOP_HD inline bool ext_stop_gate(int m, int gscore) { return m < gscore; }
+EXT_STOP_HD inline bool ext_stop_fires(int phi, int gscore) { return phi < gscore; }
+
+EXT_STOP_HD inline int ext_stop_phi(const int *eh_h, const int *eh_e, int beg, int qlen, int mx)
+{
+	int phi = 0;
+	for (int a = beg; a <= qlen; ++a) { const int t = ext_stop_term(eh_h[a], eh_e[a], (qlen - 1 - a) * mx, mx); phi = phi > t ? phi : t; }
+	return phi;
+}
diff --git a/biscuit_amd/csrc/hip/k_c2r.hip b/biscuit_amd/csrc/hip/k_c2r.hip
--- a/biscuit_amd/csrc/hip/k_c2r.hip
+++ b/biscuit_amd/csrc/hip/k_c2r.hip
@@ -216,13 +216,14 @@
 						aw = P.w << i;
 						J.w = aw;
 						if (P.prof) { const long long now_ = (long long)__builtin_readcyclecounter(); RG_PF_ADD(W, 6, now_ - pf_t); pf_t = now_; }
-						if (J.qlen < 64) res = ext_dp_reg<1>(ix, sc, reads, J, lane, win_ok > 0 ? W.win : nullptr, rmax0, W.q, qoff);
+						constexpr int XC = TALLY ? XS_FAM_C2R : -1;
+						if (J.qlen < 64) res = ext_dp_reg<1, XC>(ix, sc, reads, J, lane, win_ok > 0 ? W.win : nullptr, rmax0, W.q, qoff);
 						else if constexpr (PK && WT::QCAP <= 256) {
-							if (J.qlen < 128) res = ext_dp_pk<1>(ix, sc, reads, J, lane, win_ok > 0 ? W.win : nullptr, rmax0, W.q, qoff);
-							else res = ext_dp_pk<2>(ix, sc, reads, J, lane, win_ok > 0 ? W.win : nullptr, rmax0, W.q, qoff);
+							if (J.qlen < 128) res = ext_dp_pk<1, XC>(ix, sc, reads, J, lane, win_ok > 0 ? W.win : nullptr, rmax0, W.q, qoff);
+							else res = ext_dp_pk<2, XC>(ix, sc, reads, J, lane, win_ok > 0 ? W.win : nullptr, rmax0, W.q, qoff);
 						}
-						else if (J.qlen < 128) res = ext_dp_reg<2>(ix, sc, reads, J, lane, win_ok > 0 ? W.win : nullptr, rmax0, W.q, qoff);
-						else if (WT::QCAP <= 256 || J.qlen < 256) res = ext_dp_reg<RG_NC>(ix, sc, reads, J, lane, win_ok > 0 ? W.win : nullptr, rmax0, W.q, qoff);
+						else if (J.qlen < 128) res = ext_dp_reg<2, XC>(ix, sc, reads, J, lane, win_ok > 0 ? W.win : nullptr, rmax0, W.q, qoff);
+						else if (WT::QCAP <= 256 || J.qlen < 256) res = ext_dp_reg<RG_NC, XC>(ix, sc, reads, J, lane, win_ok > 0 ? W.win : nullptr, rmax0, W.q, qoff);
 						else if (P.ext_win && 2 * J.w + 1 <= 256 && (long long)J.h0 + (long long)J.qlen * (parent ? sc.mx_ct : sc.mx_ga) < (1 << 21))
 							res = ext_dp_win<5>(ix, sc, reads, J, lane, win_ok > 0 ? W.win : nullptr, rmax0, W.q, qoff);
 						else if (WT::ROWS && 2 * J.w + 1 <= 512) { WAVE_SYNC(); res = ext_dp<8>(ix, sc, reads, J, W.Hrow, W.Erow, W.qrow, lane); }
diff --git a/biscuit_amd/csrc/hip/k_ext4.hip b/biscuit_amd/csrc/hip/k_ext4.hip
--- a/biscuit_amd/csrc/hip/k_ext4.hip
+++ b/biscuit_amd/csrc/hip/k_ext4.hip
@@ -8,6 +8,7 @@
 #include "tune.h"
 #include "rgx.hpp"
 #include "x4.hpp"
+#include "ext_stop.hpp"
 
 size_t x4_job_bytes(void) { return sizeof(X4Job); }
 
@@ -211,6 +212,10 @@
 	for (int c = 0; c < NCQ; ++c) { Hr[c] = Er[c] = 0; sqp[c] = 0; }
 	unsigned int pf_rows = 0, pf_trips = 0, pf_jobs = 0, pf_cold = 0, pf_slots = 0, pf_nrows = 0;
 	[[maybe_unused]] unsigned int jrows = 0;
+	constexpr bool COUNT = TALLY || !CHAIN;
+	const bool xs_armed = sc.ext_stop != 0 || (COUNT && sc.xs_ctr != nullptr);
+	[[maybe_unused]] bool xs_fired = false;
+	[[maybe_unused]] unsigned int pf_xstop = 0, pf_xeval = 0, pf_xleft = 0, pf_xdead = 0;
 	for (;;) {
 		{
 			const bool cold = st != X4_ROW && st != X4_DONE;
@@ -315,6 +320,7 @@
 							else { if (l == 0) { bsx_ext_res_t r; r.score = X4_DECLINED; r.qle = r.tle = r.gtle = r.gscore = r.max_off = 0; ((bsx_ext_res_t*)res_)[e] = r; } st = X4_IDLE; }
 						} else {
 							max = h0; max_i = max_j = max_ie = -1; gscore = -1; max_off = 0;
+								if constexpr (COUNT) xs_fired = false;
 							beg = 0; end = qlen; i = 0;
 							if (tlen <= 0) st = X4_AFTER;
 							else {
@@ -351,7 +357,7 @@
 		}
 		++pf_trips;
 		const bool run = st == X4_ROW;
-		if (run) { ++pf_rows; if (CHAIN && s_len < X4_NARROW) ++pf_nrows; if constexpr (TALLY) ++jrows; }
+		if (run) { ++pf_rows; if (CHAIN && s_len < X4_NARROW) ++pf_nrows; if constexpr (TALLY) ++jrows; if constexpr (COUNT) pf_xdead += xs_fired ? 1u : 0u; }
 		const int t = (int)(y0 & 3u) ^ tcomp;
 		y0 = __builtin_amdgcn_alignbit(y1, y0, 2); y1 = __builtin_amdgcn_alignbit(y2, y1, 2); y2 >>= 2; --yleft;
 		beg = beg > i - w ? beg : i - w;
@@ -449,7 +455,35 @@
 				else if (yleft == 0) st = X4_REFILL;
 			}
 		}
+		if (xs_armed) {
+			bool gate = shrink && !stop && ext_stop_gate(m, gscore);
+			if constexpr (COUNT) gate = gate && !xs_fired;
+			if (__ballot(gate)) {
+				const int mx = par ? sc.mx_ct : sc.mx_ga;
+				int phi = 0, q1mx = (qlen - 1 - l) * mx, left = beg - l;
+#pragma unroll
+				for (int c = 0; c < NCQ; ++c) {
+					const int tm = ext_stop_term(Hr[c], Er[c], q1mx, mx);
+					phi = ((c << 4) >= left && tm > phi) ? tm : phi;
+					q1mx -= mx << 4;
+				}
+				phi = q_allmax(phi);
+				const bool fire = gate && ext_stop_fires(phi, gscore);
+				if constexpr (COUNT) {
+					if (gate) ++pf_xeval;
+					if (fire) { ++pf_xstop; pf_xleft += (unsigned int)(tlen - i); xs_fired = true; }
+				}
+				if (fire && sc.ext_stop) stop = true;
+			}
+		}
+		if constexpr (COUNT) if (run && stop) xs_fired = false;
 		if (run && stop) st = X4_AFTER;
+	}
+	if constexpr (COUNT) if (sc.xs_ctr) {
+		unsigned long long *xc = sc.xs_ctr + XS_N * XS_FAM_EXT4;
+		const unsigned int a0 = (unsigned int)wave_sum_i32(l == 0 ? (int)pf_xstop : 0), a1 = (unsigned int)wave_sum_i32(l == 0 ? (int)pf_xeval : 0);
+		const unsigned int a2 = (unsigned int)wave_sum_i32(l == 0 ? (int)pf_xleft : 0), a3 = (unsigned int)wave_sum_i32(l == 0 ? (int)pf_xdead : 0);
+		if (lane == 0) { atomicAdd(&xc[sc.ext_stop ? XS_STOPS : XS_WOULD], (unsigned long long)a0); atomicAdd(&xc[XS_EVALS], (unsigned long long)a1); atomicAdd(&xc[XS_LEFT], (unsigned long long)a2); atomicAdd(&xc[XS_DEAD], (unsigned long long)a3); }
 	}
 	if (prof) {
 		pf_rows = (unsigned int)wave_sum_i32(l == 0 ? (int)pf_rows : 0); pf_jobs = (unsigned int)wave_sum_i32(l == 0 ? (int)pf_jobs : 0);
diff --git a/biscuit_amd/csrc/hip/k_extend.hip b/biscuit_amd/csrc/hip/k_extend.hip
--- a/biscuit_amd/csrc/hip/k_extend.hip
+++ b/biscuit_amd/csrc/hip/k_extend.hip
@@ -88,9 +88,9 @@
 		const bsx_ext_job_t J = jobs[jj];
 		bsx_ext_res_t r;
 		if (J.qlen > EXT_PK_QMAX) { r.score = X4_DECLINED; r.qle = r.tle = r.gtle = r.gscore = r.max_off = 0; }
-		else if (!PK) r = ext_dp_reg<4>(ix, sc, reads, J, lane);
-		else if (J.qlen < 128) r = ext_dp_pk<1>(ix, sc, reads, J, lane);
-		else r = ext_dp_pk<2>(ix, sc, reads, J, lane);
+		else if (!PK) r = ext_dp_reg<4, XS_FAM_WAVE>(ix, sc, reads, J, lane);
+		else if (J.qlen < 128) r = ext_dp_pk<1, XS_FAM_WAVE>(ix, sc, reads, J, lane);
+		else r = ext_dp_pk<2, XS_FAM_WAVE>(ix, sc, reads, J, lane);
 		if (lane == 0) res[jj] = r;
 	}
 }
diff --git a/biscuit_amd/csrc/hip/k_extl.hip b/biscuit_amd/csrc/hip/k_extl.hip
--- a/biscuit_amd/csrc/hip/k_extl.hip
+++ b/biscuit_amd/csrc/hip/k_extl.hip
@@ -7,6 +7,7 @@
 #include "kernels.h"
 #include "rgx.hpp"
 #include "x4.hpp"
+#include "ext_stop.hpp"
 
 #define XL_W 64
 #define XL_QCOLS 128
@@ -59,6 +60,10 @@
 	for (int g = 0; g < XL_W / 16; ++g) QW[g] = 0;
 	unsigned int pf_rows = 0, pf_trips = 0, pf_jobs = 0, pf_cold = 0, pf_bail = 0;
 	[[maybe_unused]] unsigned int jrows = 0;
+	constexpr bool COUNT = TALLY || !CHAIN;
+	const bool xs_armed = sc.ext_stop != 0 || (COUNT && sc.xs_ctr != nullptr);
+	[[maybe_unused]] bool xs_fired = false;
+	[[maybe_unused]] unsigned int pf_xstop = 0, pf_xeval = 0, pf_xleft = 0, pf_xdead = 0;
 #define XL_QWIN() do { const int b16_ = base >> 4; _Pragma("unroll") for (int g_ = 0; g_ < XL_W / 16; ++g_) { uint32_t v_ = 0; \
 		_Pragma("unroll") for (int k_ = 0; k_ < XL_QCOLS / 16; ++k_) v_ = b16_ + g_ == k_ ? QF[k_] : v_; QW[g_] = v_; } } while (0)
 	for (;;) {
@@ -175,6 +180,7 @@
 					if (qlen < 0 || h0 < 0 || jmax0 + 2 >= XL_W || (long long)h0 + (long long)qlen * mx >= 32768) st = XL_BAIL;
 					else {
 						max = h0; max_i = max_j = max_ie = -1; gscore = -1; max_off = 0;
+						if constexpr (COUNT) xs_fired = false;
 						beg = 0; end = qlen; i = 0; base = 0;
 						if (tlen <= 0) st = XL_AFTER;
 						else {
@@ -228,7 +234,7 @@
 		}
 		++pf_trips;
 		const bool run = st == XL_ROW;
-		if (run) { ++pf_rows; if constexpr (TALLY) ++jrows; }
+		if (run) { ++pf_rows; if constexpr (TALLY) ++jrows; if constexpr (COUNT) pf_xdead += xs_fired ? 1u : 0u; }
 		const int t = (int)(y0 & 3u) ^ tcomp;
 		y0 = __builtin_amdgcn_alignbit(y1, y0, 2); y1 = __builtin_amdgcn_alignbit(y2, y1, 2); y2 >>= 2; --yleft;
 		beg = beg > i - w ? beg : i - w;
@@ -286,6 +292,31 @@
 				if (i >= tlen) stop = true;
 				else if (yleft == 0) st = XL_REFILL;
 			}
+		}
+		if (xs_armed) {
+			bool gate = run && !stop && !wide && ext_stop_gate(m, gscore);
+			if constexpr (COUNT) gate = gate && !xs_fired;
+			if (__ballot(gate)) {
+				const int mx = par ? sc.mx_ct : sc.mx_ga;
+				const int lo = beg - base, hi = qlen - base;
+				int q1mx = (qlen - 1 - base) * mx, phi = 0;
+#pragma unroll
+				for (int p = 0; p < XL_W; ++p) {
+					const uint32_t x = R[p];
+					const int tm = ext_stop_term((int)(x & 0xffffu), (int)(x >> 16), q1mx, mx);
+					phi = (p >= lo && p <= hi && tm > phi) ? tm : phi;
+					q1mx -= mx;
+				}
+				const bool fire = gate && ext_stop_fires(phi, gscore);
+				if constexpr (COUNT) {
+					if (gate) ++pf_xeval;
+					if (fire) { ++pf_xstop; pf_xleft += (unsigned int)(tlen - i); xs_fired = true; }
+				}
+				if (fire && sc.ext_stop) stop = true;
+			}
+		}
+		if (run) {
+			if constexpr (COUNT) if (stop || wide) xs_fired = false;
 			if (stop) st = XL_AFTER;
 			if (wide) st = XL_BAIL;
 		}
@@ -299,6 +330,12 @@
 			if (go) XL_QWIN();
 			if (sh && !go) base = beg;
 		}
+	}
+	if constexpr (COUNT) if (sc.xs_ctr) {
+		unsigned long long *xc = sc.xs_ctr + XS_N * XS_FAM_EXTL;
+		const unsigned int a0 = (unsigned int)wave_sum_i32((int)pf_xstop), a1 = (unsigned int)wave_sum_i32((int)pf_xeval);
+		const unsigned int a2 = (unsigned int)wave_sum_i32((int)pf_xleft), a3 = (unsigned int)wave_sum_i32((int)pf_xdead);
+		if (lane == 0) { atomicAdd(&xc[sc.ext_stop ? XS_STOPS : XS_WOULD], (unsigned long long)a0); atomicAdd(&xc[XS_EVALS], (unsigned long long)a1); atomicAdd(&xc[XS_LEFT], (unsigned long long)a2); atomicAdd(&xc[XS_DEAD], (unsigned long long)a3); }
 	}
 	if (prof) {
 		const unsigned int r = (unsigned int)wave_sum_i32((int)pf_rows), jb = (unsigned int)wave_sum_i32((int)pf_jobs), bl = (unsigned int)wave_sum_i32((int)pf_bail);
diff --git a/biscuit_amd/csrc/hip/rg_task.hpp b/biscuit_amd/csrc/hip/rg_task.hpp
--- a/biscuit_amd/csrc/hip/rg_task.hpp
+++ b/biscuit_amd/csrc/hip/rg_task.hpp
@@ -959,13 +959,13 @@
 						aw = P.w << i;
 						J.w = aw;
 						RG_STAGE(6);
-						if (J.qlen < 64) res = ext_dp_reg<1>(ix, sc, reads, J, lane, win_ok > 0 ? D.win : nullptr, rmax0, D.q, qoff);
+						if (J.qlen < 64) res = ext_dp_reg<1, XS_FAM_TIER>(ix, sc, reads, J, lane, win_ok > 0 ? D.win : nullptr, rmax0, D.q, qoff);
 						else if constexpr (PK) {
-							if (J.qlen < 128) res = ext_dp_pk<1>(ix, sc, reads, J, lane, win_ok > 0 ? D.win : nullptr, rmax0, D.q, qoff);
-							else res = ext_dp_pk<2>(ix, sc, reads, J, lane, win_ok > 0 ? D.win : nullptr, rmax0, D.q, qoff);
+							if (J.qlen < 128) res = ext_dp_pk<1, XS_FAM_TIER>(ix, sc, reads, J, lane, win_ok > 0 ? D.win : nullptr, rmax0, D.q, qoff);
+							else res = ext_dp_pk<2, XS_FAM_TIER>(ix, sc, reads, J, lane, win_ok > 0 ? D.win : nullptr, rmax0, D.q, qoff);
 						}
-						else if (J.qlen < 128) res = ext_dp_reg<2>(ix, sc, reads, J, lane, win_ok > 0 ? D.win : nullptr, rmax0, D.q, qoff);
-						else res = ext_dp_reg<RG_NC>(ix, sc, reads, J, lane, win_ok > 0 ? D.win : nullptr, rmax0, D.q, qoff);
+						else if (J.qlen < 128) res = ext_dp_reg<2, XS_FAM_TIER>(ix, sc, reads, J, lane, win_ok > 0 ? D.win : nullptr, rmax0, D.q, qoff);
+						else res = ext_dp_reg<RG_NC, XS_FAM_TIER>(ix, sc, reads, J, lane, win_ok > 0 ? D.win : nullptr, rmax0, D.q, qoff);
 						res.score = uni(res.score); res.qle = uni(res.qle); res.tle = uni(res.tle); res.gtle = uni(res.gtle);
 						res.gscore = uni(res.gscore); res.max_off = uni(res.max_off);
 						R.score = res.score;
diff --git a/biscuit_amd/csrc/hip/shim.hip b/biscuit_amd/csrc/hip/shim.hip
--- a/biscuit_amd/csrc/hip/shim.hip
+++ b/biscuit_amd/csrc/hip/shim.hip
@@ -3,6 +3,7 @@
 #include "shim_dev.hpp"
 #include "index_build.h"
 #include "ext_pk_bound.h"
+#include "ext_stop.hpp"
 #include "rgx.hpp"
 
 #include <sys/time.h>
@@ -276,6 +277,7 @@
 	sc.o_del = o->o_del; sc.e_del = o->e_del; sc.o_ins = o->o_ins; sc.e_ins = o->e_ins; sc.zdrop = o->zdrop; sc.a = o->a;
 	sc.mx_ct = sc.mx_ga = 0;
 	for (int k = 0; k < 25; ++k) { sc.mx_ct = std::max<int>(sc.mx_ct, sc.ctmat[k]); sc.mx_ga = std::max<int>(sc.mx_ga, sc.gamat[k]); }
+	sc.ext_stop = 0; sc.xs_ctr = nullptr;
 	return BSX_OK;
 }
 extern "C" BSX_API int bsx_device_set_opt(bsx_device_t *d, const bsx_opt_t *o) { return lane_set_opt(d, 0, o); }
@@ -447,6 +449,38 @@
 {
 	if (!c) return BSX_E_ARG;
 	for (int k = 0; k < 2; ++k) { c[k] = g_ext_forms[k].load(); if (reset) g_ext_forms[k].store(0); }
+	return BSX_OK;
+}
+
+static std::atomic<uint64_t> g_ext_stops[XS_FAM_N * XS_N];
+static int ext_stop_arm(Lane &L, hipStream_t st, bool count)
+{
+	L.sc.ext_stop = bsx_tune_long("ext_stop", 1) != 0 ? 1 : 0;
+	L.sc.xs_ctr = nullptr;
+	if (!count) return BSX_OK;
+	if (!L.xstop.p) {
+		int rc = L.xstop.reserve(sizeof(unsigned long long) * XS_FAM_N * XS_N);
+		if (rc != BSX_OK) return rc;
+		HIPCHK(hipMemsetAsync(L.xstop.p, 0, sizeof(unsigned long long) * XS_FAM_N * XS_N, st));
+	}
+	L.sc.xs_ctr = (unsigned long long*)L.xstop.p;
+	return BSX_OK;
+}
+static int ext_stop_collect(Lane &L, hipStream_t st, unsigned long long *c)
+{
+	unsigned long long h[XS_FAM_N * XS_N] = {0};
+	if (L.xstop.p) {
+		D2H(st, h, L.xstop.p, sizeof(h));
+		HIPCHK(hipMemsetAsync(L.xstop.p, 0, sizeof(h), st));
+	}
+	for (int k = 0; k < XS_FAM_N * XS_N; ++k) { g_ext_stops[k] += h[k]; if (c) c[k] = h[k]; }
+	return BSX_OK;
+}
+extern "C" BSX_API int bsx_ext_stops(uint64_t c[26], int reset)
+{
+	if (!c) return BSX_E_ARG;
+	c[XS_FAM_N * XS_N] = 0;
+	for (int k = 0; k < XS_FAM_N * XS_N; ++k) { c[k] = g_ext_stops[k].load(); if (k % XS_N == XS_STOPS) c[XS_FAM_N * XS_N] += c[k]; if (reset) g_ext_stops[k].store(0); }
 	return BSX_OK;
 }
 
@@ -818,6 +852,7 @@
 	G.seeds_dense = (const DevIntv*)L.out.p;
 	G.out = (bsx_region_t*)L.regs.p; G.out_cap = B.regs_cap; G.out_cursor = &SH->region_cursor;
 	G.counters = dev_counters(L); G.pos = (unsigned long long*)L.pos.p;
+	TRY(ext_stop_arm(L, L.st, B.trace));
 	G.ext_pk = !B.long_reads && ext_pk_wanted() && ext_pk_scoring(L.sc, 0, B.max_len, true);
 	++g_ext_forms[G.ext_pk ? 0 : 1];
 	M.X.base = (unsigned char*)L.xpool.p; M.X.cap = B.xcap; M.X.cursor = &SH->xpool_cursor; M.X.xcount = &M.c->front.x_count;
@@ -1220,6 +1255,15 @@
 	HIPCHK(hipMemsetAsync(ctr + CTR_EXT, 0, sizeof(xp), L.st));
 	if (xp[EXT4_JOBS] || xp[EXTL_JOBS]) fprintf(stderr, "[M::regions_batch] k_ext4: %llu jobs, %llu rows in %llu wave trips (%.2f rows per trip), %llu passes between extensions, %.2f slots per trip, %llu rows of narrow jobs\n", xp[0], xp[1], xp[2], xp[2] ? (double)xp[1] / xp[2] : 0.0, xp[3], xp[2] ? (double)xp[4] / xp[2] : 0.0, xp[5]);
 	if (xp[EXTL_JOBS]) fprintf(stderr, "[M::regions_batch] k_extl: %llu jobs (%llu sent on to k_ext4), %llu rows in %llu wave trips (%.1f rows per trip), %llu passes between extensions\n", xp[6], xp[10], xp[7], xp[8], xp[8] ? (double)xp[7] / xp[8] : 0.0, xp[9]);
+	{
+		unsigned long long xs[XS_FAM_N * XS_N];
+		int rc = ext_stop_collect(L, L.st, xs);
+		if (rc != BSX_OK) return rc;
+		static const char *fam[XS_FAM_N] = {"k_ext4", "k_extl", "tiers", "k_c2r", "batch"};
+		for (int k = 0; k < XS_FAM_N; ++k) if (xs[XS_N * k + XS_EVALS])
+			fprintf(stderr, "[M::regions_batch] ext_stop=%d %s: %llu extensions stopped by the rule, %llu evaluations, %llu rows still to run at the stops | the switch off: %llu would have stopped, %llu rows run after the rule would have fired\n",
+			        L.sc.ext_stop, fam[k], xs[XS_N * k + XS_STOPS], xs[XS_N * k + XS_EVALS], xs[XS_N * k + XS_LEFT], xs[XS_N * k + XS_WOULD], xs[XS_N * k + XS_DEAD]);
+	}
 	unsigned long long xw[CTR_X4W_N];
 	D2H(L.st, xw, ctr + CTR_X4W, sizeof(xw));
 	HIPCHK(hipMemsetAsync(ctr + CTR_X4W, 0, sizeof(xw), L.st));
@@ -1408,6 +1452,7 @@
 	HIPCHK(hipSetDevice(d->ordinal));
 	if (bsx_tune_is_set("ext4")) {
 		int rc, max_q = 0;
+		if ((rc = ext_stop_arm(L, L.st, true)) != BSX_OK) return rc;
 		for (int64_t i = 0; i < n; ++i) max_q = std::max(max_q, jobs[i].qlen);
 		if ((max_q > x4_max_query(16) && bsx_tune_long("ext4", 0) != 3) || n > 0x7fffffff) return BSX_E_ARG;
 		if (bsx_tune_long("ext4", 0) == 4) {
@@ -1421,6 +1466,8 @@
 			++g_ext_forms[packed ? 0 : 1];
 			HIPCHK(hipGetLastError());
 			D2H(L.st, res, L.res.p, (size_t)n * sizeof(bsx_ext_res_t));
+			if ((rc = ext_stop_collect(L, L.st, nullptr)) != BSX_OK) return rc;
+			L.sc.xs_ctr = nullptr;
 			for (int64_t i = 0; i < n; ++i) if (res[i].score == X4_DECLINED) return BSX_E_ARG;
 			return BSX_OK;
 		}
@@ -1441,6 +1488,8 @@
 		}
 		HIPCHK(hipGetLastError());
 		D2H(L.st, res, L.res.p, (size_t)n * sizeof(bsx_ext_res_t));
+		if ((rc = ext_stop_collect(L, L.st, nullptr)) != BSX_OK) return rc;
+		L.sc.xs_ctr = nullptr;
 		for (int64_t i = 0; i < n; ++i) if (res[i].score == X4_DECLINED) return BSX_E_ARG;
 		return BSX_OK;
 	}
diff --git a/biscuit_amd/csrc/hip/shim_dev.hpp b/biscuit_amd/csrc/hip/shim_dev.hpp
--- a/biscuit_amd/csrc/hip/shim_dev.hpp
+++ b/biscuit_amd/csrc/hip/shim_dev.hpp
@@ -35,6 +35,7 @@
 	int64_t rb_tasks = 0;
 	int flt_key[3] = {-1, -1, -1};
 	DevBuf fltab, jobs, res, scratch, scratch2, out, aux, pool, regs, regmeta, slabs, slabs3, slabflags, redo, pos, posoff, xpool, xmeta, x4jobs, tags, mdpool, gctx, qcjobs, qcpool, mdkeys, mdres, mdslot, dd, sswjobs, c2rslab;
+	DevBuf xstop;
 	DevBuf small;
 	HostBuf hstage;
 	HostBuf pin;
@@ -60,7 +61,7 @@
 	void release_buffers()
 	{
 		DevBuf *b[] = {&reads, &gath, &qpack, &fltab, &jobs, &res, &scratch, &scratch2, &out, &aux, &pool, &regs, &regmeta, &slabs, &slabs3, &slabflags, &redo, &pos, &posoff, &xpool, &xmeta,
-		               &x4jobs, &tags, &mdpool, &gctx, &qcjobs, &qcpool, &mdkeys, &mdres, &mdslot, &dd, &sswjobs, &c2rslab, &small, &msw_jobs, &msw_res, &msw_meta, &msw_roff};
+		               &x4jobs, &tags, &mdpool, &gctx, &qcjobs, &qcpool, &mdkeys, &mdres, &mdslot, &dd, &sswjobs, &c2rslab, &small, &xstop, &msw_jobs, &msw_res, &msw_meta, &msw_roff};
 		for (DevBuf *x : b) x->release();
 		hstage.release(); pin.release(); flt_key[0] = -1;
 	}
diff --git a/biscuit_amd/csrc/host/tune.c b/biscuit_amd/csrc/host/tune.c
--- a/biscuit_amd/csrc/host/tune.c
+++ b/biscuit_amd/csrc/host/tune.c
@@ -34,6 +34,7 @@
 	{"ext4", "[off] tests: bsx_extend_batch through the quarter-wave kernel (1) / then the lane-per-job kernel (2) of the regions path / through the wavefront-per-job form with a register window (3) / with the rows of the region kernels' inline extensions, packed 16-bit when the batch allows (4)", 0},
 	{"sw_form", "[off] tests: bsx_sw_batch through the seed filter's alignments, score only, jobs of up to 199 x 199 in the order given -- ssw16: the packed 16-bit kernel (k_swl16), sixteen consecutive jobs to a wavefront, qlen = 0 an empty job; scoring options it cannot hold fail the call / ssw32: a wavefront per job through the 32-bit alignment of a seed without room in the job list", 0},
 	{"ext_pk", "[1] extension rows of 64 columns and more in packed 16-bit, two columns per lane (ext_pk.hpp), where the scoring options keep every intermediate inside 16 bits; 0: always the 32-bit rows", 0},
+	{"ext_stop", "[1] an extension ends once no row it still has to run can change a result field (ext_stop_rule.h); 0: every row runs, as in ksw_extend2 (same results; with phases the rows that would have been saved are counted)", 0},
 	{"chain_stages", "[3] how consecutive chunks' front halves are chained on the device: 0 none, 1 seeding, 2 seeding and regions, 3 the same but the HBM tiers hold nobody back, 4 strictly one after the other", 0},
 	{"small_copies_unmasked", "[1] the front half's copies of less than 256 KB go through the lane's unmasked stream (the CUs the front-half streams leave alone); 0: through the stream they are ordered on", 0},
 	{"reserve_cu_every", "[0] n >= 2: the front-half streams leave one compute unit in n (of every shader engine of every XCD) to the back half's short batches; < 2: none", 0},
diff --git a/include/bsx.h b/include/bsx.h
--- a/include/bsx.h
+++ b/include/bsx.h
@@ -368,6 +368,7 @@
 void bsx_chunk_slice_offset(int64_t first);
 int bsx_device_region_work(bsx_device_t *dev, uint64_t w[5], int reset);
 int bsx_ext_forms(uint64_t c[2], int reset);
+int bsx_ext_stops(uint64_t c[26], int reset);
 int bsx_device_seed_table(bsx_device_t *dev, uint64_t *lookups, int *depth, int reset);
 int bsx_device_kernel_time(bsx_device_t *dev, int k, double *total_ms, int64_t *launches, int reset);
 
```

Result: faster. 753,700 (median of 6 runs) (+6.6%).
